# google/lyra

Measured on NVIDIA H100. Metric: 20ms-frame encode+decode throughput (frames/s) @16kHz, higher is better.
Workload: dtype f32+i8 (decoder fp32 GEMMs: split tf32 on tensor cores)

## Files before the change

lyra_b200/csrc/engine.cu:

```cuda
#include <cmath>
#include <cstdio>
#include <cstdlib>
#include <cstring>
#include <string>
#include <vector>

#include "../../include/lyra_b200.h"
#include "aux_kernels.cuh"
#include "model_spec.h"
#include "net_kernels.cuh"
#include "net_kernels_wgmma.cuh"
#include "plc_kernels.cuh"

using namespace lyra_b200;

namespace {

std::string g_create_error;

#define CU(call)                                                                        \
  do {                                                                                  \
    cudaError_t e_ = (call);                                                            \
    if (e_ != cudaSuccess) {                                                            \
      ctx->err = std::string(#call) + ": " + cudaGetErrorString(e_);                    \
      return LYRA_B200_ENODEV;                                                          \
    }                                                                                   \
  } while (0)

#define ENTER(role)                                                                     \
  if (!UseDevice(ctx)) return LYRA_B200_ENODEV;                                         \
  if ((role) && !RoleOk(ctx, (role))) return LYRA_B200_EINVAL;

}

struct lyra_b200_ctx {
  ModelSpec spec;
  int device = 0, max_streams = 0, ntiles = 0, padded = 0;
  int roles = LYRA_B200_ROLE_ENCODER | LYRA_B200_ROLE_DECODER;
  std::vector<void*> allocs;
  enum Check { kCheckNone, kCheckPlc, kCheckResamplerPos, kCheckStreamRate, kCheckStreamBits };
  struct StateEntry {
    StreamStateEntry e;
    bool reset;
    int check;
  };
  std::vector<StateEntry> state_list;
  StreamStateTable state_table{};
  StreamStateTable reset_table{};
  uint64_t model_fingerprint = 0;
  uint32_t* d_records = nullptr;
  int records_chunk = 0;
  uint8_t* d_blob = nullptr;
  uint32_t* d_state[4] = {nullptr, nullptr, nullptr, nullptr};
  int* d_n18[4] = {nullptr, nullptr, nullptr, nullptr};
  float* d_mid_enc = nullptr;
  float* d_mid_dec = nullptr;
  int16_t* d_logmel_prev[3] = {nullptr, nullptr, nullptr};
  float* d_noise = nullptr;
  float* d_noise_est = nullptr;
  uint8_t* d_is_noise = nullptr;
  float* d_noise_enc = nullptr;
  int16_t* d_logmel_prev_enc = nullptr;
  NoiseParams noise_params{};
  int* d_plc = nullptr;
  double* d_cng_work = nullptr;
  unsigned long long* d_cng_hops = nullptr;
  unsigned long long cng_seed = 0;
  uint8_t* d_plan = nullptr;
  uint8_t* d_skip = nullptr;
  uint8_t* d_feed = nullptr;
  uint8_t* d_is_cn = nullptr;
  int* d_fade0 = nullptr;
  int* d_dir = nullptr;
  int16_t* d_model_pcm = nullptr;
  int16_t* d_cng_pcm = nullptr;
  float* d_cng_feat = nullptr;
  int16_t* d_rs_delay[2] = {nullptr, nullptr};
  int* d_rs_pos[2] = {nullptr, nullptr};
  int16_t* d_rs_in = nullptr;
  int16_t* d_rs_out = nullptr;
  int* d_rs_counts = nullptr;
  int sample_rate = 16000;
  int codec_rs_tag = 1;
  int16_t* d_codec_rs_delay[2] = {nullptr, nullptr};
  int* d_codec_rs_pos[2] = {nullptr, nullptr};
  int* d_stream_rate = nullptr;
  bool rate_override = false;
  ByRate<NoiseParams> enc_noise_params{};
  ByRate<LogMelParams> enc_logmel{};
  int* d_stream_bits[2] = {nullptr, nullptr};
  std::vector<int> bits_mirror[2];
  int own_bits[2] = {0, 0};
  int16_t* d_pcm = nullptr;
  uint8_t* d_packets = nullptr;
  uint8_t* d_received = nullptr;
  float* d_features = nullptr;
  float* d_melout = nullptr;
  int* d_indices = nullptr;
  int* d_ids = nullptr;
  int* d_tile_list = nullptr;
  int* d_slot_of = nullptr;
  int* h_tile_list[2] = {nullptr, nullptr};
  int* h_slot_of[2] = {nullptr, nullptr};
  cudaEvent_t ev_map[2] = {nullptr, nullptr};
  bool map_pending[2] = {false, false};
  int map_buf = 0;
  std::vector<uint32_t> tile_gen;
  uint32_t map_gen = 0;
  std::vector<uint32_t> id_seen;
  uint32_t id_gen = 0;
  std::vector<int> touched[2];
  int map_dense_n = -1;
  int active_tiles = 0;
  cudaStream_t own_stream = nullptr, stream = nullptr;
  static constexpr int kMaxSplit = 4;
  cudaStream_t aux_stream[kMaxSplit - 1] = {nullptr, nullptr, nullptr};
  cudaEvent_t ev_fork = nullptr, ev_join[kMaxSplit - 1] = {nullptr, nullptr, nullptr};
  int nsplit = 3;
  bool blocking_sync = false;
  cudaEvent_t ev_sync = nullptr;
  int decoder_mode = LYRA_B200_DECODER_EXACT;
  int priority = 0;
  uint64_t launches = 0;
  struct GraphKey {
    int kind, n, num_bits, mode, nsplit;
    const void *a, *b, *c;
    bool rates, bits;
    bool operator==(const GraphKey& o) const {
      return kind == o.kind && n == o.n && num_bits == o.num_bits && mode == o.mode && nsplit == o.nsplit && a == o.a && b == o.b && c == o.c &&
             rates == o.rates && bits == o.bits;
    }
  };
  struct GraphEntry { GraphKey key; void* exec; uint64_t launches; };
  bool use_graphs = false;
  std::vector<GraphEntry> graphs;
  uint64_t graph_replays = 0;
  std::string err;
  bool profiling = false;
  std::vector<std::pair<cudaEvent_t, cudaEvent_t>> prof_events[LYRA_B200_NUM_KERNELS];
  size_t prof_used[LYRA_B200_NUM_KERNELS] = {};
  double prof_ms[LYRA_B200_NUM_KERNELS] = {};
  uint64_t prof_n[LYRA_B200_NUM_KERNELS] = {};
};

namespace {

int PacketBytes(int num_bits) { return (num_bits + 7) / 8; }

int RatePair(int rate_hz) { return rate_hz == 8000 ? 0 : rate_hz == 32000 ? 1 : rate_hz == 48000 ? 2 : -1; }
bool RateOk(int rate_hz) { return rate_hz == 16000 || RatePair(rate_hz) >= 0; }

bool Converts(const lyra_b200_ctx* ctx) { return ctx->sample_rate != 16000 || ctx->rate_override; }

NoiseParams MakeNoiseParams(int rate_hz) {
  NoiseParams p{};
  const float secs_per_hop = static_cast<float>(320) / rate_hz;
  p.nf = 160;
  p.hops_per_update = (int)std::round(1.f / secs_per_hop);
  p.max_smoothing = std::pow(0.5f, secs_per_hop / 0.7f);
  p.bound_decay = std::pow(0.5f, secs_per_hop / 1.f);
  p.log_nf = std::log((double)160);
  return p;
}

constexpr int kNoProf = -1;
struct ProfScope {
  lyra_b200_ctx* ctx;
  int k;
  cudaEvent_t stop = nullptr;
  cudaStream_t st;
  ProfScope(lyra_b200_ctx* c, int kernel, cudaStream_t stream) : ctx(c), k(kernel), st(stream) {
    if (!ctx->profiling || k == kNoProf) return;
    auto& pool = ctx->prof_events[k];
    if (ctx->prof_used[k] == pool.size()) {
      cudaEvent_t a, b;
      cudaEventCreate(&a);
      cudaEventCreate(&b);
      pool.emplace_back(a, b);
    }
    auto& ev = pool[ctx->prof_used[k]++];
    cudaEventRecord(ev.first, st);
    stop = ev.second;
  }
  ~ProfScope() { if (stop) cudaEventRecord(stop, st); }
};

template <typename Fn>
int Launch(lyra_b200_ctx* ctx, int prof, cudaStream_t st, Fn launch) {
  {
    ProfScope ps(ctx, prof, st);
    launch();
  }
  ctx->launches += 1;
  CU(cudaGetLastError());
  return LYRA_B200_OK;
}
#define LAUNCH(prof, kernel, grid, block, smem, st, ...) \
  Launch(ctx, (prof), (st), [&]() { LYRA_LAUNCH(kernel, grid, block, smem, st, __VA_ARGS__); })

void ProfDrain(lyra_b200_ctx* ctx) {
  for (int k = 0; k < LYRA_B200_NUM_KERNELS; ++k) {
    for (size_t i = 0; i < ctx->prof_used[k]; ++i) {
      float ms = 0.0f;
      if (cudaEventElapsedTime(&ms, ctx->prof_events[k][i].first, ctx->prof_events[k][i].second) == cudaSuccess) {
        ctx->prof_ms[k] += ms;
        ctx->prof_n[k] += 1;
      }
    }
    ctx->prof_used[k] = 0;
  }
}

cudaError_t SyncStream(lyra_b200_ctx* ctx) {
  if (!ctx->blocking_sync) return cudaStreamSynchronize(ctx->stream);
  cudaError_t e = cudaEventRecord(ctx->ev_sync, ctx->stream);
  return e != cudaSuccess ? e : cudaEventSynchronize(ctx->ev_sync);
}

bool UseDevice(lyra_b200_ctx* ctx) {
  if (cudaSetDevice(ctx->device) == cudaSuccess) return true;
  ctx->err = "cudaSetDevice failed";
  return false;
}

bool RoleOk(lyra_b200_ctx* ctx, int role) {
  if (ctx->roles & role) return true;
  ctx->err = role == LYRA_B200_ROLE_ENCODER ? "this context was created without the encoder role" : "this context was created without the decoder role";
  return false;
}

bool BitsOk(lyra_b200_ctx* ctx, int num_bits) {
  if (num_bits <= 0 || num_bits > LYRA_B200_MAX_BITS) { ctx->err = "the number of bits cannot exceed 184"; return false; }
  if (num_bits % ctx->spec.bits_per_stage != 0) { ctx->err = "the number of bits has to be divisible by the bits per quantizer (4)"; return false; }
  return true;
}

bool StreamBitsOk(const lyra_b200_ctx* ctx, int bits) {
  return bits > 0 && bits <= LYRA_B200_MAX_BITS && bits % ctx->spec.bits_per_stage == 0;
}

const int* BitsWord(const lyra_b200_ctx* ctx, int r) { return ctx->own_bits[r] ? ctx->d_stream_bits[r] : nullptr; }

void SetMirrorBits(lyra_b200_ctx* ctx, int r, int id, int bits) {
  int& w = ctx->bits_mirror[r][(size_t)id];
  ctx->own_bits[r] += (bits != 0) - (w != 0);
  w = bits;
}

uint32_t NextIdGen(lyra_b200_ctx* ctx) {
  if (++ctx->id_gen == 0) { std::fill(ctx->id_seen.begin(), ctx->id_seen.end(), 0u); ctx->id_gen = 1; }
  return ctx->id_gen;
}

int CheckIds(lyra_b200_ctx* ctx, const int32_t* ids, int n, bool allow_repeats) {
  if (n <= 0 || n > ctx->max_streams) { ctx->err = "stream count out of range"; return LYRA_B200_EINVAL; }
  if (!ids) return LYRA_B200_OK;
  const uint32_t gen = NextIdGen(ctx);
  for (int k = 0; k < n; ++k) {
    const int id = ids[k];
    if (id < 0 || id >= ctx->max_streams) { ctx->err = "stream id out of range"; return LYRA_B200_EINVAL; }
    if (allow_repeats) continue;
    if (ctx->id_seen[(size_t)id] == gen) { ctx->err = "duplicate stream id in one call"; return LYRA_B200_EINVAL; }
    ctx->id_seen[(size_t)id] = gen;
  }
  return LYRA_B200_OK;
}

int UploadIds(lyra_b200_ctx* ctx, const int32_t* ids, int n, const int** d_ids) {
  *d_ids = nullptr;
  if (!ids) return LYRA_B200_OK;
  CU(cudaMemcpyAsync(ctx->d_ids, ids, sizeof(int) * (size_t)n, cudaMemcpyHostToDevice, ctx->stream));
  *d_ids = ctx->d_ids;
  return LYRA_B200_OK;
}

int PrepareMap(lyra_b200_ctx* ctx, const int32_t* ids, int n) {
  int rc = CheckIds(ctx, ids, n, false);
  if (rc) return rc;
  if (ids == nullptr && ctx->map_dense_n == n) return LYRA_B200_OK;
  const int b = ctx->map_buf;
  if (ctx->map_pending[b]) { CU(cudaEventSynchronize(ctx->ev_map[b])); ctx->map_pending[b] = false; }
  int* slot_of = ctx->h_slot_of[b];
  int* tile_list = ctx->h_tile_list[b];
  for (int id : ctx->touched[b]) slot_of[id] = -1;
  ctx->touched[b].clear();
  int ntl = 0;
  for (int k = 0; k < n; ++k) {
    const int id = ids ? ids[k] : k;
    slot_of[id] = k;
    ctx->touched[b].push_back(id);
  }
  if (++ctx->map_gen == 0) { std::fill(ctx->tile_gen.begin(), ctx->tile_gen.end(), 0u); ctx->map_gen = 1; }
  for (int k = 0; k < n; ++k) {
    const int t = (ids ? ids[k] : k) / kTileStreams;
    if (ctx->tile_gen[(size_t)t] != ctx->map_gen) { ctx->tile_gen[(size_t)t] = ctx->map_gen; tile_list[ntl++] = t; }
  }
  ctx->active_tiles = ntl;
  CU(cudaMemcpyAsync(ctx->d_slot_of, slot_of, sizeof(int) * (size_t)ctx->padded, cudaMemcpyHostToDevice, ctx->stream));
  CU(cudaMemcpyAsync(ctx->d_tile_list, tile_list, sizeof(int) * (size_t)ntl, cudaMemcpyHostToDevice, ctx->stream));
  CU(cudaEventRecord(ctx->ev_map[b], ctx->stream));
  ctx->map_pending[b] = true;
  ctx->map_buf = b ^ 1;
  ctx->map_dense_n = ids ? -1 : n;
  return LYRA_B200_OK;
}

struct Part {
  int tile0, ntiles, slot0, nslots;
  cudaStream_t st;
};
Part WholeCall(lyra_b200_ctx* ctx, int n) { return Part{0, ctx->active_tiles, 0, n, ctx->stream}; }

int LaunchEncoderNets(lyra_b200_ctx* ctx, const Part& p, const uint8_t* skip, const int16_t* d_pcm, float* d_features) {
  const TileIo io{ctx->d_tile_list + p.tile0, ctx->d_slot_of, skip};
  const int rc = LAUNCH(0, EncoderKernelA, dim3((unsigned)p.ntiles), dim3(EncA::NT), (size_t)EncA::kSmemBytes, p.st,
                        ctx->d_blob, ctx->spec.enc, io, d_pcm, reinterpret_cast<float*>(ctx->d_state[0]), ctx->d_n18[0], ctx->d_mid_enc);
  return rc ? rc : LAUNCH(1, EncoderKernelB, dim3((unsigned)p.ntiles), dim3(EncB::NT), (size_t)EncB::kSmemBytes, p.st,
                          ctx->d_blob, ctx->spec.enc, io, ctx->d_mid_enc, reinterpret_cast<float*>(ctx->d_state[1]), ctx->d_n18[1], d_features);
}

int LaunchQuantize(lyra_b200_ctx* ctx, const Part& p, const float* d_features, int num_bits, uint8_t* d_packets, int* d_indices,
                   const uint8_t* d_skip = nullptr, const int* bits_word = nullptr, const int* d_ids = nullptr) {
  const int nq = num_bits / ctx->spec.bits_per_stage, pb = PacketBytes(num_bits);
  const int blocks = (p.nslots + kRvqSlotsPerBlock - 1) / kRvqSlotsPerBlock;
  return LAUNCH(2, RvqEncodeKernel, dim3((unsigned)blocks), dim3(kRvqThreads), (size_t)(2 * 1024 * 4 + kRvqSlotsPerBlock * (64 * 4 + 48 * 4)), p.st,
                ctx->d_blob, ctx->spec.rvq, d_features + (size_t)p.slot0 * 64, p.nslots, nq, d_packets + (size_t)p.slot0 * pb, pb,
                d_indices ? d_indices + (size_t)p.slot0 * 46 : nullptr, d_skip ? d_skip + p.slot0 : nullptr, bits_word, d_ids, p.slot0);
}

int LaunchDequantize(lyra_b200_ctx* ctx, const Part& p, const uint8_t* d_packets, const uint8_t* d_received, int num_bits, float* d_features,
                     const int* bits_word = nullptr, const int* d_ids = nullptr) {
  const int nq = num_bits / ctx->spec.bits_per_stage, pb = PacketBytes(num_bits);
  const int blocks = (p.nslots * 64 + 255) / 256;
  return LAUNCH(3, RvqDecodeKernel, dim3((unsigned)blocks), dim3(256), (size_t)0, p.st,
                ctx->d_blob, ctx->spec.rvq, d_packets + (size_t)p.slot0 * pb, pb, d_received ? d_received + p.slot0 : nullptr, p.nslots, nq,
                d_features + (size_t)p.slot0 * 64, bits_word, d_ids, p.slot0);
}

int LaunchDecoderNets(lyra_b200_ctx* ctx, const Part& p, const uint8_t* skip, const float* d_features, int16_t* d_pcm) {
  const TileIo io{ctx->d_tile_list + p.tile0, ctx->d_slot_of, skip};
  const bool tc = ctx->decoder_mode == LYRA_B200_DECODER_TENSOR;
  const dim3 grid((unsigned)p.ntiles);
  float* st_c = reinterpret_cast<float*>(ctx->d_state[2]);
  float* st_d = reinterpret_cast<float*>(ctx->d_state[3]);
  const int rc = tc ? LAUNCH(4, DecoderKernelC<true>, grid, dim3(DecC<true>::NT), (size_t)DecC<true>::kSmemBytes, p.st,
                             ctx->d_blob, ctx->spec.dec, io, d_features, st_c, ctx->d_n18[2], ctx->d_mid_dec)
                    : LAUNCH(4, DecoderKernelC<false>, grid, dim3(DecC<false>::NT), (size_t)DecC<false>::kSmemBytes, p.st,
                             ctx->d_blob, ctx->spec.dec, io, d_features, st_c, ctx->d_n18[2], ctx->d_mid_dec);
  if (rc) return rc;
  return tc ? LAUNCH(5, DecoderKernelDW, grid, dim3(DecDW::NT), (size_t)DecDW::kSmemBytes, p.st,
                     ctx->d_blob, ctx->spec.dec, io, ctx->d_mid_dec, st_d, ctx->d_n18[3], d_pcm)
            : LAUNCH(5, DecoderKernelD, grid, dim3(DecD::NT), (size_t)DecD::kSmemBytes, p.st,
                     ctx->d_blob, ctx->spec.dec, io, ctx->d_mid_dec, st_d, ctx->d_n18[3], d_pcm);
}

int SplitParts(lyra_b200_ctx* ctx, int n, Part* parts) {
  int np = ctx->nsplit < 1 ? 1 : (ctx->nsplit > lyra_b200_ctx::kMaxSplit ? lyra_b200_ctx::kMaxSplit : ctx->nsplit);
  if (!(ctx->map_dense_n == n && ctx->active_tiles >= 64 * np)) np = 1;
  if (np == 1) { parts[0] = WholeCall(ctx, n); return 1; }
  for (int i = 0; i < np; ++i) {
    const int t0 = (int)((long long)ctx->active_tiles * i / np), t1 = (int)((long long)ctx->active_tiles * (i + 1) / np);
    const int s0 = t0 * kTileStreams, s1 = i + 1 == np ? n : t1 * kTileStreams;
    parts[i] = Part{t0, t1 - t0, s0, s1 - s0, i == 0 ? ctx->stream : ctx->aux_stream[i - 1]};
  }
  return np;
}
int Fork(lyra_b200_ctx* ctx, int nparts) {
  if (nparts < 2) return LYRA_B200_OK;
  CU(cudaEventRecord(ctx->ev_fork, ctx->stream));
  for (int i = 1; i < nparts; ++i) CU(cudaStreamWaitEvent(ctx->aux_stream[i - 1], ctx->ev_fork, 0));
  return LYRA_B200_OK;
}
int Join(lyra_b200_ctx* ctx, int nparts) {
  for (int i = 1; i < nparts; ++i) {
    CU(cudaEventRecord(ctx->ev_join[i - 1], ctx->aux_stream[i - 1]));
    CU(cudaStreamWaitEvent(ctx->stream, ctx->ev_join[i - 1], 0));
  }
  return LYRA_B200_OK;
}
int JoinAfter(lyra_b200_ctx* ctx, int nparts, int rc) {
  if (!rc) return Join(ctx, nparts);
  const std::string first = ctx->err;
  Join(ctx, nparts);
  cudaStreamSynchronize(ctx->stream);
  ctx->err = first;
  return rc;
}

template <typename Fn>
int ForEachPart(lyra_b200_ctx* ctx, int n, Fn body) {
  Part parts[lyra_b200_ctx::kMaxSplit];
  const int np = SplitParts(ctx, n, parts);
  int rc = Fork(ctx, np);
  if (rc) return rc;
  for (int i = 0; i < np && !rc; ++i) rc = body(parts[i]);
  return JoinAfter(ctx, np, rc);
}

int LaunchLogMel(lyra_b200_ctx* ctx, cudaStream_t st, const ByRate<LogMelParams>& S, const int* rate_word, int rate, const int* d_ids,
                 int slot0, int count, int n, const int16_t* d_pcm, int16_t* carried, const uint8_t* d_mask) {
  const LogMelParams& P = S.p[0];
  const size_t smem = sizeof(double) * (size_t)(2 * kLogMelFftPadded + P.fft / 2 + 1 + P.window_len + P.window_len / 8 + 1);
  return LAUNCH(6, LogMelKernel, dim3((unsigned)count), dim3(kLogMelThreads), smem, st,
                ctx->d_blob, S, rate_word, rate, d_ids, n, d_pcm, carried, ctx->d_melout, d_mask, slot0);
}

int LaunchNoiseUpdate(lyra_b200_ctx* ctx, cudaStream_t st, const int* d_ids, int slot0, int count, int n, const int16_t* d_pcm,
                      const uint8_t* d_mask, uint8_t* d_is_noise, float* d_estimate, bool encoder_side = false) {
  float* noise_state = encoder_side ? ctx->d_noise_enc : ctx->d_noise;
  int16_t* carried = encoder_side ? ctx->d_logmel_prev_enc : ctx->d_logmel_prev[2];
  const int* rate_word = encoder_side ? ctx->d_stream_rate : nullptr;
  const int rate = encoder_side ? ctx->sample_rate : 16000;
  const int rc = LaunchLogMel(ctx, st, encoder_side ? ctx->enc_logmel : Uniform(ctx->spec.logmel160), rate_word, rate, d_ids, slot0, count, n,
                              d_pcm, carried, d_mask);
  return rc ? rc : LAUNCH(7, NoiseEstimatorKernel, dim3((unsigned)count), dim3(kNoiseThreads), sizeof(float) * (size_t)(2 * 160 + 2), st,
                          encoder_side ? ctx->enc_noise_params : Uniform(ctx->noise_params), rate_word, rate, d_ids, n, ctx->d_melout, d_mask,
                          noise_state, d_is_noise, d_estimate, slot0);
}

int LaunchComfortNoise(lyra_b200_ctx* ctx, cudaStream_t st, const int* d_ids, int slot0, int count, int n, const float* d_features,
                       const uint8_t* d_plan) {
  const size_t smem = sizeof(double) * (size_t)(4 * kLogMelFftPadded + 160);
  return LAUNCH(kNoProf, ComfortNoiseKernel, dim3((unsigned)count), dim3(kCngThreads), smem, st,
                ctx->d_blob, ctx->spec.cng, d_ids, n, d_features, ctx->d_noise, NoiseStateUnits(ctx->noise_params.nf),
                d_plan, ctx->d_cng_work, ctx->d_cng_hops, ctx->cng_seed, ctx->d_cng_pcm, slot0);
}

int LaunchCodecResample(lyra_b200_ctx* ctx, const Part& p, int dir, const int* d_ids, int n, const int16_t* in, int16_t* out) {
  const int ext = ctx->sample_rate / 50;
  const int in_stride = dir ? LYRA_B200_HOP : ext, out_stride = dir ? ext : LYRA_B200_HOP;
  return LAUNCH(kNoProf, ResampleKernel, dim3((unsigned)p.nslots), dim3(128), sizeof(float) * (size_t)(kResamplerTaps - 1 + in_stride), p.st,
                ctx->d_blob, ctx->spec.resampler, dir ? 3 : 0, ctx->codec_rs_tag, d_ids, n, in, in_stride, in_stride, out, out_stride,
                nullptr, ctx->d_codec_rs_delay[dir], ctx->d_codec_rs_pos[dir], p.slot0, ctx->d_stream_rate, ctx->sample_rate);
}

enum CallKind { kEncode, kDecode, kEncodeDtx, kDecodeTrackNoise, kDecodePlc };

struct CodecCall {
  struct Io {
    const int16_t* pcm_in = nullptr;
    int16_t* pcm_out = nullptr;
    const uint8_t* packets_in = nullptr;
    uint8_t* packets_out = nullptr;
    const uint8_t* received = nullptr;
    uint8_t* flags = nullptr;
  };
  CallKind kind;
  int n, num_bits;
  const int32_t* ids = nullptr;
  Io dev, host;
  int32_t* packet_bytes = nullptr;
  const int* d_ids = nullptr;
};

int RunEncode(lyra_b200_ctx* ctx, const CodecCall& c) {
  const CodecCall::Io &d = c.dev, &h = c.host;
  const bool dtx = c.kind == kEncodeDtx;
  const size_t pb = (size_t)PacketBytes(c.num_bits), hop = (size_t)ctx->sample_rate / 50;
  const bool rs = Converts(ctx);
  int16_t* stage = rs ? ctx->d_rs_in : ctx->d_pcm;
  const int16_t* in = h.pcm_in ? stage : d.pcm_in;
  const int16_t* pcm16 = rs ? ctx->d_pcm : in;
  const uint8_t* skip = dtx ? d.flags : nullptr;
  return ForEachPart(ctx, c.n, [&](const Part& p) {
    int rc = LYRA_B200_OK;
    if (h.pcm_in)
      CU(cudaMemcpyAsync(stage + (size_t)p.slot0 * hop, h.pcm_in + (size_t)p.slot0 * hop, sizeof(int16_t) * hop * (size_t)p.nslots,
                         cudaMemcpyHostToDevice, p.st));
    if (rs && (rc = LaunchCodecResample(ctx, p, 0, c.d_ids, c.n, in, ctx->d_pcm))) return rc;
    if (dtx) {
      if ((rc = LaunchNoiseUpdate(ctx, p.st, c.d_ids, p.slot0, p.nslots, c.n, pcm16, nullptr, d.flags, nullptr, true))) return rc;
      if (h.flags) CU(cudaMemcpyAsync(h.flags + p.slot0, d.flags + p.slot0, (size_t)p.nslots, cudaMemcpyDeviceToHost, p.st));
    }
    if ((rc = LaunchEncoderNets(ctx, p, skip, pcm16, ctx->d_features))) return rc;
    if ((rc = LaunchQuantize(ctx, p, ctx->d_features, c.num_bits, d.packets_out, nullptr, skip, BitsWord(ctx, 0), c.d_ids))) return rc;
    if (h.packets_out)
      CU(cudaMemcpyAsync(h.packets_out + (size_t)p.slot0 * pb, d.packets_out + (size_t)p.slot0 * pb, pb * (size_t)p.nslots, cudaMemcpyDeviceToHost, p.st));
    return LYRA_B200_OK;
  });
}

int RunDecode(lyra_b200_ctx* ctx, const CodecCall& c) {
  const CodecCall::Io &d = c.dev, &h = c.host;
  const size_t pb = (size_t)PacketBytes(c.num_bits), hop = (size_t)ctx->sample_rate / 50;
  const bool rs = Converts(ctx);
  int16_t* out = h.pcm_out && rs ? ctx->d_rs_out : d.pcm_out;
  int16_t* pcm16 = rs ? ctx->d_pcm : out;
  return ForEachPart(ctx, c.n, [&](const Part& p) {
    int rc = LYRA_B200_OK;
    if (h.packets_in)
      CU(cudaMemcpyAsync(ctx->d_packets + (size_t)p.slot0 * pb, h.packets_in + (size_t)p.slot0 * pb, pb * (size_t)p.nslots, cudaMemcpyHostToDevice, p.st));
    if (h.received)
      CU(cudaMemcpyAsync(ctx->d_received + p.slot0, h.received + p.slot0, (size_t)p.nslots, cudaMemcpyHostToDevice, p.st));
    if ((rc = LaunchDequantize(ctx, p, d.packets_in, d.received, c.num_bits, ctx->d_features, BitsWord(ctx, 1), c.d_ids))) return rc;
    if ((rc = LaunchDecoderNets(ctx, p, nullptr, ctx->d_features, pcm16))) return rc;
    if (c.kind == kDecodeTrackNoise) {
      if ((rc = LaunchNoiseUpdate(ctx, p.st, c.d_ids, p.slot0, p.nslots, c.n, pcm16, d.received, d.flags, nullptr))) return rc;
      if (h.flags) CU(cudaMemcpyAsync(h.flags + p.slot0, d.flags + p.slot0, (size_t)p.nslots, cudaMemcpyDeviceToHost, p.st));
    }
    if (rs && (rc = LaunchCodecResample(ctx, p, 1, c.d_ids, c.n, pcm16, out))) return rc;
    if (h.pcm_out)
      CU(cudaMemcpyAsync(h.pcm_out + (size_t)p.slot0 * hop, out + (size_t)p.slot0 * hop, sizeof(int16_t) * hop * (size_t)p.nslots,
                         cudaMemcpyDeviceToHost, p.st));
    return LYRA_B200_OK;
  });
}

int RunDecodePlc(lyra_b200_ctx* ctx, const CodecCall& c) {
  const CodecCall::Io &d = c.dev, &h = c.host;
  const size_t pb = (size_t)PacketBytes(c.num_bits), hop = (size_t)ctx->sample_rate / 50;
  const bool rs = Converts(ctx);
  int16_t* out = h.pcm_out && rs ? ctx->d_rs_out : d.pcm_out;
  int16_t* pcm16 = rs ? ctx->d_pcm : out;
  if (h.received) CU(cudaMemcpyAsync(ctx->d_received, h.received, (size_t)c.n, cudaMemcpyHostToDevice, ctx->stream));
  if (int rc = LAUNCH(kNoProf, PlcPlanKernel, dim3((unsigned)((c.n + 255) / 256)), dim3(256), (size_t)0, ctx->stream,
                      c.d_ids, c.n, d.received, ctx->d_plc, ctx->d_plan, ctx->d_fade0, ctx->d_dir, ctx->d_skip, ctx->d_feed, d.flags))
    return rc;
  return ForEachPart(ctx, c.n, [&](const Part& p) {
    int rc = LYRA_B200_OK;
    if (h.packets_in)
      CU(cudaMemcpyAsync(ctx->d_packets + (size_t)p.slot0 * pb, h.packets_in + (size_t)p.slot0 * pb, pb * (size_t)p.nslots, cudaMemcpyHostToDevice, p.st));
    if ((rc = LaunchDequantize(ctx, p, d.packets_in, d.received, c.num_bits, ctx->d_features, BitsWord(ctx, 1), c.d_ids))) return rc;
    if ((rc = LaunchDecoderNets(ctx, p, ctx->d_skip, ctx->d_features, ctx->d_model_pcm))) return rc;
    if ((rc = LaunchComfortNoise(ctx, p.st, c.d_ids, p.slot0, p.nslots, c.n, nullptr, ctx->d_plan))) return rc;
    if ((rc = LAUNCH(kNoProf, PlcMixKernel, dim3((unsigned)p.nslots), dim3(320), (size_t)0, p.st,
                     ctx->d_blob, ctx->spec.cng, p.nslots, ctx->d_plan + p.slot0, ctx->d_fade0 + p.slot0, ctx->d_dir + p.slot0,
                     ctx->d_model_pcm + (size_t)p.slot0 * 320, ctx->d_cng_pcm + (size_t)p.slot0 * 320, pcm16 + (size_t)p.slot0 * 320)))
      return rc;
    if ((rc = LaunchNoiseUpdate(ctx, p.st, c.d_ids, p.slot0, p.nslots, c.n, ctx->d_model_pcm, ctx->d_feed, nullptr, nullptr))) return rc;
    if (rs && (rc = LaunchCodecResample(ctx, p, 1, c.d_ids, c.n, pcm16, out))) return rc;
    if (h.pcm_out)
      CU(cudaMemcpyAsync(h.pcm_out + (size_t)p.slot0 * hop, out + (size_t)p.slot0 * hop, sizeof(int16_t) * hop * (size_t)p.nslots,
                         cudaMemcpyDeviceToHost, p.st));
    if (h.flags) CU(cudaMemcpyAsync(h.flags + p.slot0, d.flags + p.slot0, (size_t)p.nslots, cudaMemcpyDeviceToHost, p.st));
    return LYRA_B200_OK;
  });
}

bool SetSmemLimits() {
  return LYRA_SET_MAX_SMEM(EncoderKernelA, EncA::kSmemBytes) == 0 && LYRA_SET_MAX_SMEM(EncoderKernelB, EncB::kSmemBytes) == 0 &&
         LYRA_SET_MAX_SMEM(DecoderKernelC<false>, DecC<false>::kSmemBytes) == 0 && LYRA_SET_MAX_SMEM(DecoderKernelD, DecD::kSmemBytes) == 0 &&
         LYRA_SET_MAX_SMEM(DecoderKernelC<true>, DecC<true>::kSmemBytes) == 0 && LYRA_SET_MAX_SMEM(DecoderKernelDW, DecDW::kSmemBytes) == 0;
}

std::vector<uint32_t> InitImage(const ModelSpec& s, int which) {
  auto pack = [](int zp) { const uint32_t b = (uint32_t)(zp & 0xff); return b | (b << 8) | (b << 16) | (b << 24); };
  std::vector<uint32_t> v;
  if (which == 0) {
    v.assign(EncStateA::kUnits, 0u);
  } else if (which == 1) {
    v.assign(EncStateB::kUnits, 0u);
    for (int i = EncStateB::kRingQ0; i < EncStateB::kRingQ1; ++i) v[(size_t)i] = pack(s.enc.zp_state[0]);
    for (int i = EncStateB::kRingQ1; i < EncStateB::kDown2; ++i) v[(size_t)i] = pack(s.enc.zp_state[1]);
    for (int i = EncStateB::kDown2; i < EncStateB::kBott; ++i) v[(size_t)i] = pack(s.enc.zp_state[2]);
    for (int i = EncStateB::kBott; i < EncStateB::kUnits; ++i) v[(size_t)i] = pack(s.enc.zp_state[3]);
  } else if (which == 2) {
    v.assign(DecStateC::kUnits, 0u);
    for (int i = DecStateC::kRingM; i < DecStateC::kRingQ0; ++i) v[(size_t)i] = pack(s.dec.zp_state[0]);
    for (int i = DecStateC::kRingQ0; i < DecStateC::kRingQ1; ++i) v[(size_t)i] = pack(s.dec.zp_state[1]);
    for (int i = DecStateC::kRingQ1; i < DecStateC::kUnits; ++i) v[(size_t)i] = pack(s.dec.zp_state[2]);
  } else {
    v.assign(DecStateD::kUnits, 0u);
  }
  return v;
}

template <typename T>
bool DevAlloc(lyra_b200_ctx* ctx, T** p, size_t count) {
  const size_t bytes = sizeof(T) * (count ? count : 1);
  if (cudaMalloc(reinterpret_cast<void**>(p), bytes) != cudaSuccess) return false;
  ctx->allocs.push_back(*p);
  return cudaMemset(*p, 0, bytes) == cudaSuccess;
}

template <typename T>
bool DevStreamState(lyra_b200_ctx* ctx, T** p, size_t per_stream, const void* init = nullptr, int kind = kStatePlain,
                    int check = lyra_b200_ctx::kCheckNone, bool reset = true, int lanes = 1, int** n18 = nullptr) {
  const int words = (int)(sizeof(T) * per_stream / 4);
  uint32_t* d_init = nullptr;
  if (!DevAlloc(ctx, p, (size_t)ctx->padded * per_stream)) return false;
  if (n18 && !DevAlloc(ctx, n18, (size_t)ctx->padded)) return false;
  if (init && !(DevAlloc(ctx, &d_init, (size_t)words) && cudaMemcpy(d_init, init, 4 * (size_t)words, cudaMemcpyHostToDevice) == cudaSuccess))
    return false;
  ctx->state_list.push_back({{reinterpret_cast<uint32_t*>(*p), d_init, n18 ? *n18 : nullptr, words, lanes, 0, kind}, reset, check});
  return true;
}

uint64_t ModelFingerprint(const std::vector<uint8_t>& blob) {
  uint64_t h = 0xcbf29ce484222325ull ^ (uint64_t)blob.size();
  size_t i = 0;
  for (; i + 8 <= blob.size(); i += 8) {
    uint64_t w;
    std::memcpy(&w, blob.data() + i, 8);
    h = (h ^ w) * 0x100000001b3ull;
  }
  for (; i < blob.size(); ++i) h = (h ^ blob[i]) * 0x100000001b3ull;
  return h;
}

bool BuildStateTable(lyra_b200_ctx* ctx) {
  StreamStateTable& T = ctx->state_table;
  StreamStateTable& R = ctx->reset_table;
  if ((int)ctx->state_list.size() > kStateMaxEntries) return false;
  int off = 0;
  T.count = R.count = 0;
  for (lyra_b200_ctx::StateEntry& s : ctx->state_list) {
    s.e.offset = off;
    off += s.e.words + (s.e.n18 ? 1 : 0);
    T.e[T.count++] = s.e;
    if (s.reset) R.e[R.count++] = s.e;
  }
  T.record_words = kStateHeaderWords + off;
  std::memset(T.header, 0, sizeof(T.header));
  T.header[kHdrMagic] = kStateMagic;
  T.header[kHdrVersion] = kStateVersion;
  T.header[kHdrBytes] = (uint32_t)(4 * T.record_words);
  T.header[kHdrRoles] = (uint32_t)ctx->roles;
  T.header[kHdrModelLo] = (uint32_t)ctx->model_fingerprint;
  T.header[kHdrModelHi] = (uint32_t)(ctx->model_fingerprint >> 32);
  return true;
}

#ifndef LYRA_EMU
bool PinnedHost(const void* p) {
  if (p == nullptr) return true;
  cudaPointerAttributes at;
  if (cudaPointerGetAttributes(&at, p) != cudaSuccess) { cudaGetLastError(); return false; }
  return at.type == cudaMemoryTypeHost;
}
void DropGraphs(lyra_b200_ctx* ctx) {
  for (auto& e : ctx->graphs) cudaGraphExecDestroy(reinterpret_cast<cudaGraphExec_t>(e.exec));
  ctx->graphs.clear();
}
#endif

template <typename Fn>
int RunMaybeGraphed(lyra_b200_ctx* ctx, const lyra_b200_ctx::GraphKey& key, bool eligible, Fn enqueue) {
#ifdef LYRA_EMU
  (void)key; (void)eligible;
  return enqueue();
#else
  if (!ctx->use_graphs || !eligible || ctx->profiling || !PinnedHost(key.a) || !PinnedHost(key.b) || !PinnedHost(key.c)) return enqueue();
  for (auto& e : ctx->graphs)
    if (e.key == key) {
      CU(cudaGraphLaunch(reinterpret_cast<cudaGraphExec_t>(e.exec), ctx->stream));
      ctx->launches += e.launches;
      ++ctx->graph_replays;
      return LYRA_B200_OK;
    }
  const uint64_t l0 = ctx->launches;
  if (cudaStreamBeginCapture(ctx->stream, cudaStreamCaptureModeThreadLocal) != cudaSuccess) {
    cudaGetLastError();
    ctx->use_graphs = false;
    return enqueue();
  }
  const int rc = enqueue();
  cudaGraph_t g = nullptr;
  const cudaError_t ce = cudaStreamEndCapture(ctx->stream, &g);
  cudaGraphExec_t exec = nullptr;
  if (rc == LYRA_B200_OK && ce == cudaSuccess && g != nullptr && cudaGraphInstantiate(&exec, g, 0) == cudaSuccess) {
    cudaGraphDestroy(g);
    if (ctx->graphs.size() >= 32) {
      cudaGraphExecDestroy(reinterpret_cast<cudaGraphExec_t>(ctx->graphs.front().exec));
      ctx->graphs.erase(ctx->graphs.begin());
    }
    ctx->graphs.push_back(lyra_b200_ctx::GraphEntry{key, exec, ctx->launches - l0});
    CU(cudaGraphLaunch(exec, ctx->stream));
    return LYRA_B200_OK;
  }
  if (g) cudaGraphDestroy(g);
  cudaGetLastError();
  ctx->use_graphs = false;
  ctx->launches = l0;
  return enqueue();
#endif
}

int RunCodecCall(lyra_b200_ctx* ctx, CodecCall c) {
  const bool encoder = c.kind == kEncode || c.kind == kEncodeDtx;
  const int role = encoder ? LYRA_B200_ROLE_ENCODER : LYRA_B200_ROLE_DECODER;
  ENTER(role);
  if (!BitsOk(ctx, c.num_bits)) return LYRA_B200_EINVAL;
  const int r = encoder ? 0 : 1;
  const std::vector<int>& own = ctx->bits_mirror[r];
  for (int k = 0; k < c.n && ctx->own_bits[r]; ++k) {
    const int id = c.ids ? c.ids[k] : k;
    if (id >= 0 && id < ctx->max_streams && own[(size_t)id] > c.num_bits) {
      ctx->err = "a listed stream's own bit count (lyra_b200_set_stream_bits) is above the call's num_bits";
      return LYRA_B200_EINVAL;
    }
  }
  const bool by_id = Converts(ctx) || (c.kind != kEncode && c.kind != kDecode) || ctx->own_bits[r];
  int rc = PrepareMap(ctx, c.ids, c.n);
  if (rc || (by_id && (rc = UploadIds(ctx, c.ids, c.n, &c.d_ids)))) return rc;
  const bool host = c.host.packets_in || c.host.packets_out;
  if (host) {
    c.dev.pcm_in = c.dev.pcm_out = ctx->d_pcm;
    c.dev.packets_in = c.dev.packets_out = ctx->d_packets;
    c.dev.received = c.host.received ? ctx->d_received : nullptr;
  }
  if (!c.dev.flags) c.dev.flags = c.kind == kDecodePlc ? ctx->d_is_cn : ctx->d_is_noise;
  std::vector<uint8_t> dtx_flags;
  if (c.packet_bytes) {
    dtx_flags.resize((size_t)c.n);
    c.host.flags = dtx_flags.data();
  }
  const CodecCall::Io& h = c.host;
  const lyra_b200_ctx::GraphKey key =
      encoder ? lyra_b200_ctx::GraphKey{kEncode, c.n, c.num_bits, 0, ctx->nsplit, h.pcm_in, h.packets_out, nullptr, ctx->rate_override,
                                        ctx->own_bits[r] != 0}
              : lyra_b200_ctx::GraphKey{kDecode, c.n, c.num_bits, ctx->decoder_mode, ctx->nsplit, h.packets_in, h.received, h.pcm_out,
                                        ctx->rate_override, ctx->own_bits[r] != 0};
  const bool graphed = host && (c.kind == kEncode || c.kind == kDecode) && c.ids == nullptr && ctx->map_dense_n == c.n;
  if ((rc = RunMaybeGraphed(ctx, key, graphed, [&]() {
         return encoder ? RunEncode(ctx, c) : c.kind == kDecodePlc ? RunDecodePlc(ctx, c) : RunDecode(ctx, c);
       })))
    return rc;
  if (!host) return LYRA_B200_OK;
  CU(SyncStream(ctx));
  for (int k = 0; k < c.n && c.packet_bytes; ++k) {
    const int b = own[(size_t)(c.ids ? c.ids[k] : k)];
    c.packet_bytes[k] = dtx_flags[(size_t)k] ? 0 : PacketBytes(b ? b : c.num_bits);
  }
  return LYRA_B200_OK;
}


size_t RecordBytes(const lyra_b200_ctx* ctx) { return 4 * (size_t)ctx->state_table.record_words; }

int EnsureRecordStaging(lyra_b200_ctx* ctx) {
  if (ctx->d_records) return LYRA_B200_OK;
  const size_t fit = ((size_t)64 << 20) / RecordBytes(ctx);
  const int chunk = fit < 1 ? 1 : fit > (size_t)kStateChunk ? kStateChunk : (int)fit;
  uint32_t* p = nullptr;
  CU(cudaMalloc(reinterpret_cast<void**>(&p), RecordBytes(ctx) * (size_t)chunk));
  ctx->allocs.push_back(p);
  ctx->d_records = p;
  ctx->records_chunk = chunk;
  return LYRA_B200_OK;
}

bool PlcStateOk(int cp, int fp, int dir) {
  return cp >= 0 && cp <= kPlcConcealSamples && cp % 320 == 0 && fp >= 0 && fp <= kPlcFadeSamples && fp % 320 == 0 &&
         (dir == 1 || dir == -1);
}

bool StreamRateOk(const lyra_b200_ctx* ctx, int rate_hz) { return RateOk(rate_hz) && rate_hz <= ctx->sample_rate; }

uint32_t RecordWord(const uint8_t* rec, int i) {
  uint32_t w;
  std::memcpy(&w, rec + 4 * (size_t)i, 4);
  return w;
}

const char* RecordProblem(const lyra_b200_ctx* ctx, const uint8_t* rec) {
  const StreamStateTable& T = ctx->state_table;
  if (RecordWord(rec, kHdrMagic) != kStateMagic) return "not a stream-state record";
  if (RecordWord(rec, kHdrVersion) != kStateVersion) return "record format version differs";
  if (RecordWord(rec, kHdrBytes) != T.header[kHdrBytes] || RecordWord(rec, kHdrRoles) != T.header[kHdrRoles])
    return "record size / roles differ from this context's";
  if (RecordWord(rec, kHdrRate) != (uint32_t)ctx->sample_rate) return "record is from a context at another sample rate";
  if (RecordWord(rec, kHdrModelLo) != T.header[kHdrModelLo] || RecordWord(rec, kHdrModelHi) != T.header[kHdrModelHi])
    return "record is from another model";
  if (RecordWord(rec, kHdrZero5) || RecordWord(rec, kHdrLive0) > 1 || RecordWord(rec, kHdrLive1) > 1) return "malformed record header";
  for (int i = kHdrKeyHi + 1; i < kStateHeaderWords; ++i)
    if (RecordWord(rec, i)) return "malformed record header";
  for (int i = 0; i < T.count; ++i) {
    const StreamStateEntry& e = T.e[i];
    const int w0 = kStateHeaderWords + e.offset;
    if (e.n18 && RecordWord(rec, w0 + e.words) >= 18u) return "hop counter out of range";
    const int check = ctx->state_list[(size_t)i].check;
    if (check == lyra_b200_ctx::kCheckResamplerPos && (int32_t)RecordWord(rec, w0) < 0) return "resampler position out of range";
    if (check == lyra_b200_ctx::kCheckPlc &&
        !PlcStateOk((int32_t)RecordWord(rec, w0), (int32_t)RecordWord(rec, w0 + 1), (int32_t)RecordWord(rec, w0 + 2)))
      return "decoder control state out of range";
    if (check == lyra_b200_ctx::kCheckStreamRate && RecordWord(rec, w0) != 0 && !StreamRateOk(ctx, (int32_t)RecordWord(rec, w0)))
      return "stream sample rate unsupported or above the context's";
    if (check == lyra_b200_ctx::kCheckStreamBits && RecordWord(rec, w0) != 0 && !StreamBitsOk(ctx, (int32_t)RecordWord(rec, w0)))
      return "stream bit count is not a multiple of 4 in 4..184";
  }
  return nullptr;
}

int CheckCopyIds(lyra_b200_ctx* ctx, const int32_t* src, const int32_t* dst, int n) {
  if (n <= 0 || n > ctx->max_streams) { ctx->err = "stream count out of range"; return LYRA_B200_EINVAL; }
  const uint32_t g[2] = {NextIdGen(ctx), NextIdGen(ctx)};
  for (int k = 0; k < n; ++k) {
    const int id = src[k];
    if (id < -1 || id >= ctx->max_streams) { ctx->err = "source stream id out of range"; return LYRA_B200_EINVAL; }
    if (id < 0) continue;
    if (ctx->id_seen[(size_t)id] == g[0]) { ctx->err = "repeated source stream id"; return LYRA_B200_EINVAL; }
    ctx->id_seen[(size_t)id] = g[0];
  }
  for (int k = 0; k < n; ++k) {
    const int id = dst[k];
    if (id < 0 || id >= ctx->max_streams) { ctx->err = "destination stream id out of range"; return LYRA_B200_EINVAL; }
    if (ctx->id_seen[(size_t)id] == g[1]) { ctx->err = "repeated destination stream id"; return LYRA_B200_EINVAL; }
    if (ctx->id_seen[(size_t)id] == g[0]) { ctx->err = "a stream id is both a source and a destination"; return LYRA_B200_EINVAL; }
    ctx->id_seen[(size_t)id] = g[1];
  }
  return LYRA_B200_OK;
}

dim3 StateGrid(const StreamStateTable& T, int rows, int extra) {
  return dim3((unsigned)((rows + kStateRows - 1) / kStateRows), (unsigned)(T.count + extra));
}

int CopyStreamState(lyra_b200_ctx* ctx, const StreamStateTable& T, const int32_t* src, const int32_t* dst, int n) {
  StreamIdChunk ids;
  for (int k0 = 0; k0 < n; k0 += kStateChunk) {
    ids.n = n - k0 < kStateChunk ? n - k0 : kStateChunk;
    for (int k = 0; k < ids.n; ++k) {
      ids.src[k] = src ? src[k0 + k] : -1;
      ids.dst[k] = dst ? dst[k0 + k] : k0 + k;
    }
    if (int rc = LAUNCH(kNoProf, StreamStateCopyKernel, StateGrid(T, ids.n, 0), dim3(kStateThreads), (size_t)0, ctx->stream, T, ids))
      return rc;
  }
  return LYRA_B200_OK;
}

int LaunchStreamWords(lyra_b200_ctx* ctx, const int32_t* ids, int n, const int32_t* values, int ctx_value, int* word, int* conv0 = nullptr,
                      int* conv1 = nullptr) {
  StreamRateChunk c;
  for (int k0 = 0; k0 < n; k0 += kStateChunk) {
    c.n = n - k0 < kStateChunk ? n - k0 : kStateChunk;
    for (int k = 0; k < c.n; ++k) {
      c.ids[k] = ids ? ids[k0 + k] : k0 + k;
      c.rates[k] = values ? values[k0 + k] : ctx_value;
    }
    if (int rc = LAUNCH(kNoProf, StreamRateKernel, dim3((unsigned)((c.n + kStreamRateThreads - 1) / kStreamRateThreads)),
                        dim3(kStreamRateThreads), (size_t)0, ctx->stream, c, ctx_value, word, conv0, conv1))
      return rc;
  }
  return LYRA_B200_OK;
}
int LaunchStreamRates(lyra_b200_ctx* ctx, const int32_t* ids, int n, const int32_t* rates) {
  return LaunchStreamWords(ctx, ids, n, rates, ctx->sample_rate, ctx->d_stream_rate, ctx->d_codec_rs_pos[0], ctx->d_codec_rs_pos[1]);
}

int BitsRole(lyra_b200_ctx* ctx, int role) {
  if (role != LYRA_B200_ROLE_ENCODER && role != LYRA_B200_ROLE_DECODER) { ctx->err = "role must be LYRA_B200_ROLE_ENCODER or _DECODER"; return -1; }
  return RoleOk(ctx, role) ? role - 1 : -1;
}

}

extern "C" {

int lyra_b200_create(const char* model_dir, int device, int max_streams, lyra_b200_ctx** out) {
  return lyra_b200_create_ex(model_dir, device, max_streams, LYRA_B200_ROLE_ENCODER | LYRA_B200_ROLE_DECODER, out);
}

int lyra_b200_create_ex(const char* model_dir, int device, int max_streams, int roles, lyra_b200_ctx** out) {
  if (out) *out = nullptr;
  if (!out || !model_dir || max_streams <= 0 || (roles & ~3) || roles == 0) { g_create_error = "bad argument"; return LYRA_B200_EINVAL; }
  int ndev = 0;
  if (cudaGetDeviceCount(&ndev) != cudaSuccess || ndev <= 0) {
    g_create_error = "no CUDA device available (lyra_b200 has no CPU fallback)";
    return LYRA_B200_ENODEV;
  }
  if (device < 0 || device >= ndev) { g_create_error = "CUDA device index out of range"; return LYRA_B200_ENODEV; }
  lyra_b200_ctx* ctx = new lyra_b200_ctx();
  try {
    ctx->spec = BuildModelSpec(model_dir);
  } catch (const std::exception& e) {
    g_create_error = e.what();
    delete ctx;
    return LYRA_B200_EMODEL;
  }
  ctx->device = device;
  ctx->max_streams = max_streams;
  ctx->roles = roles;
  ctx->ntiles = (max_streams + kTileStreams - 1) / kTileStreams;
  ctx->padded = ctx->ntiles * kTileStreams;
  ctx->tile_gen.assign((size_t)ctx->ntiles, 0u);
  ctx->id_seen.assign((size_t)max_streams, 0u);
  const size_t P = (size_t)ctx->padded;
  bool ok = cudaSetDevice(device) == cudaSuccess;
  int prio = 0;
  if (const char* e = std::getenv(roles == LYRA_B200_ROLE_DECODER ? "LYRA_B200_DEC_PRIORITY" : "LYRA_B200_ENC_PRIORITY")) prio = std::atoi(e);
  ctx->priority = prio;
  ok = ok && cudaStreamCreateWithPriority(&ctx->own_stream, cudaStreamDefault, prio) == cudaSuccess;
  for (int i = 0; i < lyra_b200_ctx::kMaxSplit - 1; ++i) {
    ok = ok && cudaStreamCreateWithPriority(&ctx->aux_stream[i], cudaStreamDefault, prio) == cudaSuccess;
    ok = ok && cudaEventCreateWithFlags(&ctx->ev_join[i], cudaEventDisableTiming) == cudaSuccess;
  }
  ok = ok && cudaEventCreateWithFlags(&ctx->ev_fork, cudaEventDisableTiming) == cudaSuccess;
  ok = ok && cudaEventCreateWithFlags(&ctx->ev_sync, cudaEventDisableTiming | cudaEventBlockingSync) == cudaSuccess;
  ctx->stream = ctx->own_stream;
  ok = ok && DevAlloc(ctx, &ctx->d_blob, ctx->spec.blob.size());
  ok = ok && cudaMemcpy(ctx->d_blob, ctx->spec.blob.data(), ctx->spec.blob.size(), cudaMemcpyHostToDevice) == cudaSuccess;
  const int units[4] = {EncStateA::kUnits, EncStateB::kUnits, DecStateC::kUnits, DecStateD::kUnits};
  for (int w = 0; w < 4 && ok; ++w) {
    if (!(roles & (w < 2 ? LYRA_B200_ROLE_ENCODER : LYRA_B200_ROLE_DECODER))) continue;
    ok = DevStreamState(ctx, &ctx->d_state[w], (size_t)units[w], InitImage(ctx->spec, w).data(), kStatePlain, lyra_b200_ctx::kCheckNone,
                        true, kTileStreams, &ctx->d_n18[w]);
  }
  if (roles & LYRA_B200_ROLE_ENCODER) ok = ok && DevAlloc(ctx, &ctx->d_mid_enc, P * 128 * 4);
  if (roles & LYRA_B200_ROLE_DECODER) ok = ok && DevAlloc(ctx, &ctx->d_mid_dec, P * 128 * 4);
  for (int b = 0; b < 3; ++b) ok = ok && DevStreamState(ctx, &ctx->d_logmel_prev[b], LYRA_B200_HOP);
  ctx->noise_params = MakeNoiseParams(16000);
  for (int r : {16000, 8000, 32000, 48000}) {
    ctx->enc_noise_params.p[RateIndex(r)] = MakeNoiseParams(r);
    ctx->enc_logmel.p[RateIndex(r)] = r == 16000 ? ctx->spec.logmel160 : ctx->spec.logmel160_ext[RatePair(r)];
  }
  ok = ok && DevStreamState(ctx, &ctx->d_noise, NoiseStateUnits(160));
  ok = ok && DevAlloc(ctx, &ctx->d_noise_est, P * 160);
  ok = ok && DevStreamState(ctx, &ctx->d_noise_enc, NoiseStateUnits(160));
  ok = ok && DevStreamState(ctx, &ctx->d_logmel_prev_enc, LYRA_B200_HOP);
  const int plc0[4] = {0, 0, -1, 0};
  ok = ok && DevStreamState(ctx, &ctx->d_plc, 4, plc0, kStatePlain, lyra_b200_ctx::kCheckPlc);
  ok = ok && DevStreamState(ctx, &ctx->d_cng_work, 1024);
  ok = ok && DevStreamState(ctx, &ctx->d_cng_hops, 2, nullptr, kStateCng);
  ok = ok && DevAlloc(ctx, &ctx->d_plan, P);
  ok = ok && DevAlloc(ctx, &ctx->d_skip, P);
  ok = ok && DevAlloc(ctx, &ctx->d_feed, P);
  ok = ok && DevAlloc(ctx, &ctx->d_is_cn, P);
  ok = ok && DevAlloc(ctx, &ctx->d_fade0, P);
  ok = ok && DevAlloc(ctx, &ctx->d_dir, P);
  ok = ok && DevAlloc(ctx, &ctx->d_model_pcm, P * LYRA_B200_HOP);
  ok = ok && DevAlloc(ctx, &ctx->d_cng_pcm, P * LYRA_B200_HOP);
  ok = ok && DevAlloc(ctx, &ctx->d_cng_feat, P * 160);
  for (int d = 0; d < 2; ++d) {
    ok = ok && DevStreamState(ctx, &ctx->d_rs_delay[d], (size_t)(kResamplerTaps - 1), nullptr, kStatePlain, lyra_b200_ctx::kCheckNone, false);
    ok = ok && DevStreamState(ctx, &ctx->d_rs_pos[d], 2, nullptr, kStatePlain, lyra_b200_ctx::kCheckResamplerPos);
  }
  for (int d = 0; d < 2; ++d) {
    if (!(roles & (d == 0 ? LYRA_B200_ROLE_ENCODER : LYRA_B200_ROLE_DECODER))) continue;
    ok = ok && DevStreamState(ctx, &ctx->d_codec_rs_delay[d], (size_t)(kResamplerTaps - 1));
    ok = ok && DevStreamState(ctx, &ctx->d_codec_rs_pos[d], 2, nullptr, d == 0 ? kStateCodecRs0 : kStateCodecRs1,
                              lyra_b200_ctx::kCheckResamplerPos);
  }
  for (int r = 0; r < 2; ++r) {
    if (!(roles & (r + 1))) continue;
    ok = ok && DevStreamState(ctx, &ctx->d_stream_bits[r], 1, nullptr, kStatePlain, lyra_b200_ctx::kCheckStreamBits);
    ctx->bits_mirror[r].assign((size_t)max_streams, 0);
  }
  ok = ok && DevStreamState(ctx, &ctx->d_stream_rate, 1, nullptr, kStatePlain, lyra_b200_ctx::kCheckStreamRate);
  ok = ok && DevAlloc(ctx, &ctx->d_rs_in, P * 960);
  ok = ok && DevAlloc(ctx, &ctx->d_rs_out, P * 968);
  ok = ok && DevAlloc(ctx, &ctx->d_rs_counts, P);
  ok = ok && DevAlloc(ctx, &ctx->d_is_noise, P);
  ok = ok && DevAlloc(ctx, &ctx->d_pcm, P * LYRA_B200_HOP);
  ok = ok && DevAlloc(ctx, &ctx->d_packets, P * 24);
  ok = ok && DevAlloc(ctx, &ctx->d_received, P);
  ok = ok && DevAlloc(ctx, &ctx->d_features, P * LYRA_B200_NUM_FEATURES);
  ok = ok && DevAlloc(ctx, &ctx->d_melout, P * 160);
  ok = ok && DevAlloc(ctx, &ctx->d_indices, P * LYRA_B200_MAX_STAGES);
  ok = ok && DevAlloc(ctx, &ctx->d_ids, P);
  ok = ok && DevAlloc(ctx, &ctx->d_tile_list, (size_t)ctx->ntiles);
  ok = ok && DevAlloc(ctx, &ctx->d_slot_of, P);
  for (int b = 0; b < 2 && ok; ++b) {
    ok = ok && cudaMallocHost(reinterpret_cast<void**>(&ctx->h_slot_of[b]), sizeof(int) * P) == cudaSuccess;
    ok = ok && cudaMallocHost(reinterpret_cast<void**>(&ctx->h_tile_list[b]), sizeof(int) * (size_t)ctx->ntiles) == cudaSuccess;
    ok = ok && cudaEventCreateWithFlags(&ctx->ev_map[b], cudaEventDisableTiming) == cudaSuccess;
    if (ok) for (size_t i = 0; i < P; ++i) ctx->h_slot_of[b][i] = -1;
  }
  if (ok) ok = SetSmemLimits();
  ctx->model_fingerprint = ModelFingerprint(ctx->spec.blob);
  ok = ok && BuildStateTable(ctx);
  if (!ok) {
    g_create_error = std::string("CUDA allocation / setup failed: ") + cudaGetErrorString(cudaGetLastError());
    lyra_b200_destroy(ctx);
    return LYRA_B200_ENODEV;
  }
  if (lyra_b200_reset(ctx, nullptr, max_streams) != LYRA_B200_OK) {
    g_create_error = ctx->err;
    lyra_b200_destroy(ctx);
    return LYRA_B200_ENODEV;
  }
  *out = ctx;
  return LYRA_B200_OK;
}

void lyra_b200_destroy(lyra_b200_ctx* ctx) {
  if (!ctx) return;
  UseDevice(ctx);
  for (void* p : ctx->allocs) cudaFree(p);
  for (int b = 0; b < 2; ++b) {
    if (ctx->h_slot_of[b]) cudaFreeHost(ctx->h_slot_of[b]);
    if (ctx->h_tile_list[b]) cudaFreeHost(ctx->h_tile_list[b]);
    if (ctx->ev_map[b]) cudaEventDestroy(ctx->ev_map[b]);
  }
  for (int k = 0; k < LYRA_B200_NUM_KERNELS; ++k)
    for (auto& ev : ctx->prof_events[k]) { cudaEventDestroy(ev.first); cudaEventDestroy(ev.second); }
#ifndef LYRA_EMU
  DropGraphs(ctx);
#endif
  if (ctx->ev_fork) cudaEventDestroy(ctx->ev_fork);
  if (ctx->ev_sync) cudaEventDestroy(ctx->ev_sync);
  for (int i = 0; i < lyra_b200_ctx::kMaxSplit - 1; ++i) {
    if (ctx->ev_join[i]) cudaEventDestroy(ctx->ev_join[i]);
    if (ctx->aux_stream[i]) cudaStreamDestroy(ctx->aux_stream[i]);
  }
  if (ctx->own_stream) cudaStreamDestroy(ctx->own_stream);
  delete ctx;
}

const char* lyra_b200_last_error(const lyra_b200_ctx* ctx) { return ctx ? ctx->err.c_str() : g_create_error.c_str(); }
int lyra_b200_max_streams(const lyra_b200_ctx* ctx) { return ctx ? ctx->max_streams : 0; }
int lyra_b200_tile_streams(const lyra_b200_ctx* ctx) { return ctx ? kTileStreams : 0; }
uint64_t lyra_b200_launch_count(const lyra_b200_ctx* ctx) { return ctx ? ctx->launches : 0; }

int lyra_b200_profile_enable(lyra_b200_ctx* ctx, int enable) {
  if (!ctx) return LYRA_B200_EINVAL;
  ENTER(0);
  CU(SyncStream(ctx));
  ProfDrain(ctx);
  ctx->profiling = enable != 0;
  if (enable) for (int k = 0; k < LYRA_B200_NUM_KERNELS; ++k) { ctx->prof_ms[k] = 0.0; ctx->prof_n[k] = 0; }
  return LYRA_B200_OK;
}

int lyra_b200_profile_read(lyra_b200_ctx* ctx, double* ms_sum, uint64_t* launches) {
  if (!ctx || !ms_sum || !launches) return LYRA_B200_EINVAL;
  ENTER(0);
  CU(SyncStream(ctx));
  ProfDrain(ctx);
  for (int k = 0; k < LYRA_B200_NUM_KERNELS; ++k) { ms_sum[k] = ctx->prof_ms[k]; launches[k] = ctx->prof_n[k]; }
  return LYRA_B200_OK;
}

int lyra_b200_reset(lyra_b200_ctx* ctx, const int32_t* stream_ids, int n) {
  if (!ctx) return LYRA_B200_EINVAL;
  ENTER(0);
  int rc = CheckIds(ctx, stream_ids, n, true);
  if (rc) return rc;
  std::vector<int32_t> distinct;
  if (stream_ids) {
    const uint32_t gen = NextIdGen(ctx);
    for (int k = 0; k < n; ++k)
      if (ctx->id_seen[(size_t)stream_ids[k]] != gen) { ctx->id_seen[(size_t)stream_ids[k]] = gen; distinct.push_back(stream_ids[k]); }
    stream_ids = distinct.data();
    n = (int)distinct.size();
  }
  if ((rc = CopyStreamState(ctx, ctx->reset_table, nullptr, stream_ids, n))) return rc;
  for (int r = 0; r < 2; ++r)
    for (int k = 0; k < n && ctx->own_bits[r]; ++k) SetMirrorBits(ctx, r, stream_ids ? stream_ids[k] : k, 0);
  CU(SyncStream(ctx));
  return LYRA_B200_OK;
}

int lyra_b200_set_stream(lyra_b200_ctx* ctx, void* cuda_stream) {
  if (!ctx) return LYRA_B200_EINVAL;
  ENTER(0);
  ctx->stream = cuda_stream ? reinterpret_cast<cudaStream_t>(cuda_stream) : ctx->own_stream;
  return LYRA_B200_OK;
}

int lyra_b200_set_split(lyra_b200_ctx* ctx, int parts) {
  if (!ctx || parts < 1 || parts > lyra_b200_ctx::kMaxSplit) return LYRA_B200_EINVAL;
  ENTER(0);
  ctx->nsplit = parts;
  return LYRA_B200_OK;
}

int lyra_b200_set_blocking_sync(lyra_b200_ctx* ctx, int enable) {
  if (!ctx) return LYRA_B200_EINVAL;
  ENTER(0);
  ctx->blocking_sync = enable != 0;
  return LYRA_B200_OK;
}

int lyra_b200_set_priority(lyra_b200_ctx* ctx, int priority) {
  if (!ctx) return LYRA_B200_EINVAL;
  ENTER(0);
  CU(SyncStream(ctx));
#ifndef LYRA_EMU
  DropGraphs(ctx);
#endif
  const bool own = ctx->stream == ctx->own_stream;
  cudaStream_t fresh[lyra_b200_ctx::kMaxSplit];
  for (int i = 0; i < lyra_b200_ctx::kMaxSplit; ++i)
    if (cudaStreamCreateWithPriority(&fresh[i], cudaStreamDefault, priority) != cudaSuccess) {
      while (i-- > 0) cudaStreamDestroy(fresh[i]);
      ctx->err = "cudaStreamCreateWithPriority failed";
      return LYRA_B200_ENODEV;
    }
  cudaStreamDestroy(ctx->own_stream);
  ctx->own_stream = fresh[0];
  for (int i = 0; i < lyra_b200_ctx::kMaxSplit - 1; ++i) { cudaStreamDestroy(ctx->aux_stream[i]); ctx->aux_stream[i] = fresh[i + 1]; }
  if (own) ctx->stream = ctx->own_stream;
  ctx->priority = priority;
  return LYRA_B200_OK;
}

int lyra_b200_set_decoder_mode(lyra_b200_ctx* ctx, int mode) {
  if (!ctx || (mode != LYRA_B200_DECODER_EXACT && mode != LYRA_B200_DECODER_TENSOR)) return LYRA_B200_EINVAL;
  ENTER(0);
  ctx->decoder_mode = mode;
  return LYRA_B200_OK;
}

int lyra_b200_decoder_mode(const lyra_b200_ctx* ctx) { return ctx ? ctx->decoder_mode : LYRA_B200_EINVAL; }

int lyra_b200_set_sample_rate(lyra_b200_ctx* ctx, int sample_rate_hz) {
  if (!ctx) return LYRA_B200_EINVAL;
  if (!RateOk(sample_rate_hz)) { ctx->err = "the codec calls run at 8000, 16000, 32000 or 48000 Hz"; return LYRA_B200_EINVAL; }
  ENTER(0);
  if (sample_rate_hz == ctx->sample_rate && !ctx->rate_override) return LYRA_B200_OK;
  CU(SyncStream(ctx));
  if (sample_rate_hz == ctx->sample_rate) {
    int rc = LaunchStreamRates(ctx, nullptr, ctx->max_streams, nullptr);
    if (rc) return rc;
    CU(SyncStream(ctx));
    ctx->rate_override = false;
    return LYRA_B200_OK;
  }
#ifndef LYRA_EMU
  DropGraphs(ctx);
#endif
  if (ctx->rate_override) {
    CU(cudaMemsetAsync(ctx->d_stream_rate, 0, sizeof(int) * (size_t)ctx->padded, ctx->stream));
    CU(SyncStream(ctx));
    ctx->rate_override = false;
  }
  ctx->sample_rate = sample_rate_hz;
  ctx->codec_rs_tag = ctx->codec_rs_tag % 1000000000 + 1;
  return LYRA_B200_OK;
}

int lyra_b200_set_stream_sample_rates(lyra_b200_ctx* ctx, const int32_t* stream_ids, int n, const int32_t* rates_hz) {
  if (!ctx || !rates_hz) return LYRA_B200_EINVAL;
  ENTER(0);
  int rc = CheckIds(ctx, stream_ids, n, false);
  if (rc) return rc;
  bool differs = false;
  for (int k = 0; k < n; ++k) {
    if (!StreamRateOk(ctx, rates_hz[k])) {
      ctx->err = "a stream runs at 8000, 16000, 32000 or 48000 Hz, at most the context's rate (lyra_b200_set_sample_rate)";
      return LYRA_B200_EINVAL;
    }
    differs |= rates_hz[k] != ctx->sample_rate;
  }
  if (!differs && !ctx->rate_override) return LYRA_B200_OK;
  if ((rc = LaunchStreamRates(ctx, stream_ids, n, rates_hz))) return rc;
  ctx->rate_override = true;
  return LYRA_B200_OK;
}

int lyra_b200_stream_sample_rates(lyra_b200_ctx* ctx, const int32_t* stream_ids, int n, int32_t* rates_hz) {
  if (!ctx || !rates_hz) return LYRA_B200_EINVAL;
  ENTER(0);
  const int rc = CheckIds(ctx, stream_ids, n, true);
  if (rc) return rc;
  CU(SyncStream(ctx));
  std::vector<int> words((size_t)ctx->max_streams);
  CU(cudaMemcpy(words.data(), ctx->d_stream_rate, sizeof(int) * words.size(), cudaMemcpyDeviceToHost));
  for (int k = 0; k < n; ++k) {
    const int w = words[(size_t)(stream_ids ? stream_ids[k] : k)];
    rates_hz[k] = w ? w : ctx->sample_rate;
  }
  return LYRA_B200_OK;
}

int lyra_b200_sample_rate(const lyra_b200_ctx* ctx) { return ctx ? ctx->sample_rate : LYRA_B200_EINVAL; }

int lyra_b200_set_stream_bits(lyra_b200_ctx* ctx, int role, const int32_t* stream_ids, int n, const int32_t* bits) {
  if (!ctx || !bits) return LYRA_B200_EINVAL;
  ENTER(0);
  const int r = BitsRole(ctx, role);
  if (r < 0) return LYRA_B200_EINVAL;
  int rc = CheckIds(ctx, stream_ids, n, false);
  if (rc) return rc;
  bool changes = false;
  for (int k = 0; k < n; ++k) {
    if (bits[k] != 0 && !StreamBitsOk(ctx, bits[k])) {
      ctx->err = "a stream's own bit count is 0 (the call's) or a multiple of 4 in 4..184";
      return LYRA_B200_EINVAL;
    }
    changes |= ctx->bits_mirror[r][(size_t)(stream_ids ? stream_ids[k] : k)] != bits[k];
  }
  if (!changes) return LYRA_B200_OK;
  if ((rc = LaunchStreamWords(ctx, stream_ids, n, bits, 0, ctx->d_stream_bits[r]))) return rc;
  for (int k = 0; k < n; ++k) SetMirrorBits(ctx, r, stream_ids ? stream_ids[k] : k, bits[k]);
  return LYRA_B200_OK;
}

int lyra_b200_stream_bits(lyra_b200_ctx* ctx, int role, const int32_t* stream_ids, int n, int32_t* bits) {
  if (!ctx || !bits) return LYRA_B200_EINVAL;
  ENTER(0);
  const int r = BitsRole(ctx, role);
  if (r < 0) return LYRA_B200_EINVAL;
  const int rc = CheckIds(ctx, stream_ids, n, true);
  if (rc) return rc;
  CU(SyncStream(ctx));
  std::vector<int> words((size_t)ctx->max_streams);
  CU(cudaMemcpy(words.data(), ctx->d_stream_bits[r], sizeof(int) * words.size(), cudaMemcpyDeviceToHost));
  for (int k = 0; k < n; ++k) bits[k] = words[(size_t)(stream_ids ? stream_ids[k] : k)];
  return LYRA_B200_OK;
}

int lyra_b200_synchronize(lyra_b200_ctx* ctx) {
  if (!ctx) return LYRA_B200_EINVAL;
  ENTER(0);
  CU(SyncStream(ctx));
  return LYRA_B200_OK;
}

int lyra_b200_encode_device(lyra_b200_ctx* ctx, int n, const int16_t* d_pcm, int num_bits, uint8_t* d_packets) {
  if (!ctx || !d_pcm || !d_packets) return LYRA_B200_EINVAL;
  CodecCall c{kEncode, n, num_bits};
  c.dev.pcm_in = d_pcm;
  c.dev.packets_out = d_packets;
  return RunCodecCall(ctx, c);
}

int lyra_b200_decode_device(lyra_b200_ctx* ctx, int n, const uint8_t* d_packets, const uint8_t* d_received, int num_bits,
                            int16_t* d_pcm) {
  if (!ctx || !d_packets || !d_pcm) return LYRA_B200_EINVAL;
  CodecCall c{kDecode, n, num_bits};
  c.dev.packets_in = d_packets;
  c.dev.received = d_received;
  c.dev.pcm_out = d_pcm;
  return RunCodecCall(ctx, c);
}

int lyra_b200_set_graphs(lyra_b200_ctx* ctx, int enable) {
  if (!ctx) return LYRA_B200_EINVAL;
  ENTER(0);
#ifndef LYRA_EMU
  CU(SyncStream(ctx));
  if (!enable) DropGraphs(ctx);
#endif
  ctx->use_graphs = enable != 0;
  return LYRA_B200_OK;
}
uint64_t lyra_b200_graph_replays(const lyra_b200_ctx* ctx) { return ctx ? ctx->graph_replays : 0; }

int lyra_b200_encode(lyra_b200_ctx* ctx, const int32_t* ids, int n, const int16_t* pcm, int num_bits, uint8_t* packets) {
  if (!ctx || !pcm || !packets) return LYRA_B200_EINVAL;
  CodecCall c{kEncode, n, num_bits, ids};
  c.host.pcm_in = pcm;
  c.host.packets_out = packets;
  return RunCodecCall(ctx, c);
}

int lyra_b200_decode(lyra_b200_ctx* ctx, const int32_t* ids, int n, const uint8_t* packets, const uint8_t* received,
                     int num_bits, int16_t* pcm) {
  if (!ctx || !packets || !pcm) return LYRA_B200_EINVAL;
  CodecCall c{kDecode, n, num_bits, ids};
  c.host.packets_in = packets;
  c.host.received = received;
  c.host.pcm_out = pcm;
  return RunCodecCall(ctx, c);
}

int lyra_b200_extract_features(lyra_b200_ctx* ctx, const int32_t* ids, int n, const int16_t* pcm, float* features) {
  if (!ctx || !pcm || !features) return LYRA_B200_EINVAL;
  ENTER(LYRA_B200_ROLE_ENCODER);
  int rc = PrepareMap(ctx, ids, n);
  if (rc) return rc;
  CU(cudaMemcpyAsync(ctx->d_pcm, pcm, sizeof(int16_t) * 320 * (size_t)n, cudaMemcpyHostToDevice, ctx->stream));
  if ((rc = LaunchEncoderNets(ctx, WholeCall(ctx, n), nullptr, ctx->d_pcm, ctx->d_features))) return rc;
  CU(cudaMemcpyAsync(features, ctx->d_features, sizeof(float) * 64 * (size_t)n, cudaMemcpyDeviceToHost, ctx->stream));
  CU(SyncStream(ctx));
  return LYRA_B200_OK;
}

int lyra_b200_quantize(lyra_b200_ctx* ctx, int n, const float* features, int num_bits, uint8_t* packets, int32_t* indices) {
  if (!ctx || !features || !packets) return LYRA_B200_EINVAL;
  ENTER(0);
  if (!BitsOk(ctx, num_bits)) return LYRA_B200_EINVAL;
  int rc = CheckIds(ctx, nullptr, n, false);
  if (rc) return rc;
  CU(cudaMemcpyAsync(ctx->d_features, features, sizeof(float) * 64 * (size_t)n, cudaMemcpyHostToDevice, ctx->stream));
  const Part whole{0, 0, 0, n, ctx->stream};
  rc = LaunchQuantize(ctx, whole, ctx->d_features, num_bits, ctx->d_packets, indices ? ctx->d_indices : nullptr);
  if (rc) return rc;
  CU(cudaMemcpyAsync(packets, ctx->d_packets, (size_t)PacketBytes(num_bits) * (size_t)n, cudaMemcpyDeviceToHost, ctx->stream));
  if (indices) CU(cudaMemcpyAsync(indices, ctx->d_indices, sizeof(int) * 46 * (size_t)n, cudaMemcpyDeviceToHost, ctx->stream));
  CU(SyncStream(ctx));
  return LYRA_B200_OK;
}

int lyra_b200_dequantize(lyra_b200_ctx* ctx, int n, const uint8_t* packets, int num_bits, float* features) {
  if (!ctx || !features || !packets) return LYRA_B200_EINVAL;
  ENTER(0);
  if (!BitsOk(ctx, num_bits)) return LYRA_B200_EINVAL;
  int rc = CheckIds(ctx, nullptr, n, false);
  if (rc) return rc;
  CU(cudaMemcpyAsync(ctx->d_packets, packets, (size_t)PacketBytes(num_bits) * (size_t)n, cudaMemcpyHostToDevice, ctx->stream));
  const Part whole{0, 0, 0, n, ctx->stream};
  rc = LaunchDequantize(ctx, whole, ctx->d_packets, nullptr, num_bits, ctx->d_features);
  if (rc) return rc;
  CU(cudaMemcpyAsync(features, ctx->d_features, sizeof(float) * 64 * (size_t)n, cudaMemcpyDeviceToHost, ctx->stream));
  CU(SyncStream(ctx));
  return LYRA_B200_OK;
}

int lyra_b200_generate(lyra_b200_ctx* ctx, const int32_t* ids, int n, const float* features, int16_t* pcm) {
  if (!ctx || !features || !pcm) return LYRA_B200_EINVAL;
  ENTER(LYRA_B200_ROLE_DECODER);
  int rc = PrepareMap(ctx, ids, n);
  if (rc) return rc;
  CU(cudaMemcpyAsync(ctx->d_features, features, sizeof(float) * 64 * (size_t)n, cudaMemcpyHostToDevice, ctx->stream));
  if ((rc = LaunchDecoderNets(ctx, WholeCall(ctx, n), nullptr, ctx->d_features, ctx->d_pcm))) return rc;
  CU(cudaMemcpyAsync(pcm, ctx->d_pcm, sizeof(int16_t) * 320 * (size_t)n, cudaMemcpyDeviceToHost, ctx->stream));
  CU(SyncStream(ctx));
  return LYRA_B200_OK;
}

int lyra_b200_logmel(lyra_b200_ctx* ctx, int bank, const int32_t* ids, int n, const int16_t* pcm, int num_mel_bins, float* out) {
  if (!ctx || !pcm || !out) return LYRA_B200_EINVAL;
  ENTER(0);
  if (bank < 0 || bank > 1) { ctx->err = "log-mel bank must be 0 or 1"; return LYRA_B200_EINVAL; }
  if (num_mel_bins != 160 && num_mel_bins != 64) { ctx->err = "log-mel supports 160 or 64 mel bins"; return LYRA_B200_EINVAL; }
  const int* d_ids = nullptr;
  int rc = CheckIds(ctx, ids, n, false);
  if (rc || (rc = UploadIds(ctx, ids, n, &d_ids))) return rc;
  const LogMelParams& P = num_mel_bins == 160 ? ctx->spec.logmel160 : ctx->spec.logmel64;
  CU(cudaMemcpyAsync(ctx->d_pcm, pcm, sizeof(int16_t) * 320 * (size_t)n, cudaMemcpyHostToDevice, ctx->stream));
  if ((rc = LaunchLogMel(ctx, ctx->stream, Uniform(P), nullptr, 16000, d_ids, 0, n, n, ctx->d_pcm, ctx->d_logmel_prev[bank], nullptr)))
    return rc;
  CU(cudaMemcpyAsync(out, ctx->d_melout, sizeof(float) * (size_t)num_mel_bins * (size_t)n, cudaMemcpyDeviceToHost, ctx->stream));
  CU(SyncStream(ctx));
  return LYRA_B200_OK;
}

int lyra_b200_noise_update(lyra_b200_ctx* ctx, const int32_t* ids, int n, const int16_t* pcm, const uint8_t* update_mask,
                           uint8_t* is_noise, float* noise_estimate) {
  if (!ctx || !pcm) return LYRA_B200_EINVAL;
  ENTER(0);
  const int* d_ids = nullptr;
  int rc = CheckIds(ctx, ids, n, false);
  if (rc || (rc = UploadIds(ctx, ids, n, &d_ids))) return rc;
  CU(cudaMemcpyAsync(ctx->d_pcm, pcm, sizeof(int16_t) * 320 * (size_t)n, cudaMemcpyHostToDevice, ctx->stream));
  if (update_mask) CU(cudaMemcpyAsync(ctx->d_received, update_mask, (size_t)n, cudaMemcpyHostToDevice, ctx->stream));
  rc = LaunchNoiseUpdate(ctx, ctx->stream, d_ids, 0, n, n, ctx->d_pcm, update_mask ? ctx->d_received : nullptr,
                         is_noise ? ctx->d_is_noise : nullptr, noise_estimate ? ctx->d_noise_est : nullptr);
  if (rc) return rc;
  if (is_noise) CU(cudaMemcpyAsync(is_noise, ctx->d_is_noise, (size_t)n, cudaMemcpyDeviceToHost, ctx->stream));
  if (noise_estimate) CU(cudaMemcpyAsync(noise_estimate, ctx->d_noise_est, sizeof(float) * 160 * (size_t)n, cudaMemcpyDeviceToHost, ctx->stream));
  CU(SyncStream(ctx));
  return LYRA_B200_OK;
}

int lyra_b200_noise_update_device(lyra_b200_ctx* ctx, int n, const int16_t* d_pcm, const uint8_t* d_update_mask,
                                  uint8_t* d_is_noise, float* d_noise_estimate) {
  if (!ctx || !d_pcm) return LYRA_B200_EINVAL;
  ENTER(0);
  const int rc = CheckIds(ctx, nullptr, n, false);
  if (rc) return rc;
  return LaunchNoiseUpdate(ctx, ctx->stream, nullptr, 0, n, n, d_pcm, d_update_mask, d_is_noise, d_noise_estimate);
}

int lyra_b200_decode_track_noise(lyra_b200_ctx* ctx, const int32_t* ids, int n, const uint8_t* packets, const uint8_t* received,
                                 int num_bits, int16_t* pcm, uint8_t* is_noise) {
  if (!ctx || !packets || !pcm) return LYRA_B200_EINVAL;
  CodecCall c{kDecodeTrackNoise, n, num_bits, ids};
  c.host.packets_in = packets;
  c.host.received = received;
  c.host.pcm_out = pcm;
  c.host.flags = is_noise;
  return RunCodecCall(ctx, c);
}

int lyra_b200_decode_track_noise_device(lyra_b200_ctx* ctx, int n, const uint8_t* d_packets, const uint8_t* d_received, int num_bits,
                                        int16_t* d_pcm, uint8_t* d_is_noise) {
  if (!ctx || !d_packets || !d_pcm) return LYRA_B200_EINVAL;
  CodecCall c{kDecodeTrackNoise, n, num_bits};
  c.dev.packets_in = d_packets;
  c.dev.received = d_received;
  c.dev.pcm_out = d_pcm;
  c.dev.flags = d_is_noise;
  return RunCodecCall(ctx, c);
}

int lyra_b200_encode_dtx(lyra_b200_ctx* ctx, const int32_t* ids, int n, const int16_t* pcm, int num_bits, uint8_t* packets,
                         int32_t* packet_bytes) {
  if (!ctx || !pcm || !packets || !packet_bytes) return LYRA_B200_EINVAL;
  CodecCall c{kEncodeDtx, n, num_bits, ids};
  c.host.pcm_in = pcm;
  c.host.packets_out = packets;
  c.packet_bytes = packet_bytes;
  return RunCodecCall(ctx, c);
}

int lyra_b200_encode_dtx_device(lyra_b200_ctx* ctx, int n, const int16_t* d_pcm, int num_bits, uint8_t* d_packets, uint8_t* d_is_noise) {
  if (!ctx || !d_pcm || !d_packets || !d_is_noise) return LYRA_B200_EINVAL;
  CodecCall c{kEncodeDtx, n, num_bits};
  c.dev.pcm_in = d_pcm;
  c.dev.packets_out = d_packets;
  c.dev.flags = d_is_noise;
  return RunCodecCall(ctx, c);
}

int lyra_b200_decode_plc(lyra_b200_ctx* ctx, const int32_t* ids, int n, const uint8_t* packets, const uint8_t* received, int num_bits,
                         int16_t* pcm, uint8_t* is_comfort_noise) {
  if (!ctx || !packets || !pcm) return LYRA_B200_EINVAL;
  CodecCall c{kDecodePlc, n, num_bits, ids};
  c.host.packets_in = packets;
  c.host.received = received;
  c.host.pcm_out = pcm;
  c.host.flags = is_comfort_noise;
  return RunCodecCall(ctx, c);
}

int lyra_b200_decode_plc_device(lyra_b200_ctx* ctx, int n, const uint8_t* d_packets, const uint8_t* d_received, int num_bits,
                                int16_t* d_pcm, uint8_t* d_is_comfort_noise) {
  if (!ctx || !d_packets || !d_pcm) return LYRA_B200_EINVAL;
  CodecCall c{kDecodePlc, n, num_bits};
  c.dev.packets_in = d_packets;
  c.dev.received = d_received;
  c.dev.pcm_out = d_pcm;
  c.dev.flags = d_is_comfort_noise;
  return RunCodecCall(ctx, c);
}

int lyra_b200_plc_get_state(lyra_b200_ctx* ctx, const int32_t* ids, int n, int32_t* state) {
  if (!ctx || !state) return LYRA_B200_EINVAL;
  ENTER(0);
  const int rc = CheckIds(ctx, ids, n, true);
  if (rc) return rc;
  CU(SyncStream(ctx));
  for (int k = 0; k < n; ++k) {
    const int id = ids ? ids[k] : k;
    CU(cudaMemcpy(state + (size_t)k * 3, ctx->d_plc + (size_t)id * 4, sizeof(int) * 3, cudaMemcpyDeviceToHost));
  }
  return LYRA_B200_OK;
}

int lyra_b200_plc_set_state(lyra_b200_ctx* ctx, const int32_t* ids, int n, const int32_t* state) {
  if (!ctx || !state) return LYRA_B200_EINVAL;
  ENTER(0);
  const int rc = CheckIds(ctx, ids, n, true);
  if (rc) return rc;
  CU(SyncStream(ctx));
  for (int k = 0; k < n; ++k) {
    const int id = ids ? ids[k] : k;
    const int32_t* s3 = state + (size_t)k * 3;
    if (!PlcStateOk(s3[0], s3[1], s3[2])) {
      ctx->err = "decoder control state must be hop aligned: concealment 0..1280, fade 0..640, direction +-1";
      return LYRA_B200_EINVAL;
    }
    CU(cudaMemcpy(ctx->d_plc + (size_t)id * 4, s3, sizeof(int) * 3, cudaMemcpyHostToDevice));
  }
  return LYRA_B200_OK;
}

int lyra_b200_set_cng_seed(lyra_b200_ctx* ctx, uint64_t seed) {
  if (!ctx) return LYRA_B200_EINVAL;
  ctx->cng_seed = seed;
  return LYRA_B200_OK;
}

int lyra_b200_cng_generate(lyra_b200_ctx* ctx, const int32_t* ids, int n, const float* features, int16_t* pcm) {
  if (!ctx || !features || !pcm) return LYRA_B200_EINVAL;
  ENTER(0);
  const int* d_ids = nullptr;
  int rc = CheckIds(ctx, ids, n, false);
  if (rc || (rc = UploadIds(ctx, ids, n, &d_ids))) return rc;
  CU(cudaMemcpyAsync(ctx->d_cng_feat, features, sizeof(float) * 160 * (size_t)n, cudaMemcpyHostToDevice, ctx->stream));
  if ((rc = LaunchComfortNoise(ctx, ctx->stream, d_ids, 0, n, n, ctx->d_cng_feat, nullptr))) return rc;
  CU(cudaMemcpyAsync(pcm, ctx->d_cng_pcm, sizeof(int16_t) * 320 * (size_t)n, cudaMemcpyDeviceToHost, ctx->stream));
  CU(SyncStream(ctx));
  return LYRA_B200_OK;
}

int lyra_b200_resample(lyra_b200_ctx* ctx, int to_internal, const int32_t* ids, int n, int external_rate_hz, const int16_t* in,
                       int in_samples, int16_t* out, int out_stride, int32_t* out_counts) {
  if (!ctx || !in || !out) return LYRA_B200_EINVAL;
  ENTER(0);
  const int pair = RatePair(external_rate_hz);
  if (pair < 0) { ctx->err = "the resampler converts between 16 kHz and 8 / 32 / 48 kHz"; return LYRA_B200_EINVAL; }
  const int pr = to_internal ? pair : pair + 3;
  const int num = ctx->spec.resampler.num[pr], den = ctx->spec.resampler.den[pr];
  const int max_out = (in_samples * den + num - 1) / num;
  if (in_samples <= 0 || in_samples > 960 || max_out > 960 || out_stride < max_out || out_stride > 968) {
    ctx->err = "resample: at most 960 input and 960 output samples per stream and call, and room for ceil(n * out / in) outputs";
    return LYRA_B200_EINVAL;
  }
  const int* d_ids = nullptr;
  int rc = CheckIds(ctx, ids, n, false);
  if (rc || (rc = UploadIds(ctx, ids, n, &d_ids))) return rc;
  CU(cudaMemcpyAsync(ctx->d_rs_in, in, sizeof(int16_t) * (size_t)in_samples * (size_t)n, cudaMemcpyHostToDevice, ctx->stream));
  const int dir = to_internal ? 0 : 1;
  if ((rc = LAUNCH(kNoProf, ResampleKernel, dim3((unsigned)n), dim3(128), sizeof(float) * (size_t)(kResamplerTaps - 1 + in_samples),
                   ctx->stream, ctx->d_blob, ctx->spec.resampler, pr, external_rate_hz, d_ids, n, ctx->d_rs_in, in_samples, in_samples,
                   ctx->d_rs_out, out_stride, ctx->d_rs_counts, ctx->d_rs_delay[dir], ctx->d_rs_pos[dir], 0, nullptr, external_rate_hz)))
    return rc;
  CU(cudaMemcpyAsync(out, ctx->d_rs_out, sizeof(int16_t) * (size_t)out_stride * (size_t)n, cudaMemcpyDeviceToHost, ctx->stream));
  std::vector<int> counts((size_t)n);
  CU(cudaMemcpyAsync(counts.data(), ctx->d_rs_counts, sizeof(int) * (size_t)n, cudaMemcpyDeviceToHost, ctx->stream));
  CU(SyncStream(ctx));
  if (out_counts) for (int k = 0; k < n; ++k) out_counts[k] = counts[(size_t)k];
  return LYRA_B200_OK;
}

int lyra_b200_stream_state_bytes(const lyra_b200_ctx* ctx) { return ctx ? (int)RecordBytes(ctx) : 0; }

int lyra_b200_export_streams(lyra_b200_ctx* ctx, const int32_t* stream_ids, int n, void* records) {
  if (!ctx || !records) return LYRA_B200_EINVAL;
  ENTER(0);
  int rc = CheckIds(ctx, stream_ids, n, true);
  if (rc || (rc = EnsureRecordStaging(ctx))) return rc;
  ctx->state_table.header[kHdrRate] = (uint32_t)ctx->sample_rate;
  const size_t rb = RecordBytes(ctx);
  StreamIdChunk ids;
  for (int k0 = 0; k0 < n; k0 += ctx->records_chunk) {
    ids.n = n - k0 < ctx->records_chunk ? n - k0 : ctx->records_chunk;
    for (int k = 0; k < ids.n; ++k) ids.src[k] = stream_ids ? stream_ids[k0 + k] : k0 + k;
    if ((rc = LAUNCH(kNoProf, StreamStateGatherKernel, StateGrid(ctx->state_table, ids.n, 1), dim3(kStateThreads), (size_t)kStateSmemBytes,
                     ctx->stream, ctx->state_table, ids, ctx->d_records, ctx->codec_rs_tag)))
      return rc;
    CU(cudaMemcpyAsync(static_cast<uint8_t*>(records) + rb * (size_t)k0, ctx->d_records, rb * (size_t)ids.n, cudaMemcpyDeviceToHost, ctx->stream));
  }
  CU(SyncStream(ctx));
  return LYRA_B200_OK;
}

int lyra_b200_import_streams(lyra_b200_ctx* ctx, const int32_t* stream_ids, int n, const void* records) {
  if (!ctx || !records) return LYRA_B200_EINVAL;
  ENTER(0);
  int rc = CheckIds(ctx, stream_ids, n, false);
  if (rc) return rc;
  const size_t rb = RecordBytes(ctx);
  const uint8_t* recs = static_cast<const uint8_t*>(records);
  bool own_rate = false;
  for (int k = 0; k < n; ++k) {
    if (const char* why = RecordProblem(ctx, recs + rb * (size_t)k)) {
      ctx->err = "record " + std::to_string(k) + ": " + why;
      return LYRA_B200_EINVAL;
    }
    for (size_t i = 0; i < ctx->state_list.size(); ++i)
      if (ctx->state_list[i].check == lyra_b200_ctx::kCheckStreamRate)
        own_rate |= RecordWord(recs + rb * (size_t)k, kStateHeaderWords + ctx->state_list[i].e.offset) != 0;
  }
  if ((rc = EnsureRecordStaging(ctx))) return rc;
  if (own_rate) ctx->rate_override = true;
  for (size_t i = 0; i < ctx->state_list.size(); ++i) {
    const StreamStateEntry& e = ctx->state_list[i].e;
    for (int r = 0; r < 2; ++r)
      if (e.state == reinterpret_cast<uint32_t*>(ctx->d_stream_bits[r]))
        for (int k = 0; k < n; ++k)
          SetMirrorBits(ctx, r, stream_ids ? stream_ids[k] : k, (int32_t)RecordWord(recs + rb * (size_t)k, kStateHeaderWords + e.offset));
  }
  StreamIdChunk ids;
  for (int k0 = 0; k0 < n; k0 += ctx->records_chunk) {
    ids.n = n - k0 < ctx->records_chunk ? n - k0 : ctx->records_chunk;
    for (int k = 0; k < ids.n; ++k) ids.dst[k] = stream_ids ? stream_ids[k0 + k] : k0 + k;
    CU(cudaMemcpyAsync(ctx->d_records, recs + rb * (size_t)k0, rb * (size_t)ids.n, cudaMemcpyHostToDevice, ctx->stream));
    if ((rc = LAUNCH(kNoProf, StreamStateScatterKernel, StateGrid(ctx->state_table, ids.n, 0), dim3(kStateThreads), (size_t)kStateSmemBytes,
                     ctx->stream, ctx->state_table, ids, ctx->d_records, ctx->codec_rs_tag)))
      return rc;
  }
  CU(SyncStream(ctx));
  return LYRA_B200_OK;
}

int lyra_b200_copy_streams(lyra_b200_ctx* ctx, const int32_t* src_ids, const int32_t* dst_ids, int n) {
  if (!ctx || !src_ids || !dst_ids) return LYRA_B200_EINVAL;
  ENTER(0);
  int rc = CheckCopyIds(ctx, src_ids, dst_ids, n);
  if (rc || (rc = CopyStreamState(ctx, ctx->state_table, src_ids, dst_ids, n))) return rc;
  for (int r = 0; r < 2; ++r)
    for (int k = 0; k < n && ctx->d_stream_bits[r]; ++k)
      SetMirrorBits(ctx, r, dst_ids[k], src_ids[k] < 0 ? 0 : ctx->bits_mirror[r][(size_t)src_ids[k]]);
  return LYRA_B200_OK;
}

int lyra_b200_noise_estimate(lyra_b200_ctx* ctx, const int32_t* ids, int n, float* noise_estimate, uint8_t* is_noise) {
  if (!ctx || (!noise_estimate && !is_noise)) return LYRA_B200_EINVAL;
  ENTER(0);
  const int* d_ids = nullptr;
  int rc = CheckIds(ctx, ids, n, false);
  if (rc || (rc = UploadIds(ctx, ids, n, &d_ids))) return rc;
  if ((rc = LAUNCH(kNoProf, NoiseReadKernel, dim3((unsigned)n), dim3(192), (size_t)0, ctx->stream,
                   d_ids, n, ctx->d_noise, ctx->noise_params.nf, noise_estimate ? ctx->d_noise_est : nullptr, is_noise ? ctx->d_is_noise : nullptr)))
    return rc;
  if (noise_estimate) CU(cudaMemcpyAsync(noise_estimate, ctx->d_noise_est, sizeof(float) * 160 * (size_t)n, cudaMemcpyDeviceToHost, ctx->stream));
  if (is_noise) CU(cudaMemcpyAsync(is_noise, ctx->d_is_noise, (size_t)n, cudaMemcpyDeviceToHost, ctx->stream));
  CU(SyncStream(ctx));
  return LYRA_B200_OK;
}

}
```

lyra_b200/csrc/kernel_prims.cuh:

```cuda
#pragma once

#include "device_compat.h"
#include "net_params.h"

namespace lyra_b200 {

template <typename T>
__device__ __forceinline__ const T* BlobPtr(const uint8_t* blob, uint32_t off) {
  return reinterpret_cast<const T*>(blob + off);
}

__device__ __forceinline__ float LeakyRelu(float v) { return fmaxf(v, __fmul_rn(v, 0.3f)); }

__device__ __forceinline__ int QuantizeF32(float v, float scale, int zp) {
  int q = (int)roundf(__fdiv_rn(v, scale)) + zp;
  q = q < -128 ? -128 : (q > 127 ? 127 : q);
  return q;
}
__device__ __forceinline__ float DequantizeI8(int q, float scale, int zp) { return __fmul_rn(scale, (float)(q - zp)); }

__device__ __forceinline__ int Mbqm(int x, int qm, int shift) {
  const int left = shift > 0 ? shift : 0, right = shift > 0 ? 0 : -shift;
  const long long ab = (long long)(int)((unsigned)x << left) * (long long)qm;
  const int hi = (int)((ab + (1ll << 30)) >> 31);
  const int half = (int)((1u << right) >> 1);
  return right ? (hi + half + (hi >> 31)) >> right : hi;
}
__device__ __forceinline__ int ClampI8(int v) { return v < -128 ? -128 : (v > 127 ? 127 : v); }
__device__ __forceinline__ int RequantI8(int acc, int bias, int mult, int shift, int out_zp) {
  return ClampI8(Mbqm(acc + bias, mult, shift) + out_zp);
}
struct RequantP4 { int b[4], m[4], s[4]; };
__device__ __forceinline__ RequantP4 LoadRequant4(const int* __restrict__ bias, const int* __restrict__ mult, const int* __restrict__ shift, int n0) {
  const int4 b = *reinterpret_cast<const int4*>(bias + n0), m = *reinterpret_cast<const int4*>(mult + n0), s = *reinterpret_cast<const int4*>(shift + n0);
  return RequantP4{{b.x, b.y, b.z, b.w}, {m.x, m.y, m.z, m.w}, {s.x, s.y, s.z, s.w}};
}
__device__ __forceinline__ uint32_t PackI8x4(int a, int b, int c, int d) {
  return (uint32_t)(a & 0xff) | ((uint32_t)(b & 0xff) << 8) | ((uint32_t)(c & 0xff) << 16) | ((uint32_t)(d & 0xff) << 24);
}
__device__ __forceinline__ int UnpackI8(uint32_t w, int i) { return (int)(int8_t)((w >> (8 * i)) & 0xff); }

template <int NT, int U, typename T, typename LoadFn, typename StoreFn>
__device__ __forceinline__ void BatchedLoop(int n, LoadFn ld, StoreFn st) {
  for (int i0 = (int)threadIdx.x; i0 < n; i0 += NT * U) {
    T v[U];
#pragma unroll
    for (int k = 0; k < U; ++k) { const int i = i0 + k * NT; if (i < n) v[k] = ld(i); }
#pragma unroll
    for (int k = 0; k < U; ++k) { const int i = i0 + k * NT; if (i < n) st(i, v[k]); }
  }
}

constexpr int kStages = 3;
constexpr int kMaxStages = 8;

struct WeightPipe {
  LyraMbar full[2][kMaxStages];
  LyraMbar empty[2][kMaxStages];
  int cur;
};

__device__ __forceinline__ WeightPipe* GetWeightPipe() {
  LYRA_STATIC_SMEM(WeightPipe, pipe, 1);
  return pipe;
}

__device__ __forceinline__ void InitPipeSet(WeightPipe* pipe, int set, int nwarps) {
#pragma unroll
  for (int s = 0; s < kMaxStages; ++s) { lyra_mbar_init(&pipe->full[set][s], 1); lyra_mbar_init(&pipe->empty[set][s], (unsigned)nwarps); }
  lyra_mbar_fence_init();
}

template <int NT>
__device__ __forceinline__ void InitWeightPipe() {
  WeightPipe* pipe = GetWeightPipe();
  if (threadIdx.x == 0) {
    InitPipeSet(pipe, 0, NT / 32);
    InitPipeSet(pipe, 1, NT / 32);
    pipe->cur = 0;
  }
}

struct WNext {
  const void* w;
  int chunk_words;
  int nchunks;
  void* ring;
  int stages;
};
__device__ __forceinline__ WNext NoNext() { return WNext{nullptr, 0, 0, nullptr, kStages}; }
__device__ __forceinline__ WNext NextF32(const float* w, int KC, int N, int Ktot, void* ring = nullptr, int stages = kStages) {
  return WNext{w, KC * N, Ktot / KC, ring, stages};
}

__device__ __forceinline__ void IssuePrologueSet(WeightPipe* pipe, int set, void* wbuf, const void* w, int chunk_words, int nchunks,
                                                 int stages = kStages) {
#pragma unroll
  for (int p = 0; p < kMaxStages - 1; ++p)
    if (p < stages - 1 && p < nchunks)
      lyra_bulk_g2s(reinterpret_cast<uint32_t*>(wbuf) + (size_t)p * chunk_words,
                    reinterpret_cast<const uint32_t*>(w) + (size_t)p * chunk_words, (unsigned)chunk_words * 4u, &pipe->full[set][p]);
}

template <int NT>
__device__ __forceinline__ void IssuePrologue(void* wbuf_default, const WNext& nx) {
  if (nx.w == nullptr) return;
  lyra_fence_proxy_async();
  __syncthreads();
  if (threadIdx.x == 0) {
    WeightPipe* pipe = GetWeightPipe();
    IssuePrologueSet(pipe, pipe->cur, nx.ring ? nx.ring : wbuf_default, nx.w, nx.chunk_words, nx.nchunks, nx.stages);
  }
}

template <int WM>
struct TileMap {
  int MGB, NGB, nwt;
  __device__ __forceinline__ TileMap(int MG, int NG) {
    MGB = (MG + WM - 1) / WM;
    NGB = (NG + (32 / WM) - 1) / (32 / WM);
    nwt = MGB * NGB;
  }
  __device__ __forceinline__ bool Locate(int wt, int MG, int NG, int& mg, int& ng) const {
    const int lane = (int)threadIdx.x & 31;
    mg = (wt % MGB) * WM + lane % WM;
    ng = (wt / MGB) * (32 / WM) + lane / WM;
    return wt < nwt && mg < MG && ng < NG;
  }
};

template <int S, int NT, int TM, int TN, int KC, int WM, bool CIN1, int STG = kStages, typename Epi>
__device__ __forceinline__ void GemmF32Tap(const float* A, int ldA, int rowA0, int row_stride, int ntaps, int CinG,
                                           int groups, int T_out, int N, const float* __restrict__ Wg, float* wbuf,
                                           bool pre, const WNext& nxt, Epi epi) {
  static_assert(S % TM == 0 && TM % 4 == 0 && 32 % WM == 0, "tile shape");
  constexpr int MGS = S / TM;
  const int MG = T_out * MGS, NG = N / TN;
  const TileMap<WM> map(MG, NG);
  const int Ktot = ntaps * CinG, nchunks = Ktot / KC;
  const int CoutG = N / groups;
  const int warp = (int)threadIdx.x >> 5, lane = (int)threadIdx.x & 31;
  WeightPipe* pipe = GetWeightPipe();
  const int set = pipe->cur;
  const int npass = (map.nwt + NT / 32 - 1) / (NT / 32);
  const int total = npass * nchunks;
  const unsigned chunk_bytes = (unsigned)(KC * N) * 4u;
  static_assert(STG >= 2 && STG <= kMaxStages, "ring depth");
  if (nchunks < STG - 1) LYRA_TRAP();
  if (threadIdx.x == 0) {
    InitPipeSet(pipe, set ^ 1, NT / 32);
    if (!pre) IssuePrologueSet(pipe, set, wbuf, Wg, KC * N, nchunks, STG);
  }
  int cg = 0;
  for (int wt0 = 0; wt0 < map.nwt; wt0 += NT / 32) {
    int mg, ng;
    const bool active = map.Locate(wt0 + warp, MG, NG, mg, ng);
    const int nbusy = min(NT / 32, map.nwt - wt0);
    const bool busy = warp < nbusy;
    const int t_out = active ? mg / MGS : 0, s0 = active ? (mg % MGS) * TM : 0, n0 = active ? ng * TN : 0;
    const int g = n0 / CoutG;
    const float* Abase = A + (size_t)(g * CinG) * ldA + (rowA0 + t_out * row_stride) * S + s0;
    float acc[TM][TN];
#pragma unroll
    for (int i = 0; i < TM; ++i)
#pragma unroll
      for (int j = 0; j < TN; ++j) acc[i][j] = 0.0f;

    if (!busy) cg += nchunks;
    for (int c = 0; busy && c < nchunks; ++c, ++cg) {
      if (threadIdx.x == 0) {
        const int ci = cg + STG - 1;
        if (ci < total) {
          const int si = ci % STG;
          if (ci >= STG) lyra_mbar_wait(&pipe->empty[set][si], (unsigned)((ci / STG - 1) & 1));
          lyra_bulk_g2s(wbuf + (size_t)si * (KC * N), Wg + (size_t)(ci % nchunks) * KC * N, chunk_bytes, &pipe->full[set][si]);
        }
      }
      const int st = cg % STG;
      lyra_mbar_wait(&pipe->full[set][st], (unsigned)((cg / STG) & 1));
      if (active) {
        const float* wcur = wbuf + (size_t)st * (KC * N);
        const int kk0 = c * KC;
        const float* Ap;
        int astep;
        if (CIN1) { Ap = Abase + (kk0 + (kk0 >> 4)) * S; astep = S; }
        else { const int tap = kk0 / CinG, ci0 = kk0 - tap * CinG; Ap = Abase + (size_t)ci0 * ldA + tap * S; astep = ldA; }
        const float* wp = wcur + n0;
#pragma unroll 4
        for (int kk = 0; kk < KC; ++kk) {
          float a[TM];
          float w[TN];
#pragma unroll
          for (int i = 0; i < TM; i += 4) {
            const float4 v = *reinterpret_cast<const float4*>(Ap + i);
            a[i] = v.x; a[i + 1] = v.y; a[i + 2] = v.z; a[i + 3] = v.w;
          }
          if (TN % 4 == 0) {
#pragma unroll
            for (int j = 0; j + 3 < TN; j += 4) {
              const float4 v = *reinterpret_cast<const float4*>(wp + j);
              w[j] = v.x; w[j + 1] = v.y; w[j + 2] = v.z; w[j + 3] = v.w;
            }
          } else if (TN % 2 == 0) {
#pragma unroll
            for (int j = 0; j + 1 < TN; j += 2) {
              const float2 v = *reinterpret_cast<const float2*>(wp + j);
              w[j] = v.x; w[j + 1] = v.y;
            }
          } else {
#pragma unroll
            for (int j = 0; j < TN; ++j) w[j] = wp[j];
          }
#pragma unroll
          for (int j = 0; j < TN; ++j)
#pragma unroll
            for (int i = 0; i < TM; ++i) acc[i][j] = __fmaf_rn(a[i], w[j], acc[i][j]);
          Ap += astep;
          wp += N;
        }
      }
      __syncwarp();
      if (lane == 0) {
        if (warp == 0 && nbusy < NT / 32) lyra_mbar_arrive_n(&pipe->empty[set][st], (unsigned)(1 + NT / 32 - nbusy));
        else lyra_mbar_arrive(&pipe->empty[set][st]);
      }
    }
    lyra_fence_proxy_async();
    __syncthreads();
    if (wt0 + NT / 32 >= map.nwt && threadIdx.x == 0) {
      if (nxt.w != nullptr) IssuePrologueSet(pipe, set ^ 1, nxt.ring ? nxt.ring : wbuf, nxt.w, nxt.chunk_words, nxt.nchunks, nxt.stages);
      pipe->cur = set ^ 1;
    }
    if (active) epi(t_out, s0, n0, acc);
  }
  __syncthreads();
}

constexpr int kI8Pd = 2;
template <int S, int NT, int NTW, int PDI = kI8Pd, typename Epi>
__device__ __forceinline__ void GemmI8Mma(const uint32_t* A, int ldA, int rowA0, int row_stride, int ntaps, int CinG,
                                          int groups, int T_out, int N, const uint2* __restrict__ Wf, Epi epi) {
  constexpr int PD = PDI;
  const int lane = (int)threadIdx.x & 31, warp = (int)threadIdx.x >> 5, g = lane >> 2, t4 = lane & 3;
  const int M = T_out * S, MT = (M + 15) / 16, NTILES = N / 8, NWT = MT * (NTILES / NTW);
  const int CinG4 = CinG / 4, KS = ntaps * CinG4 / 8, CoutG = N / groups;
  for (int wt = warp; wt < NWT; wt += NT / 32) {
    const int mt = wt % MT, nt0 = (wt / MT) * NTW;
    const int m0 = mt * 16 + g, m1 = m0 + 8;
    const bool valid0 = m0 < M, valid1 = m1 < M;
    const int tr0 = valid0 ? m0 / S : T_out - 1, tr1 = valid1 ? m1 / S : T_out - 1;
    const int s0 = m0 % S, s1 = m1 % S;
    const int grp = (nt0 * 8) / CoutG;
    const uint32_t* pa0 = A + (size_t)(grp * CinG4) * ldA + (rowA0 + tr0 * row_stride) * S + s0;
    const uint32_t* pa1 = A + (size_t)(grp * CinG4) * ldA + (rowA0 + tr1 * row_stride) * S + s1;
    const uint2* wp = Wf + (size_t)nt0 * 32 + lane;
    const size_t ks_stride = (size_t)NTILES * 32;
    int acc[NTW][4];
#pragma unroll
    for (int j = 0; j < NTW; ++j) { acc[j][0] = 0; acc[j][1] = 0; acc[j][2] = 0; acc[j][3] = 0; }
    uint2 bf[PD][NTW];
#pragma unroll
    for (int p = 0; p < PD; ++p)
      if (p < KS) {
#pragma unroll
        for (int j = 0; j < NTW; ++j) bf[p][j] = __ldg(wp + p * ks_stride + j * 32);
      }
    for (int ks0 = 0; ks0 < KS; ks0 += PD) {
#pragma unroll
      for (int p = 0; p < PD; ++p) {
        const int ks = ks0 + p;
        if (ks < KS) {
          const int kw = ks * 8, tap = kw / CinG4, kw0 = kw - tap * CinG4;
          const size_t off = (size_t)(kw0 + t4) * ldA + tap * S;
          uint32_t a[4];
          a[0] = pa0[off]; a[1] = pa1[off]; a[2] = pa0[off + 4 * (size_t)ldA]; a[3] = pa1[off + 4 * (size_t)ldA];
#pragma unroll
          for (int j = 0; j < NTW; ++j) {
            const uint32_t b[2] = {bf[p][j].x, bf[p][j].y};
            lyra_mma_s8_16x8x32(acc[j], a, b);
          }
          if (ks + PD < KS) {
#pragma unroll
            for (int j = 0; j < NTW; ++j) bf[p][j] = __ldg(wp + (size_t)(ks + PD) * ks_stride + j * 32);
          }
        }
      }
    }
    const bool even = (t4 & 1) == 0;
#pragma unroll
    for (int j = 0; j < NTW; ++j) {
      const int r0 = __shfl_xor_sync(0xffffffffu, even ? acc[j][2] : acc[j][0], 1);
      const int r1 = __shfl_xor_sync(0xffffffffu, even ? acc[j][3] : acc[j][1], 1);
      int out[1][4];
      if (even) { out[0][0] = acc[j][0]; out[0][1] = acc[j][1]; out[0][2] = r0; out[0][3] = r1; }
      else { out[0][0] = r0; out[0][1] = r1; out[0][2] = acc[j][2]; out[0][3] = acc[j][3]; }
      const int n4 = (nt0 + j) * 8 + (t4 >> 1) * 4;
      if (even ? valid0 : valid1) epi(even ? tr0 : tr1, even ? s0 : s1, n4, out);
    }
  }
  __syncthreads();
}

__host__ __device__ constexpr int PadLd(int x) {
  while (!(x % 4 == 0 && (x % 32 == 8 || x % 32 == 24))) ++x;
  return x;
}

__device__ __forceinline__ void SplitTf32(float x, uint32_t& hi, uint32_t& lo) {
  hi = __float_as_uint(x) & 0xffffe000u;
  lo = __float_as_uint(__fsub_rn(x, __uint_as_float(hi)));
}

template <int S, int NT, int WTM, int WTN, bool SYNC_EPI, typename Epi>
__device__ __forceinline__ void GemmTf32Mma(const float* A, int ldA, int rowA0, int row_stride, int ntaps, int CinG,
                                            int groups, int T_out, int N, const float2* __restrict__ Wf, Epi epi) {
  constexpr int PD = 8;
  constexpr int NW = NT / 32;
  const int lane = (int)threadIdx.x & 31, warp = (int)threadIdx.x >> 5, g = lane >> 2, t4 = lane & 3;
  const int M = T_out * S, MT = (M + 15) / 16, MTW = (MT + WTM - 1) / WTM, NTILES = N / 8, NWT = MTW * (NTILES / WTN);
  const int KS = ntaps * CinG / 8, CoutG = N / groups;
  const size_t ks_stride = (size_t)NTILES * 32;
  float acc[WTM][WTN][4];
  int tr[WTM][2], sr[WTM][2];
  bool vr[WTM][2];
  int nt0 = 0;

  auto kloop = [&](int wt) {
    const int mtb = (wt % MTW) * WTM;
    nt0 = (wt / MTW) * WTN;
    const int grp = (nt0 * 8) / CoutG;
    const float* pa[WTM][2];
#pragma unroll
    for (int i = 0; i < WTM; ++i)
#pragma unroll
      for (int h = 0; h < 2; ++h) {
        const int m = (mtb + i) * 16 + g + 8 * h;
        vr[i][h] = m < M;
        tr[i][h] = vr[i][h] ? m / S : T_out - 1;
        sr[i][h] = m % S;
        pa[i][h] = A + (size_t)(grp * CinG) * ldA + (rowA0 + tr[i][h] * row_stride) * S + sr[i][h];
      }
#pragma unroll
    for (int i = 0; i < WTM; ++i)
#pragma unroll
      for (int j = 0; j < WTN; ++j) { acc[i][j][0] = 0.0f; acc[i][j][1] = 0.0f; acc[i][j][2] = 0.0f; acc[i][j][3] = 0.0f; }
    const float2* wp = Wf + (size_t)nt0 * 32 + lane;
    float2 bf[PD][WTN];
#pragma unroll
    for (int p = 0; p < PD; ++p)
      if (p < KS) {
#pragma unroll
        for (int j = 0; j < WTN; ++j) bf[p][j] = __ldg(wp + p * ks_stride + j * 32);
      }
    for (int ks0 = 0; ks0 < KS; ks0 += PD) {
#pragma unroll
      for (int p = 0; p < PD; ++p) {
        const int ks = ks0 + p;
        if (ks < KS) {
          const int k0 = ks * 8, tap = k0 / CinG, c0 = k0 - tap * CinG;
          const size_t off = (size_t)(c0 + t4) * ldA + tap * S, off4 = off + 4 * (size_t)ldA;
          uint32_t ahi[WTM][4], alo[WTM][4];
#pragma unroll
          for (int i = 0; i < WTM; ++i) {
            SplitTf32(pa[i][0][off], ahi[i][0], alo[i][0]);
            SplitTf32(pa[i][1][off], ahi[i][1], alo[i][1]);
            SplitTf32(pa[i][0][off4], ahi[i][2], alo[i][2]);
            SplitTf32(pa[i][1][off4], ahi[i][3], alo[i][3]);
          }
#pragma unroll
          for (int j = 0; j < WTN; ++j) {
            uint32_t bhi[2], blo[2];
            SplitTf32(bf[p][j].x, bhi[0], blo[0]);
            SplitTf32(bf[p][j].y, bhi[1], blo[1]);
#pragma unroll
            for (int i = 0; i < WTM; ++i) {
              lyra_mma_tf32_16x8x8(acc[i][j], alo[i], bhi);
              lyra_mma_tf32_16x8x8(acc[i][j], ahi[i], blo);
              lyra_mma_tf32_16x8x8(acc[i][j], ahi[i], bhi);
            }
          }
          if (ks + PD < KS) {
#pragma unroll
            for (int j = 0; j < WTN; ++j) bf[p][j] = __ldg(wp + (size_t)(ks + PD) * ks_stride + j * 32);
          }
        }
      }
    }
  };
  auto epilogue = [&]() {
#pragma unroll
    for (int i = 0; i < WTM; ++i)
#pragma unroll
      for (int h = 0; h < 2; ++h)
        if (vr[i][h]) {
#pragma unroll
          for (int j = 0; j < WTN; ++j) {
            float o[1][2] = {{acc[i][j][2 * h], acc[i][j][2 * h + 1]}};
            epi(tr[i][h], sr[i][h], (nt0 + j) * 8 + 2 * t4, o);
          }
        }
  };
  if (SYNC_EPI) {
    if (NWT > NW) LYRA_TRAP();
    const bool has = warp < NWT;
    if (has) kloop(warp);
    __syncthreads();
    if (has) epilogue();
  } else {
    for (int wt = warp; wt < NWT; wt += NW) {
      kloop(wt);
      epilogue();
    }
  }
  __syncthreads();
}

__device__ __forceinline__ int RingSlot(int base, int t, int R) {
  int v = (base + t) % R;
  return v < 0 ? v + R : v;
}

__device__ __forceinline__ float4 LeakyRelu4(float4 v) {
  return make_float4(LeakyRelu(v.x), LeakyRelu(v.y), LeakyRelu(v.z), LeakyRelu(v.w));
}

template <int S, int NT, int C, int T, int DIL>
__device__ __forceinline__ void DwF32RingFast(const float* u, int ldu, int row0u, float* dout, int ldd,
                                              const float* __restrict__ w, const float* __restrict__ bias,
                                              float* __restrict__ ring, int n18u, const int* active) {
  constexpr int R = 2 * DIL, Q = S / 4;
  const int base = (n18u * T) % R;
  for (int item = (int)threadIdx.x; item < C * Q; item += NT) {
    const int c = item / Q, s4 = (item % Q) * 4;
    float* rc = ring + (size_t)c * R * S + s4;
    float4 rg[R];
#pragma unroll
    for (int j = 0; j < R; ++j) rg[j] = *reinterpret_cast<const float4*>(rc + ((base + j) % R) * S);
    const float w0 = w[c], w1 = w[C + c], w2 = w[2 * C + c], b = bias[c];
    const float* uc = u + (size_t)c * ldu + row0u * S + s4;
    float* dc = dout + (size_t)c * ldd + s4;
#pragma unroll
    for (int t = 0; t < T; ++t) {
      const float4 x2 = LeakyRelu4(*reinterpret_cast<const float4*>(uc + t * S));
      float4 x1, x0;
      if (t - DIL >= 0) x1 = LeakyRelu4(*reinterpret_cast<const float4*>(uc + (t - DIL) * S));
      else x1 = rg[(t - DIL + R) % R];
      if (t - 2 * DIL >= 0) x0 = LeakyRelu4(*reinterpret_cast<const float4*>(uc + (t - 2 * DIL) * S));
      else x0 = rg[(t - 2 * DIL + R) % R];
      float4 o;
      o.x = __fadd_rn(__fmaf_rn(x2.x, w2, __fmaf_rn(x1.x, w1, __fmaf_rn(x0.x, w0, 0.0f))), b);
      o.y = __fadd_rn(__fmaf_rn(x2.y, w2, __fmaf_rn(x1.y, w1, __fmaf_rn(x0.y, w0, 0.0f))), b);
      o.z = __fadd_rn(__fmaf_rn(x2.z, w2, __fmaf_rn(x1.z, w1, __fmaf_rn(x0.z, w0, 0.0f))), b);
      o.w = __fadd_rn(__fmaf_rn(x2.w, w2, __fmaf_rn(x1.w, w1, __fmaf_rn(x0.w, w0, 0.0f))), b);
      *reinterpret_cast<float4*>(dc + t * S) = o;
    }
    constexpr int TF = T > R ? T - R : 0;
    const bool all4 = active[s4] && active[s4 + 1] && active[s4 + 2] && active[s4 + 3];
#pragma unroll
    for (int t = TF; t < T; ++t) {
      const float4 a = LeakyRelu4(*reinterpret_cast<const float4*>(uc + t * S));
      float* dst = rc + ((base + t) % R) * S;
      if (all4) {
        *reinterpret_cast<float4*>(dst) = a;
      } else {
        if (active[s4]) dst[0] = a.x;
        if (active[s4 + 1]) dst[1] = a.y;
        if (active[s4 + 2]) dst[2] = a.z;
        if (active[s4 + 3]) dst[3] = a.w;
      }
    }
  }
  __syncthreads();
}

template <int S, int NT, int C, int T, int DIL>
__device__ __forceinline__ void DwI8RingFast(const uint32_t* aq, int lda, int row0a, uint32_t* dq, int ldd,
                                             const uint8_t* blob, const DwI8& p, uint32_t* __restrict__ ring, int n18u,
                                             const int* active) {
  constexpr int R = 2 * DIL, C4 = C / 4;
  const int base = (n18u * T) % R;
  const int* w = BlobPtr<int>(blob, p.w);
  const int* bias = BlobPtr<int>(blob, p.bias);
  const int* mult = BlobPtr<int>(blob, p.mult);
  const int* shift = BlobPtr<int>(blob, p.shift);
  for (int item = (int)threadIdx.x; item < C4 * S; item += NT) {
    const int c4 = item / S, s = item % S;
    uint32_t* rc = ring + (size_t)c4 * R * S + s;
    const uint32_t* ac = aq + (size_t)c4 * lda + row0a * S + s;
    uint32_t x0[T], x1[T], x2[T];
#pragma unroll
    for (int t = 0; t < T; ++t) {
      x2[t] = ac[t * S];
      x1[t] = t - DIL >= 0 ? ac[(t - DIL) * S] : rc[((base + t - DIL + 2 * R) % R) * S];
      x0[t] = t - 2 * DIL >= 0 ? ac[(t - 2 * DIL) * S] : rc[((base + t - 2 * DIL + 2 * R) % R) * S];
    }
    int wk[3][4], bb[4], mm[4], sh[4];
#pragma unroll
    for (int b = 0; b < 4; ++b) {
      const int c = c4 * 4 + b;
      wk[0][b] = w[c]; wk[1][b] = w[C + c]; wk[2][b] = w[2 * C + c];
      bb[b] = bias[c]; mm[b] = mult[c]; sh[b] = shift[c];
    }
#pragma unroll
    for (int t = 0; t < T; ++t) {
      int q[4];
#pragma unroll
      for (int b = 0; b < 4; ++b) {
        const int acc = UnpackI8(x0[t], b) * wk[0][b] + UnpackI8(x1[t], b) * wk[1][b] + UnpackI8(x2[t], b) * wk[2][b];
        q[b] = RequantI8(acc, bb[b], mm[b], sh[b], p.out_zp);
      }
      dq[(size_t)c4 * ldd + t * S + s] = PackI8x4(q[0], q[1], q[2], q[3]);
    }
    constexpr int TF = T > R ? T - R : 0;
    if (active[s]) {
#pragma unroll
      for (int t = TF; t < T; ++t) rc[((base + t) % R) * S] = x2[t];
    }
  }
  __syncthreads();
}

template <int S, int NT>
__device__ __forceinline__ void DwF32Ring(const float* u, int ldu, int row0u, float* dout, int ldd, int C, int T, int dil,
                                          const float* __restrict__ w, const float* __restrict__ bias,
                                          float* __restrict__ ring, const int* n18, const int* active) {
  const int R = 2 * dil;
  const int total = C * T * S;
  for (int idx = (int)threadIdx.x; idx < total; idx += NT) {
    const int s = idx % S, t = (idx / S) % T, c = idx / (S * T);
    const int base = (n18[s] * T) % R;
    const float* uc = u + (size_t)c * ldu + row0u * S + s;
    const float x2 = LeakyRelu(uc[t * S]);
    const float x1 = t - dil >= 0 ? LeakyRelu(uc[(t - dil) * S]) : ring[((size_t)c * R + RingSlot(base, t - dil, R)) * S + s];
    const float x0 = t - 2 * dil >= 0 ? LeakyRelu(uc[(t - 2 * dil) * S]) : ring[((size_t)c * R + RingSlot(base, t - 2 * dil, R)) * S + s];
    float acc = __fmaf_rn(x0, w[c], 0.0f);
    acc = __fmaf_rn(x1, w[C + c], acc);
    acc = __fmaf_rn(x2, w[2 * C + c], acc);
    dout[(size_t)c * ldd + t * S + s] = __fadd_rn(acc, bias[c]);
  }
  __syncthreads();
  const int tfirst = T > R ? T - R : 0;
  const int nrows = T - tfirst;
  const int wtotal = C * nrows * S;
  for (int idx = (int)threadIdx.x; idx < wtotal; idx += NT) {
    const int s = idx % S, t = tfirst + (idx / S) % nrows, c = idx / (S * nrows);
    if (!active[s]) continue;
    const int base = (n18[s] * T) % R;
    ring[((size_t)c * R + RingSlot(base, t, R)) * S + s] = LeakyRelu(u[(size_t)c * ldu + (row0u + t) * S + s]);
  }
  __syncthreads();
}

template <int S, int NT>
__device__ __forceinline__ void DwI8Ring(const uint32_t* aq, int lda, int row0a, uint32_t* dq, int ldd, int C, int T, int dil,
                                         const uint8_t* blob, const DwI8& p, uint32_t* __restrict__ ring, const int* n18,
                                         const int* active) {
  const int R = 2 * dil, C4 = C / 4;
  const int* w = BlobPtr<int>(blob, p.w);
  const int* bias = BlobPtr<int>(blob, p.bias);
  const int* mult = BlobPtr<int>(blob, p.mult);
  const int* shift = BlobPtr<int>(blob, p.shift);
  const int total = C4 * T * S;
  for (int idx = (int)threadIdx.x; idx < total; idx += NT) {
    const int s = idx % S, t = (idx / S) % T, c4 = idx / (S * T);
    const int base = (n18[s] * T) % R;
    const uint32_t* ac = aq + (size_t)c4 * lda + row0a * S + s;
    const uint32_t x2 = ac[t * S];
    const uint32_t x1 = t - dil >= 0 ? ac[(t - dil) * S] : ring[((size_t)c4 * R + RingSlot(base, t - dil, R)) * S + s];
    const uint32_t x0 = t - 2 * dil >= 0 ? ac[(t - 2 * dil) * S] : ring[((size_t)c4 * R + RingSlot(base, t - 2 * dil, R)) * S + s];
    int o[4];
#pragma unroll
    for (int b = 0; b < 4; ++b) {
      const int c = c4 * 4 + b;
      const int acc = UnpackI8(x0, b) * w[c] + UnpackI8(x1, b) * w[C + c] + UnpackI8(x2, b) * w[2 * C + c];
      o[b] = RequantI8(acc, bias[c], mult[c], shift[c], p.out_zp);
    }
    dq[(size_t)c4 * ldd + t * S + s] = PackI8x4(o[0], o[1], o[2], o[3]);
  }
  __syncthreads();
  const int tfirst = T > R ? T - R : 0;
  const int nrows = T - tfirst;
  const int wtotal = C4 * nrows * S;
  for (int idx = (int)threadIdx.x; idx < wtotal; idx += NT) {
    const int s = idx % S, t = tfirst + (idx / S) % nrows, c4 = idx / (S * nrows);
    if (!active[s]) continue;
    const int base = (n18[s] * T) % R;
    ring[((size_t)c4 * R + RingSlot(base, t, R)) * S + s] = aq[(size_t)c4 * lda + (row0a + t) * S + s];
  }
  __syncthreads();
}

}
```

lyra_b200/csrc/net_kernels.cuh:

```cuda
#pragma once

#include <type_traits>

#include "kernel_prims.cuh"

namespace lyra_b200 {

constexpr int kTileStreams = 8;

struct EncStateA {
  static constexpr int kFirst = 0;
  static constexpr int kRing0 = 48, kRing1 = kRing0 + 64 * 2, kRing2 = kRing1 + 64 * 6;
  static constexpr int kDown0 = kRing2 + 64 * 18;
  static constexpr int kUnits = kDown0 + 64 * 5;
};
struct EncStateB {
  static constexpr int kRing0 = 0, kRing1 = 128 * 2, kRing2 = kRing1 + 128 * 6;
  static constexpr int kDown1 = kRing2 + 128 * 18;
  static constexpr int kRingM = kDown1 + 128 * 2;
  static constexpr int kRingQ0 = kRingM + 256 * 2;
  static constexpr int kRingQ1 = kRingQ0 + 64 * 6;
  static constexpr int kDown2 = kRingQ1 + 64 * 18;
  static constexpr int kBott = kDown2 + 64 * 2;
  static constexpr int kUnits = kBott + 128 * 2;
};
struct DecStateC {
  static constexpr int kBott = 0;
  static constexpr int kUp0 = 128;
  static constexpr int kUp1 = kUp0 + 512;
  static constexpr int kRing0 = kUp1 + 256, kRing1 = kRing0 + 128 * 2, kRing2 = kRing1 + 128 * 6;
  static constexpr int kRingM = kRing2 + 128 * 18;
  static constexpr int kRingQ0 = kRingM + 64 * 2;
  static constexpr int kRingQ1 = kRingQ0 + 64 * 6;
  static constexpr int kUnits = kRingQ1 + 64 * 18;
};
struct DecStateD {
  static constexpr int kUp2 = 0;
  static constexpr int kRing0 = 320, kRing1 = kRing0 + 64 * 2, kRing2 = kRing1 + 64 * 6;
  static constexpr int kLast = kRing2 + 64 * 18;
  static constexpr int kUnits = kLast + 48;
};

struct TileIo {
  const int* tile_list;
  const int* slot_of_stream;
  const uint8_t* skip;
};

template <int S>
__device__ __forceinline__ void LoadTileMeta(const TileIo& io, const int* n18_global, int* slot, int* active, int* n18, int& tile) {
  tile = io.tile_list[blockIdx.x];
  if ((int)threadIdx.x < S) {
    const int stream = tile * S + (int)threadIdx.x;
    const int sl = io.slot_of_stream[stream];
    slot[threadIdx.x] = sl;
    active[threadIdx.x] = sl >= 0 && !(io.skip != nullptr && io.skip[sl]);
    n18[threadIdx.x] = n18_global[stream];
  }
  __syncthreads();
  if (threadIdx.x == 0) {
    int u = -2;
    for (int s = 0; s < S; ++s)
      if (active[s]) u = (u == -2 || u == n18[s]) ? n18[s] : -1;
    n18[S] = u;
  }
  __syncthreads();
}
constexpr int kTileIdle = -2;

constexpr int kMax(int a, int b) { return a > b ? a : b; }

__device__ __forceinline__ void PrefetchTileState(const void* p, int bytes) {
  if (threadIdx.x == 0) lyra_prefetch_l2(p, (unsigned)bytes);
}

template <int S>
__device__ __forceinline__ bool BeginTile(const TileIo& io, const int* n18g, int* meta, float* state, int units, int& tile) {
  LoadTileMeta<S>(io, n18g, meta, meta + S, meta + 2 * S, tile);
  if (meta[3 * S] == kTileIdle) return false;
  PrefetchTileState(state + (size_t)tile * units * S, units * S * 4);
  return true;
}

template <int S>
__device__ __forceinline__ void AdvanceHopCounters(int* n18g, int tile, const int* active, const int* n18) {
  const int tid = (int)threadIdx.x;
  if (tid < S && active[tid]) n18g[tile * S + tid] = (n18[tid] + 1) % 18;
}

template <int S, int NT, int C, int R, typename T>
__device__ __forceinline__ void StoreCarriedRows(T* st, int unit, const T* buf, int ld, int row0, const int* active) {
  for (int i = (int)threadIdx.x; i < C * R * S; i += NT) {
    const int c = i / (R * S), r = i % (R * S);
    if (active[r % S]) st[unit * S + i] = buf[(size_t)c * ld + row0 * S + r];
  }
}

template <int S, int NT, int TM, int TN1, int TN2, int WM, int KC, int C, int T, int DIL, bool TC = false, int LDD = T * S,
          int WTM = 1, int WTN = 1, int STG = kStages>
__device__ __forceinline__ void ResUnitF32(const uint8_t* blob, const ResF32& p, float* u, int ldu, int row0u, float* d,
                                           int groups2, float* ring, const int* n18,
                                           const int* active, float* wbuf, bool last, const WNext& after, int dil_rt = DIL) {
  constexpr int ldd = LDD;
  if (n18[S] >= 0) {
    auto dw = [&](auto dil) {
      DwF32RingFast<S, NT, C, T, decltype(dil)::value>(u, ldu, row0u, d, ldd, BlobPtr<float>(blob, p.dw.w), BlobPtr<float>(blob, p.dw.bias), ring, n18[S], active);
    };
    if constexpr (DIL != 0) dw(std::integral_constant<int, DIL>());
    else if (dil_rt == 1) dw(std::integral_constant<int, 1>());
    else if (dil_rt == 3) dw(std::integral_constant<int, 3>());
    else dw(std::integral_constant<int, 9>());
  } else {
    DwF32Ring<S, NT>(u, ldu, row0u, d, ldd, C, T, dil_rt, BlobPtr<float>(blob, p.dw.w), BlobPtr<float>(blob, p.dw.bias), ring, n18, active);
  }
  {
    const float* b1 = BlobPtr<float>(blob, p.pw1.bias);
    auto epi1 = [&](int t, int s0, int n0, auto& acc) {
      constexpr int TMx = sizeof(acc) / sizeof(acc[0]), TNx = sizeof(acc[0]) / sizeof(float);
#pragma unroll
      for (int j = 0; j < TNx; ++j) {
        const float b = b1[n0 + j];
        float* o = d + (size_t)(n0 + j) * ldd + t * S + s0;
#pragma unroll
        for (int i = 0; i < TMx; ++i) o[i] = LeakyRelu(__fadd_rn(acc[i][j], b));
      }
    };
    if constexpr (TC)
      GemmTf32Mma<S, NT, WTM, WTN, true>(d, ldd, 0, 1, 1, C, 1, T, C, BlobPtr<float2>(blob, p.pw1.wf), epi1);
    else
      GemmF32Tap<S, NT, TM, TN1, KC, WM, false, STG>(d, ldd, 0, 1, 1, C, 1, T, C, BlobPtr<float>(blob, p.pw1.w), wbuf, true,
                                                     NextF32(BlobPtr<float>(blob, p.pw2.w), KC, C, C / groups2, nullptr, STG), epi1);
  }
  {
    const float* b2 = BlobPtr<float>(blob, p.pw2.bias);
    auto epi2 = [&](int t, int s0, int n0, auto& acc) {
      constexpr int TMx = sizeof(acc) / sizeof(acc[0]), TNx = sizeof(acc[0]) / sizeof(float);
#pragma unroll
      for (int j = 0; j < TNx; ++j) {
        const float b = b2[n0 + j];
        float* o = u + (size_t)(n0 + j) * ldu + (row0u + t) * S + s0;
#pragma unroll
        for (int i = 0; i < TMx; ++i) {
          const float v = __fadd_rn(__fadd_rn(acc[i][j], b), o[i]);
          o[i] = last ? LeakyRelu(v) : v;
        }
      }
    };
    if constexpr (TC)
      GemmTf32Mma<S, NT, WTM, WTN, false>(d, ldd, 0, 1, 1, C / groups2, groups2, T, C, BlobPtr<float2>(blob, p.pw2.wf), epi2);
    else
      GemmF32Tap<S, NT, TM, TN2, KC, WM, false, STG>(d, ldd, 0, 1, 1, C / groups2, groups2, T, C, BlobPtr<float>(blob, p.pw2.w), wbuf, true, after, epi2);
  }
}

template <int S, int NT, int TM, int TN1, int TN2, int WM, int KC, int C, int T, bool TC = false, int LDD = T * S, int WTM = 1, int WTN = 1,
          int STG = kStages>
__device__ __forceinline__ void ResUnitsF32x3(const uint8_t* blob, const ResF32* p3, float* u, int ldu, int row0u, float* d, int groups2,
                                              float* ring0, const int* n18, const int* active, float* wbuf, const WNext& after) {
#pragma unroll 1
  for (int i = 0; i < 3; ++i) {
    const ResF32& p = p3[i];
    const int dil = i == 0 ? 1 : (i == 1 ? 3 : 9);
    float* ring = ring0 + (size_t)(i == 0 ? 0 : (i == 1 ? 2 : 8)) * C * S;
    const WNext nx = i < 2 ? NextF32(BlobPtr<float>(blob, p3[i + 1].pw1.w), KC, C, C, nullptr, STG) : after;
    ResUnitF32<S, NT, TM, TN1, TN2, WM, KC, C, T, 0, TC, LDD, WTM, WTN, STG>(blob, p, u, ldu, row0u, d, groups2, ring, n18, active, wbuf, i == 2, nx,
                                                                       dil);
  }
}

struct RequantLutPack {
  const int* bias;
  const int* mult;
  const int* shift;
  const int8_t* lut;
  int out_zp;
  __device__ __forceinline__ RequantLutPack(const uint8_t* blob, const GemmI8& g, const LReluQ& lr)
      : bias(BlobPtr<int>(blob, g.bias)), mult(BlobPtr<int>(blob, g.mult)), shift(BlobPtr<int>(blob, g.shift)),
        lut(BlobPtr<int8_t>(blob, lr.lut)), out_zp(g.out_zp) {}
  __device__ __forceinline__ uint32_t operator()(const int (&acc)[1][4], int n0) const {
    const RequantP4 rq = LoadRequant4(bias, mult, shift, n0);
    int q[4];
#pragma unroll
    for (int j = 0; j < 4; ++j) q[j] = lut[RequantI8(acc[0][j], rq.b[j], rq.m[j], rq.s[j], out_zp) + 128];
    return PackI8x4(q[0], q[1], q[2], q[3]);
  }
};

template <int S, int NT, int PDI, typename Params>
__device__ __forceinline__ void MixedUnitPw2I8(const uint8_t* blob, const Params& P, const uint32_t* hq, const float* u,
                                               uint32_t* resq, uint32_t* aq, int lda, int row0a) {
  constexpr int LQ2 = PadLd(2 * S), LD2 = 2 * S;
  const int* bias = BlobPtr<int>(blob, P.m_pw2.bias);
  const int* mult = BlobPtr<int>(blob, P.m_pw2.mult);
  const int* shift = BlobPtr<int>(blob, P.m_pw2.shift);
  const int8_t* lut = BlobPtr<int8_t>(blob, P.m_lr2.lut);
  const QuantP dq = P.m_dq, q2 = P.m_q2;
  const int out_zp = P.m_pw2.out_zp;
  GemmI8Mma<S, NT, 4, PDI>(hq, LQ2, 0, 1, 1, 64, 4, 2, 256, BlobPtr<uint2>(blob, P.m_pw2.w),
    [&](int t, int s, int n0, int (&acc)[1][4]) {
      const RequantP4 rq = LoadRequant4(bias, mult, shift, n0);
      int r[4], a[4];
#pragma unroll
      for (int j = 0; j < 4; ++j) {
        const int q = RequantI8(acc[0][j], rq.b[j], rq.m[j], rq.s[j], out_zp);
        const float v = __fadd_rn(DequantizeI8(q, dq.scale, dq.zp), u[(size_t)(n0 + j) * LD2 + t * S + s]);
        r[j] = QuantizeF32(v, q2.scale, q2.zp);
        a[j] = lut[r[j] + 128];
      }
      resq[(size_t)(n0 / 4) * LQ2 + t * S + s] = PackI8x4(r[0], r[1], r[2], r[3]);
      aq[(size_t)(n0 / 4) * lda + (row0a + t) * S + s] = PackI8x4(a[0], a[1], a[2], a[3]);
    });
}

template <int S, int NT, int DIL, int PDI = kI8Pd>
__device__ __forceinline__ void ResUnitI8(const uint8_t* blob, const ResI8& p, uint32_t* aq, int lda, int row0a,
                                          uint32_t* resq, uint32_t* dq8, uint32_t* hq, uint32_t* ring,
                                          const int* n18, const int* active, int dil_rt = DIL) {
  constexpr int T = 2, C = 256, LD = PadLd(T * S);
  constexpr int NTW = 4;
  if (n18[S] >= 0) {
    if constexpr (DIL != 0) DwI8RingFast<S, NT, C, T, DIL>(aq, lda, row0a, dq8, LD, blob, p.dw, ring, n18[S], active);
    else if (dil_rt == 3) DwI8RingFast<S, NT, C, T, 3>(aq, lda, row0a, dq8, LD, blob, p.dw, ring, n18[S], active);
    else DwI8RingFast<S, NT, C, T, 9>(aq, lda, row0a, dq8, LD, blob, p.dw, ring, n18[S], active);
  } else {
    DwI8Ring<S, NT>(aq, lda, row0a, dq8, LD, C, T, dil_rt, blob, p.dw, ring, n18, active);
  }
  {
    const RequantLutPack epi(blob, p.pw1, p.lr1);
    GemmI8Mma<S, NT, NTW, PDI>(dq8, LD, 0, 1, 1, C, 1, T, C, BlobPtr<uint2>(blob, p.pw1.w),
      [&](int t, int s, int n0, int (&acc)[1][4]) { hq[(size_t)(n0 / 4) * LD + t * S + s] = epi(acc, n0); });
  }
  {
    const int* bias = BlobPtr<int>(blob, p.pw2.bias);
    const int* mult = BlobPtr<int>(blob, p.pw2.mult);
    const int* shift = BlobPtr<int>(blob, p.pw2.shift);
    const int* l1 = BlobPtr<int>(blob, p.add.lut1);
    const int* l2 = BlobPtr<int>(blob, p.add.lut2);
    const int8_t* lut = BlobPtr<int8_t>(blob, p.lr2.lut);
    const int out_zp = p.pw2.out_zp, m3 = p.add.m3, s3 = p.add.s3, add_zp = p.add.out_zp;
    GemmI8Mma<S, NT, NTW, PDI>(hq, LD, 0, 1, 1, C / 4, 4, T, C, BlobPtr<uint2>(blob, p.pw2.w),
      [&](int t, int s, int n0, int (&acc)[1][4]) {
        const RequantP4 rq = LoadRequant4(bias, mult, shift, n0);
        const size_t ro = (size_t)(n0 / 4) * LD + t * S + s;
        const uint32_t rw = resq[ro];
        int r[4], a[4];
#pragma unroll
        for (int j = 0; j < 4; ++j) {
          const int q = RequantI8(acc[0][j], rq.b[j], rq.m[j], rq.s[j], out_zp);
          r[j] = ClampI8(Mbqm(l1[q + 128] + l2[UnpackI8(rw, j) + 128], m3, s3) + add_zp);
          a[j] = lut[r[j] + 128];
        }
        resq[ro] = PackI8x4(r[0], r[1], r[2], r[3]);
        aq[(size_t)(n0 / 4) * lda + (row0a + t) * S + s] = PackI8x4(a[0], a[1], a[2], a[3]);
      });
  }
}

template <int S, int NT, int PDI = kI8Pd>
__device__ __forceinline__ void ResUnitsI8x2(const uint8_t* blob, const ResI8* p2, uint32_t* aq, int lda, int row0a,
                                             uint32_t* resq, uint32_t* dq8, uint32_t* hq, uint32_t* ring0,
                                             const int* n18, const int* active) {
#pragma unroll 1
  for (int i = 0; i < 2; ++i)
    ResUnitI8<S, NT, 0, PDI>(blob, p2[i], aq, lda, row0a, resq, dq8, hq, ring0 + (size_t)(i ? 64 * 6 : 0) * S, n18, active, i ? 9 : 3);
}

struct EncA {
  static constexpr int S = kTileStreams;
  static constexpr int NT = 320;
  static constexpr int TN = 4;
  static constexpr int kMinBlocks = 2;
  static constexpr int LDU = 25 * S, LDD = 20 * S;
  static constexpr int kStgDown = 5;
  static constexpr int DTM = 8, DTN = 4;
  static constexpr int kSmemU = 0;
  static constexpr int kSmemD = kSmemU + 64 * LDU * 4;
  static constexpr int kSmemW = kSmemD + 64 * LDD * 4;
  static constexpr int kSmemI = kSmemW + kStages * 16 * 64 * 4;
  static constexpr int kSmemBytes = kSmemI + 3 * S * 4 + 16;
  static_assert(391 * S <= 64 * LDD, "first-layer input (368 rows + 23 skew rows) must fit in the d buffer");
};

__global__ void __launch_bounds__(EncA::NT, EncA::kMinBlocks)
EncoderKernelA(const uint8_t* __restrict__ blob, EncoderParams P, TileIo io, const int16_t* __restrict__ pcm,
               float* __restrict__ state, int* __restrict__ n18g, float* __restrict__ mid) {
  using L = EncA;
  constexpr int S = L::S, NT = L::NT;
  unsigned char* smem = LYRA_DYN_SMEM();
  float* u = reinterpret_cast<float*>(smem + L::kSmemU);
  float* d = reinterpret_cast<float*>(smem + L::kSmemD);
  float* wbuf = reinterpret_cast<float*>(smem + L::kSmemW);
  int* slot = reinterpret_cast<int*>(smem + L::kSmemI);
  int* active = slot + S;
  int* n18 = active + S;
  int tile;
  InitWeightPipe<NT>();
  if (!BeginTile<S>(io, n18g, slot, state, EncStateA::kUnits, tile)) return;
  float* st = state + (size_t)tile * EncStateA::kUnits * S;
  const int tid = (int)threadIdx.x;
  IssuePrologue<NT>(wbuf, NextF32(BlobPtr<float>(blob, P.first.w), 16, 64, 64));

  float* X = d;
  BatchedLoop<NT, 2, float>(48 * S, [&](int i) { return st[EncStateA::kFirst * S + i]; },
                            [&](int i, float v) { const int r = i / S; X[(r + (r >> 4)) * S + i % S] = v; });
  BatchedLoop<NT, 8, float>(320 * S,
    [&](int i) { const int s = i / 320, k = i % 320; return active[s] ? (float)pcm[(size_t)slot[s] * 320 + k] * (1.0f / 32768.0f) : 0.0f; },
    [&](int i, float v) { const int s = i / 320, k = i % 320; X[(48 + k + ((48 + k) >> 4)) * S + s] = v; });
  BatchedLoop<NT, 8, float>(64 * 5 * S, [&](int i) { return st[EncStateA::kDown0 * S + i]; },
                            [&](int i, float v) { const int c = i / (5 * S), r = i % (5 * S); u[(size_t)c * L::LDU + r] = v; });
  __syncthreads();
  for (int i = tid; i < 48 * S; i += NT)
    if (active[i % S]) { const int r = 320 + i / S; st[EncStateA::kFirst * S + i] = X[(r + (r >> 4)) * S + i % S]; }
  {
    const float* b = BlobPtr<float>(blob, P.first.bias);
    GemmF32Tap<S, NT, 8, L::TN, 16, 4, true>(X, 0, 0, 17, 64, 1, 1, 20, 64, BlobPtr<float>(blob, P.first.w), wbuf, true,
      NextF32(BlobPtr<float>(blob, P.r0[0].pw1.w), 16, 64, 64),
      [&](int t, int s0, int n0, float (&acc)[8][L::TN]) {
#pragma unroll
        for (int j = 0; j < L::TN; ++j) {
          float* o = u + (size_t)(n0 + j) * L::LDU + (5 + t) * S + s0;
#pragma unroll
          for (int i = 0; i < 8; ++i) o[i] = __fadd_rn(acc[i][j], b[n0 + j]);
        }
      });
  }
  static_assert(EncStateA::kRing1 == EncStateA::kRing0 + 64 * 2 && EncStateA::kRing2 == EncStateA::kRing1 + 64 * 6, "ring blocks back to back");
  ResUnitsF32x3<S, NT, 8, L::TN, L::TN, 4, 16, 64, 20>(blob, P.r0, u, L::LDU, 5, d, 1, st + (size_t)EncStateA::kRing0 * S, n18, active, wbuf,
                                                       NextF32(BlobPtr<float>(blob, P.down0.w), 16, 128, 640, d, L::kStgDown));
  StoreCarriedRows<S, NT, 64, 5>(st, EncStateA::kDown0, u, L::LDU, 20, active);
  {
    const float* b = BlobPtr<float>(blob, P.down0.bias);
    float* out = mid + (size_t)tile * 128 * 4 * S;
    static_assert(L::kStgDown * 16 * 128 * 4 <= 64 * L::LDD * 4, "simpleconv weight ring must fit in d");
    constexpr int DTM = L::DTM, DTN = L::DTN;
    GemmF32Tap<S, NT, DTM, DTN, 16, 4, false, L::kStgDown>(u, L::LDU, 0, 5, 10, 64, 1, 4, 128, BlobPtr<float>(blob, P.down0.w), d, true, NoNext(),
      [&](int t, int s0, int n0, float (&acc)[DTM][DTN]) {
#pragma unroll
        for (int j = 0; j < DTN; ++j) {
          float* o = out + ((size_t)(n0 + j) * 4 + t) * S + s0;
#pragma unroll
          for (int i = 0; i < DTM; ++i) o[i] = __fadd_rn(acc[i][j], b[n0 + j]);
        }
      });
  }
  AdvanceHopCounters<S>(n18g, tile, active, n18);
}

struct EncB {
  static constexpr int S = kTileStreams;
  static constexpr int NT = 256;
  static constexpr int kMinBlocks = 3;
  static constexpr int TM = 8;
  static constexpr int TN = 4;
  static constexpr int WM4 = 4 * S / TM >= 4 ? 4 : 4 * S / TM;
  static constexpr int WM2 = 2 * S / TM >= 4 ? 4 : 2 * S / TM;
  static constexpr int WM1 = 1 * S / TM >= 4 ? 4 : 1 * S / TM;
  static constexpr int LD1 = 6 * S;
  static constexpr int LQ2 = PadLd(2 * S), LQA = PadLd(4 * S), LQB = PadLd(3 * S);
  static constexpr int kRA = 0;
  static constexpr int kRABytes = kMax(kMax(128 * LD1 * 4, 256 * 2 * S * 4), 64 * LQA * 4 + 128 * LQB * 4);
  static constexpr int kRB = kRA + kRABytes;
  static constexpr int kRBBytes = kMax(128 * 4 * S * 4, 256 * 2 * S * 4);
  static constexpr int kRC = kRB + kRBBytes;
  static constexpr int kW = kRC + 64 * LQ2 * 4;
  static constexpr int kStg = 3;
  static constexpr int kWBytes = kMax(kStg * 8 * 256 * 4, 2 * 64 * LQ2 * 4);
  static constexpr int kI8Pd = 4;
  static constexpr int kI = kW + kWBytes;
  static constexpr int kSmemBytes = kI + 3 * S * 4 + 16;
};

__global__ void __launch_bounds__(EncB::NT, EncB::kMinBlocks)
EncoderKernelB(const uint8_t* __restrict__ blob, EncoderParams P, TileIo io, const float* __restrict__ mid,
               float* __restrict__ state, int* __restrict__ n18g, float* __restrict__ features) {
  using L = EncB;
  constexpr int S = L::S, NT = L::NT;
  constexpr int TM = L::TM, TN = L::TN;
  unsigned char* smem = LYRA_DYN_SMEM();
  constexpr int LQ2 = L::LQ2, LQA = L::LQA, LQB = L::LQB;
  float* u1 = reinterpret_cast<float*>(smem + L::kRA);
  float* d2 = reinterpret_cast<float*>(smem + L::kRA);
  uint32_t* aq = reinterpret_cast<uint32_t*>(smem + L::kRA);
  uint32_t* bq = aq + 64 * LQA;
  float* d1 = reinterpret_cast<float*>(smem + L::kRB);
  float* u2 = reinterpret_cast<float*>(smem + L::kRB);
  uint32_t* hq = reinterpret_cast<uint32_t*>(smem + L::kRC);
  float* wbuf = reinterpret_cast<float*>(smem + L::kW);
  uint32_t* dq8 = reinterpret_cast<uint32_t*>(smem + L::kW);
  uint32_t* resq = dq8 + 64 * LQ2;
  int* slot = reinterpret_cast<int*>(smem + L::kI);
  int* active = slot + S;
  int* n18 = active + S;
  int tile;
  InitWeightPipe<NT>();
  if (!BeginTile<S>(io, n18g, slot, state, EncStateB::kUnits, tile)) return;
  float* st = state + (size_t)tile * EncStateB::kUnits * S;
  uint32_t* stw = reinterpret_cast<uint32_t*>(st);
  IssuePrologue<NT>(wbuf, NextF32(BlobPtr<float>(blob, P.r1[0].pw1.w), 16, 128, 128, nullptr, L::kStg));

  {
    const float* in = mid + (size_t)tile * 128 * 4 * S;
    BatchedLoop<NT, 4, float4>(128 * S, [&](int i) { return reinterpret_cast<const float4*>(in)[i]; },
      [&](int i, float4 v) { const int c = i / S, r = (i % S) * 4; *reinterpret_cast<float4*>(u1 + (size_t)c * L::LD1 + 2 * S + r) = v; });
    BatchedLoop<NT, 8, float>(128 * 2 * S, [&](int i) { return st[EncStateB::kDown1 * S + i]; },
      [&](int i, float v) { const int c = i / (2 * S), r = i % (2 * S); u1[(size_t)c * L::LD1 + r] = v; });
  }
  __syncthreads();
  static_assert(EncStateB::kRing1 == EncStateB::kRing0 + 128 * 2 && EncStateB::kRing2 == EncStateB::kRing1 + 128 * 6, "ring blocks back to back");
  ResUnitsF32x3<S, NT, TM, TN, TN, L::WM4, 16, 128, 4, false, 4 * S, 1, 1, L::kStg>(
      blob, P.r1, u1, L::LD1, 2, d1, 2, st + (size_t)EncStateB::kRing0 * S, n18, active, wbuf,
      NextF32(BlobPtr<float>(blob, P.down1.w), 8, 256, 256, wbuf, L::kStg));
  StoreCarriedRows<S, NT, 128, 2>(st, EncStateB::kDown1, u1, L::LD1, 4, active);
  {
    const float* b = BlobPtr<float>(blob, P.down1.bias);
    GemmF32Tap<S, NT, TM, TN, 8, L::WM2, false, L::kStg>(u1, L::LD1, 0, 2, 4, 64, 2, 2, 256, BlobPtr<float>(blob, P.down1.w), wbuf, true,
      NextF32(BlobPtr<float>(blob, P.m_pw1.w), 8, 256, 256, wbuf, L::kStg),
      [&](int t, int s0, int n0, float (&acc)[TM][TN]) {
#pragma unroll
        for (int j = 0; j < TN; ++j) {
          float* o = u2 + (size_t)(n0 + j) * 2 * S + t * S + s0;
#pragma unroll
          for (int i = 0; i < TM; ++i) o[i] = __fadd_rn(acc[i][j], b[n0 + j]);
        }
      });
  }
  constexpr int LD2 = 2 * S;
  if (n18[S] >= 0)
    DwF32RingFast<S, NT, 256, 2, 1>(u2, LD2, 0, d2, LD2, BlobPtr<float>(blob, P.m_dw.w), BlobPtr<float>(blob, P.m_dw.bias),
                                    st + (size_t)EncStateB::kRingM * S, n18[S], active);
  else
    DwF32Ring<S, NT>(u2, LD2, 0, d2, LD2, 256, 2, 1, BlobPtr<float>(blob, P.m_dw.w), BlobPtr<float>(blob, P.m_dw.bias),
                     st + (size_t)EncStateB::kRingM * S, n18, active);
  {
    const float* b = BlobPtr<float>(blob, P.m_pw1.bias);
    const int8_t* lut = BlobPtr<int8_t>(blob, P.m_lr1.lut);
    const QuantP q1 = P.m_q1;
    static_assert(TN == 4, "the epilogue packs one word of four channels per (row, stream)");
    GemmF32Tap<S, NT, TM, TN, 8, L::WM2, false, L::kStg>(d2, LD2, 0, 1, 1, 256, 1, 2, 256, BlobPtr<float>(blob, P.m_pw1.w), wbuf, true,
      NoNext(),
      [&](int t, int s0, int n0, float (&acc)[TM][TN]) {
#pragma unroll
        for (int i = 0; i < TM; ++i) {
          int q[TN];
#pragma unroll
          for (int j = 0; j < TN; ++j) q[j] = lut[QuantizeF32(__fadd_rn(acc[i][j], b[n0 + j]), q1.scale, q1.zp) + 128];
          hq[(size_t)(n0 / 4) * LQ2 + t * S + s0 + i] = PackI8x4(q[0], q[1], q[2], q[3]);
        }
      });
  }
  MixedUnitPw2I8<S, NT, L::kI8Pd>(blob, P, hq, u2, resq, aq, LQA, 2);
  static_assert(EncStateB::kRingQ1 == EncStateB::kRingQ0 + 64 * 6, "ring blocks back to back");
  ResUnitsI8x2<S, NT, L::kI8Pd>(blob, P.q, aq, LQA, 2, resq, dq8, hq, stw + (size_t)EncStateB::kRingQ0 * S, n18, active);
  BatchedLoop<NT, 4, uint32_t>(64 * 2 * S, [&](int i) { return stw[EncStateB::kDown2 * S + i]; },
    [&](int i, uint32_t v) { const int c = i / (2 * S), r = i % (2 * S); aq[(size_t)c * LQA + r] = v; });
  BatchedLoop<NT, 8, uint32_t>(128 * 2 * S, [&](int i) { return stw[EncStateB::kBott * S + i]; },
    [&](int i, uint32_t v) { const int c = i / (2 * S), r = i % (2 * S); bq[(size_t)c * LQB + r] = v; });
  __syncthreads();
  StoreCarriedRows<S, NT, 64, 2>(stw, EncStateB::kDown2, aq, LQA, 2, active);
  {
    const RequantLutPack epi(blob, P.down2, P.down2_lr);
    GemmI8Mma<S, NT, 8, L::kI8Pd>(aq, LQA, 0, 2, 4, 64, 4, 1, 512, BlobPtr<uint2>(blob, P.down2.w),
      [&](int, int s, int n0, int (&acc)[1][4]) { bq[(size_t)(n0 / 4) * LQB + 2 * S + s] = epi(acc, n0); });
  }
  StoreCarriedRows<S, NT, 128, 2>(stw, EncStateB::kBott, bq, LQB, 1, active);
  {
    const int* bias = BlobPtr<int>(blob, P.bott.bias);
    const int* mult = BlobPtr<int>(blob, P.bott.mult);
    const int* shift = BlobPtr<int>(blob, P.bott.shift);
    const QuantP dq = P.out_dq;
    const int out_zp = P.bott.out_zp;
    GemmI8Mma<S, NT, 1, L::kI8Pd>(bq, LQB, 0, 1, 3, 128, 4, 1, 64, BlobPtr<uint2>(blob, P.bott.w),
      [&](int t, int s, int n0, int (&acc)[1][4]) {
        const RequantP4 rq = LoadRequant4(bias, mult, shift, n0);
        (void)t;
        if (!active[s]) return;
        float* o = features + (size_t)slot[s] * 64 + n0;
#pragma unroll
        for (int j = 0; j < 4; ++j)
          o[j] = DequantizeI8(RequantI8(acc[0][j], rq.b[j], rq.m[j], rq.s[j], out_zp), dq.scale, dq.zp);
      });
  }
  AdvanceHopCounters<S>(n18g, tile, active, n18);
}

template <bool TC = false>
struct DecC {
  static constexpr int S = kTileStreams;
  static constexpr int NT = 256;
  static constexpr int kMinBlocks = 3;
  static constexpr int kI8Pd = 2;
  static constexpr int TM = 8;
  static constexpr int TN = 4;
  static constexpr int WM4 = 4 * S / TM >= 4 ? 4 : 4 * S / TM;
  static constexpr int WM2 = 2 * S / TM >= 4 ? 4 : 2 * S / TM;
  static constexpr int WM1 = 1 * S / TM >= 4 ? 4 : 1 * S / TM;
  static constexpr int LQ2 = PadLd(2 * S), LQA = PadLd(4 * S), LQB = PadLd(3 * S);
  static constexpr int kF = 0;
  static constexpr int kXq = kF + 64 * 3 * S * 4;
  static constexpr int LD1 = TC ? PadLd(4 * S) : 4 * S;
  static constexpr int RWM = 2, RWN = 2;
  static_assert(!TC || ((4 * S + 31) / 32) * (16 / RWN) <= NT / 32, "decoder_1: one warp tile per warp");
  static constexpr int kR1Bytes = kMax(kMax(64 * 3 * S * 4 + 128 * LQB * 4, 64 * LQA * 4), 128 * LD1 * 4);
  static constexpr int kU = kF + kR1Bytes;
  static constexpr int kW = kU + 256 * 2 * S * 4;
  static constexpr int kWBytes = kMax(kStages * 4 * 512 * 4, 3 * 64 * LQ2 * 4);
  static constexpr int kI = kW + kWBytes;
  static constexpr int kSmemBytes = kI + 3 * S * 4 + 16;
};

template <bool TC>
__global__ void __launch_bounds__(DecC<TC>::NT, DecC<TC>::kMinBlocks)
DecoderKernelC(const uint8_t* __restrict__ blob, DecoderParams P, TileIo io,
               const float* __restrict__ features, float* __restrict__ state, int* __restrict__ n18g,
               float* __restrict__ mid) {
  using L = DecC<TC>;
  constexpr int S = L::S, NT = L::NT;
  constexpr int TM = L::TM, TN = L::TN;
  unsigned char* smem = LYRA_DYN_SMEM();
  float* F = reinterpret_cast<float*>(smem + L::kF);
  uint32_t* xq = reinterpret_cast<uint32_t*>(smem + L::kXq);
  float* u = reinterpret_cast<float*>(smem + L::kU);
  float* u1 = u;
  constexpr int LQ2 = L::LQ2, LQA = L::LQA, LQB = L::LQB;
  uint32_t* aq = reinterpret_cast<uint32_t*>(smem + L::kF);
  float* d1 = reinterpret_cast<float*>(smem + L::kF);
  float* wbuf = reinterpret_cast<float*>(smem + L::kW);
  uint32_t* hq = reinterpret_cast<uint32_t*>(smem + L::kW);
  uint32_t* dq8 = hq + 64 * LQ2;
  uint32_t* resq = dq8 + 64 * LQ2;
  int* slot = reinterpret_cast<int*>(smem + L::kI);
  int* active = slot + S;
  int* n18 = active + S;
  int tile;
  InitWeightPipe<NT>();
  if (!BeginTile<S>(io, n18g, slot, state, DecStateC::kUnits, tile)) return;
  uint32_t* stw = reinterpret_cast<uint32_t*>(state) + (size_t)tile * DecStateC::kUnits * S;
  float* st = reinterpret_cast<float*>(stw);
  const int tid = (int)threadIdx.x;
  constexpr int LD2 = 2 * S;
  const UpI8& up0 = P.up0;
  const UpI8& up1 = P.up1;
  IssuePrologue<NT>(wbuf, NextF32(BlobPtr<float>(blob, P.bott.w), 4, 512, 48));

  BatchedLoop<NT, 4, float>(64 * 2 * S, [&](int i) { return st[DecStateC::kBott * S + i]; },
    [&](int i, float v) { const int c = i / (2 * S), r = i % (2 * S); F[(size_t)c * 3 * S + r] = v; });
  BatchedLoop<NT, 2, float>(64 * S, [&](int i) { const int s = i / 64, c = i % 64; return active[s] ? features[(size_t)slot[s] * 64 + c] : 0.0f; },
    [&](int i, float v) { const int s = i / 64, c = i % 64; F[(size_t)c * 3 * S + 2 * S + s] = v; });
  BatchedLoop<NT, 4, float4>(256 * 2 * S / 4, [&](int i) { return reinterpret_cast<const float4*>(st + (size_t)DecStateC::kUp0 * S)[i]; },
    [&](int i, float4 v) { reinterpret_cast<float4*>(u)[i] = v; });
  {
    const uint32_t pad = PackI8x4(P.bott_q.zp, P.bott_q.zp, P.bott_q.zp, P.bott_q.zp);
    for (int i = tid; i < 128 * S; i += NT) { const int c = i / S, s = i % S; xq[(size_t)c * LQB + s] = pad; xq[(size_t)c * LQB + 2 * S + s] = pad; }
  }
  __syncthreads();
  StoreCarriedRows<S, NT, 64, 2>(st, DecStateC::kBott, F, 3 * S, 1, active);
  {
    const float* b = BlobPtr<float>(blob, P.bott.bias);
    const QuantP q = P.bott_q;
    GemmF32Tap<S, NT, TM, 4, 4, L::WM1, false>(F, 3 * S, 0, 1, 3, 16, 4, 1, 512, BlobPtr<float>(blob, P.bott.w), wbuf, true,
      NoNext(),
      [&](int t, int s0, int n0, float (&acc)[TM][4]) {
        (void)t;
#pragma unroll
        for (int i = 0; i < TM; ++i) {
          int v[4];
#pragma unroll
          for (int j = 0; j < 4; ++j) v[j] = QuantizeF32(LeakyRelu(__fadd_rn(acc[i][j], b[n0 + j])), q.scale, q.zp);
          xq[(size_t)(n0 / 4) * LQB + S + s0 + i] = PackI8x4(v[0], v[1], v[2], v[3]);
        }
      });
  }
  {
    const int* bias = BlobPtr<int>(blob, up0.g.bias);
    const int* mult = BlobPtr<int>(blob, up0.g.mult);
    const int* shift = BlobPtr<int>(blob, up0.g.shift);
    float* tail = st + (size_t)DecStateC::kUp0 * S;
    GemmI8Mma<S, NT, 8>(xq, LQB, 0, 1, 2, 128, 4, 2, 512, BlobPtr<uint2>(blob, up0.g.w),
      [&](int q, int s, int n0, int (&acc)[1][4]) {
        const RequantP4 rq = LoadRequant4(bias, mult, shift, n0);
        const int g = n0 / 128, r = (n0 % 128) / 64;
        const float* bf = BlobPtr<float>(blob, up0.bias_f32[g]);
#pragma unroll
        for (int j = 0; j < 4; ++j) {
          const int co = (n0 + j) % 64, ch = g * 64 + co;
          const int qv = RequantI8(acc[0][j], rq.b[j], rq.m[j], rq.s[j], up0.out_zp[g]);
          const float f = DequantizeI8(qv, up0.dq[g].scale, up0.dq[g].zp);
          if (q == 0) {
            float* o = u + (size_t)ch * LD2 + r * S + s;
            *o = __fadd_rn(f, *o);
          } else if (active[s]) {
            tail[((size_t)ch * 2 + r) * S + s] = __fsub_rn(__fadd_rn(f, 0.0f), bf[co]);
          }
        }
      });
  }
  {
    const QuantP q = P.up0_q;
    for (int i = tid; i < 64 * 2 * S; i += NT) {
      const int c4 = i / (2 * S), r = i % (2 * S);
      int v[4];
#pragma unroll
      for (int b = 0; b < 4; ++b) v[b] = QuantizeF32(LeakyRelu(u[(size_t)(c4 * 4 + b) * LD2 + r]), q.scale, q.zp);
      aq[(size_t)c4 * LQA + S + r] = PackI8x4(v[0], v[1], v[2], v[3]);
    }
  }
  __syncthreads();
  if (n18[S] >= 0) DwI8RingFast<S, NT, 256, 2, 1>(aq, LQA, 1, dq8, LQ2, blob, P.m_dw, stw + (size_t)DecStateC::kRingM * S, n18[S], active);
  else DwI8Ring<S, NT>(aq, LQA, 1, dq8, LQ2, 256, 2, 1, blob, P.m_dw, stw + (size_t)DecStateC::kRingM * S, n18, active);
  {
    const RequantLutPack epi(blob, P.m_pw1, P.m_lr1);
    GemmI8Mma<S, NT, 4, L::kI8Pd>(dq8, LQ2, 0, 1, 1, 256, 1, 2, 256, BlobPtr<uint2>(blob, P.m_pw1.w),
      [&](int t, int s, int n0, int (&acc)[1][4]) { hq[(size_t)(n0 / 4) * LQ2 + t * S + s] = epi(acc, n0); });
  }
  MixedUnitPw2I8<S, NT, L::kI8Pd>(blob, P, hq, u, resq, aq, LQA, 1);
  static_assert(DecStateC::kRingQ1 == DecStateC::kRingQ0 + 64 * 6, "ring blocks back to back");
  ResUnitsI8x2<S, NT, L::kI8Pd>(blob, P.q, aq, LQA, 1, resq, dq8, hq, stw + (size_t)DecStateC::kRingQ0 * S, n18, active);
  {
    const uint32_t pad = PackI8x4(up1.g.in_zp, up1.g.in_zp, up1.g.in_zp, up1.g.in_zp);
    for (int i = tid; i < 64 * S; i += NT) { const int c = i / S, s = i % S; aq[(size_t)c * LQA + s] = pad; aq[(size_t)c * LQA + 3 * S + s] = pad; }
    BatchedLoop<NT, 8, float>(128 * 4 * S,
      [&](int i) { const int c = i / (4 * S), r = i % (4 * S); return r < 2 * S ? st[DecStateC::kUp1 * S + (size_t)c * 2 * S + r] : 0.0f; },
      [&](int i, float v) { u1[i] = v; });
  }
  __syncthreads();
  {
    const int* bias = BlobPtr<int>(blob, up1.g.bias);
    const int* mult = BlobPtr<int>(blob, up1.g.mult);
    const int* shift = BlobPtr<int>(blob, up1.g.shift);
    float* tail = st + (size_t)DecStateC::kUp1 * S;
    if (!TC) IssuePrologue<NT>(wbuf, NextF32(BlobPtr<float>(blob, P.r1[0].pw1.w), 16, 128, 128));
    GemmI8Mma<S, NT, 8>(aq, LQA, 0, 1, 2, 128, 2, 3, 256, BlobPtr<uint2>(blob, up1.g.w),
      [&](int q, int s, int n0, int (&acc)[1][4]) {
        const RequantP4 rq = LoadRequant4(bias, mult, shift, n0);
        const int g = n0 / 128, r = (n0 % 128) / 64;
        const float* bf = BlobPtr<float>(blob, up1.bias_f32[g]);
#pragma unroll
        for (int j = 0; j < 4; ++j) {
          const int co = (n0 + j) % 64, ch = g * 64 + co;
          const int qv = RequantI8(acc[0][j], rq.b[j], rq.m[j], rq.s[j], up1.out_zp[g]);
          const float f = DequantizeI8(qv, up1.dq[g].scale, up1.dq[g].zp);
          if (q < 2) {
            float* o = u1 + (size_t)ch * 4 * S + (2 * q + r) * S + s;
            *o = __fadd_rn(f, *o);
          } else if (active[s]) {
            tail[((size_t)ch * 2 + r) * S + s] = __fsub_rn(__fadd_rn(f, 0.0f), bf[co]);
          }
        }
      });
  }
  static_assert(DecStateC::kRing1 == DecStateC::kRing0 + 128 * 2 && DecStateC::kRing2 == DecStateC::kRing1 + 128 * 6, "ring blocks back to back");
  ResUnitsF32x3<S, NT, TM, TN, TN, L::WM4, 16, 128, 4, TC, L::LD1, L::RWM, L::RWN>(
      blob, P.r1, u1, 4 * S, 0, d1, 2, st + (size_t)DecStateC::kRing0 * S, n18, active, wbuf, NoNext());
  {
    float* out = mid + (size_t)tile * 128 * 4 * S;
    for (int i = tid; i < 128 * 4 * S; i += NT) out[i] = u1[i];
  }
  AdvanceHopCounters<S>(n18g, tile, active, n18);
}

struct DecD {
  static constexpr int S = kTileStreams;
  static constexpr int NT = 320;
  static constexpr int TN = 4;
  static constexpr int kMinBlocks = 2;
  static constexpr int TNU = 5;
  static constexpr int TNL = 2;
  static constexpr int WML = 4;
  static constexpr int WMU = 1;
  static constexpr int KCU = 8;
  static constexpr int LDU = 26 * S, LDD = 20 * S, LDX = 6 * S;
  static constexpr int kU = 0;
  static constexpr int kD = kU + 64 * LDU * 4;
  static constexpr int kW = kD + 64 * LDD * 4;
  static constexpr int kWBytes = kStages * 16 * 64 * 4 + 2048;
  static constexpr int kSl = kW + kWBytes;
  static_assert(128 * 6 * S * 4 + kStages * KCU * 320 * 4 <= 64 * LDD * 4 + kWBytes, "decoder_2/simple ring must fit behind X");
  static constexpr int kI = kSl + 48 * S * 4;
  static constexpr int kSmemBytes = kI + 3 * S * 4 + 16;
  static_assert(128 * LDX <= 64 * LDD, "X must fit in d");
  static_assert(S * 320 * 2 <= 64 * LDD * 4, "PCM staging must fit in d");
};

__global__ void __launch_bounds__(DecD::NT, DecD::kMinBlocks)
DecoderKernelD(const uint8_t* __restrict__ blob, DecoderParams P, TileIo io, const float* __restrict__ mid,
               float* __restrict__ state, int* __restrict__ n18g, int16_t* __restrict__ pcm) {
  using L = DecD;
  constexpr int S = L::S, NT = L::NT;
  unsigned char* smem = LYRA_DYN_SMEM();
  float* u = reinterpret_cast<float*>(smem + L::kU);
  float* d = reinterpret_cast<float*>(smem + L::kD);
  float* X = d;
  float* wbuf = reinterpret_cast<float*>(smem + L::kW);
  float* sl = reinterpret_cast<float*>(smem + L::kSl);
  int* slot = reinterpret_cast<int*>(smem + L::kI);
  int* active = slot + S;
  int* n18 = active + S;
  int tile;
  InitWeightPipe<NT>();
  if (!BeginTile<S>(io, n18g, slot, state, DecStateD::kUnits, tile)) return;
  float* st = state + (size_t)tile * DecStateD::kUnits * S;
  const int tid = (int)threadIdx.x;
  constexpr int LDX = L::LDX;
  float* wbuf_up2 = X + 128 * LDX;
  IssuePrologue<NT>(wbuf_up2, NextF32(BlobPtr<float>(blob, P.up2.w), L::KCU, 320, 256));

  {
    const float* in = mid + (size_t)tile * 128 * 4 * S;
    BatchedLoop<NT, 4, float4>(128 * S, [&](int i) { return reinterpret_cast<const float4*>(in)[i]; },
      [&](int i, float4 v) { const int c = i / S, r = (i % S) * 4; *reinterpret_cast<float4*>(X + (size_t)c * LDX + S + r) = v; });
    for (int i = tid; i < 128 * 2 * S; i += NT) { const int c = i / (2 * S), r = i % (2 * S); X[(size_t)c * LDX + (r < S ? r : 4 * S + r)] = 0.0f; }
    for (int i = tid; i < 64 * 26 * S / 4; i += NT) {
      const int c = (i * 4) / (26 * S), r = (i * 4) % (26 * S);
      if (!(r >= 3 * S && r < 8 * S)) *reinterpret_cast<float4*>(u + (size_t)c * L::LDU + r) = make_float4(0.0f, 0.0f, 0.0f, 0.0f);
    }
    BatchedLoop<NT, 8, float>(64 * 5 * S, [&](int i) { return st[DecStateD::kUp2 * S + i]; },
      [&](int i, float v) { const int c = i / (5 * S), r = i % (5 * S); u[(size_t)c * L::LDU + 3 * S + r] = v; });
    BatchedLoop<NT, 2, float>(48 * S, [&](int i) { return st[DecStateD::kLast * S + i]; }, [&](int i, float v) { sl[i] = v; });
  }
  __syncthreads();
  {
    const float* b = BlobPtr<float>(blob, P.up2.bias);
    float* tail = st + (size_t)DecStateD::kUp2 * S;
    auto epi_up = [&](int q, int s0, int n0, auto& acc) {
      constexpr int TMx = sizeof(acc) / sizeof(acc[0]), TNx = sizeof(acc[0]) / sizeof(float);
#pragma unroll
      for (int j = 0; j < TNx; ++j) {
        const int r = (n0 + j) / 64, co = (n0 + j) % 64;
        const float bias = b[co];
#pragma unroll
        for (int i = 0; i < TMx; ++i) {
          const float y = __fadd_rn(acc[i][j], bias);
          if (q < 4) {
            float* o = u + (size_t)co * L::LDU + (3 + 5 * q + r) * S + s0 + i;
            *o = __fadd_rn(y, *o);
          } else if (active[s0 + i]) {
            tail[((size_t)co * 5 + r) * S + s0 + i] = __fsub_rn(__fadd_rn(y, 0.0f), bias);
          }
        }
      }
    };
    GemmF32Tap<S, NT, 8, L::TNU, L::KCU, L::WMU, false>(X, LDX, 0, 1, 2, 128, 1, 5, 320, BlobPtr<float>(blob, P.up2.w), wbuf_up2, true,
                                                        NextF32(BlobPtr<float>(blob, P.r2[0].pw1.w), 16, 64, 64, wbuf), epi_up);
  }
  static_assert(DecStateD::kRing1 == DecStateD::kRing0 + 64 * 2 && DecStateD::kRing2 == DecStateD::kRing1 + 64 * 6, "ring blocks back to back");
  ResUnitsF32x3<S, NT, 8, L::TN, L::TN, 4, 16, 64, 20>(blob, P.r2, u, L::LDU, 3, d, 1, st + (size_t)DecStateD::kRing0 * S, n18, active, wbuf,
                                                       NextF32(BlobPtr<float>(blob, P.last.w), 16, 16, 256));
  {
    const float bias = BlobPtr<float>(blob, P.last.bias)[0];
    float* tail = st + (size_t)DecStateD::kLast * S;
    int16_t* stage = reinterpret_cast<int16_t*>(d);
    auto epi_last = [&](int q, int s0, int n0, auto& acc) {
      constexpr int TMx = sizeof(acc) / sizeof(acc[0]), TNx = sizeof(acc[0]) / sizeof(float);
#pragma unroll
      for (int j = 0; j < TNx; ++j) {
        const int t = 16 * q + n0 + j;
#pragma unroll
        for (int i = 0; i < TMx; ++i) {
          const float y = __fadd_rn(__fadd_rn(acc[i][j], bias), t < 48 ? sl[t * S + s0 + i] : 0.0f);
          if (t < 320) {
            float v = __fmul_rn(y, 32768.0f);
            v = v > -32768.0f ? v : -32768.0f;
            v = v < 32767.0f ? v : 32767.0f;
            stage[(s0 + i) * 320 + t] = (int16_t)(int)v;
          } else if (active[s0 + i]) {
            tail[(t - 320) * S + s0 + i] = __fsub_rn(y, bias);
          }
        }
      }
    };
    GemmF32Tap<S, NT, 8, L::TNL, 16, L::WML, false>(u, L::LDU, 0, 1, 4, 64, 1, 23, 16, BlobPtr<float>(blob, P.last.w), wbuf, true, NoNext(), epi_last);
    for (int i = tid; i < S * 320; i += NT) {
      const int s = i / 320;
      if (active[s]) pcm[(size_t)slot[s] * 320 + (i % 320)] = stage[i];
    }
  }
  AdvanceHopCounters<S>(n18g, tile, active, n18);
}

}
```

Baseline: 4.217 million.

## Process two stream tiles per block in encoder kernel B

Templates EncoderKernelB on tiles-per-block and launches a two-tile variant when enough tiles are active, using a TileLanes accessor so that state, ring buffers and inputs address two separate per-tile bases. The int8 MMA GEMM gains an MTW parameter so that each warp handles several M tiles and reuses each loaded weight fragment across them. The aim is to amortise weight loads and staging across twice as many streams per block and to give larger GEMM M dimensions. The cost is more shared memory and registers per block, which may reduce occupancy, and half as many blocks.

```diff
diff --git a/lyra_b200/csrc/engine.cu b/lyra_b200/csrc/engine.cu
--- a/lyra_b200/csrc/engine.cu
+++ b/lyra_b200/csrc/engine.cu
@@ -311,12 +311,19 @@
 };
 Part WholeCall(lyra_b200_ctx* ctx, int n) { return Part{0, ctx->active_tiles, 0, n, ctx->stream}; }
 
+constexpr int kEncBPairMinTiles = 128;
+
 int LaunchEncoderNets(lyra_b200_ctx* ctx, const Part& p, const uint8_t* skip, const int16_t* d_pcm, float* d_features) {
-  const TileIo io{ctx->d_tile_list + p.tile0, ctx->d_slot_of, skip};
+  const TileIo io{ctx->d_tile_list + p.tile0, p.ntiles, ctx->d_slot_of, skip};
   const int rc = LAUNCH(0, EncoderKernelA, dim3((unsigned)p.ntiles), dim3(EncA::NT), (size_t)EncA::kSmemBytes, p.st,
                         ctx->d_blob, ctx->spec.enc, io, d_pcm, reinterpret_cast<float*>(ctx->d_state[0]), ctx->d_n18[0], ctx->d_mid_enc);
-  return rc ? rc : LAUNCH(1, EncoderKernelB, dim3((unsigned)p.ntiles), dim3(EncB::NT), (size_t)EncB::kSmemBytes, p.st,
-                          ctx->d_blob, ctx->spec.enc, io, ctx->d_mid_enc, reinterpret_cast<float*>(ctx->d_state[1]), ctx->d_n18[1], d_features);
+  if (rc) return rc;
+  float* st_b = reinterpret_cast<float*>(ctx->d_state[1]);
+  return p.ntiles >= kEncBPairMinTiles
+             ? LAUNCH(1, EncoderKernelB<2>, dim3((unsigned)((p.ntiles + 1) / 2)), dim3(EncB<2>::NT), (size_t)EncB<2>::kSmemBytes, p.st,
+                      ctx->d_blob, ctx->spec.enc, io, ctx->d_mid_enc, st_b, ctx->d_n18[1], d_features)
+             : LAUNCH(1, EncoderKernelB<1>, dim3((unsigned)p.ntiles), dim3(EncB<1>::NT), (size_t)EncB<1>::kSmemBytes, p.st,
+                      ctx->d_blob, ctx->spec.enc, io, ctx->d_mid_enc, st_b, ctx->d_n18[1], d_features);
 }
 
 int LaunchQuantize(lyra_b200_ctx* ctx, const Part& p, const float* d_features, int num_bits, uint8_t* d_packets, int* d_indices,
@@ -338,7 +345,7 @@
 }
 
 int LaunchDecoderNets(lyra_b200_ctx* ctx, const Part& p, const uint8_t* skip, const float* d_features, int16_t* d_pcm) {
-  const TileIo io{ctx->d_tile_list + p.tile0, ctx->d_slot_of, skip};
+  const TileIo io{ctx->d_tile_list + p.tile0, p.ntiles, ctx->d_slot_of, skip};
   const bool tc = ctx->decoder_mode == LYRA_B200_DECODER_TENSOR;
   const dim3 grid((unsigned)p.ntiles);
   float* st_c = reinterpret_cast<float*>(ctx->d_state[2]);
@@ -538,7 +545,8 @@
 }
 
 bool SetSmemLimits() {
-  return LYRA_SET_MAX_SMEM(EncoderKernelA, EncA::kSmemBytes) == 0 && LYRA_SET_MAX_SMEM(EncoderKernelB, EncB::kSmemBytes) == 0 &&
+  return LYRA_SET_MAX_SMEM(EncoderKernelA, EncA::kSmemBytes) == 0 && LYRA_SET_MAX_SMEM(EncoderKernelB<1>, EncB<1>::kSmemBytes) == 0 &&
+         LYRA_SET_MAX_SMEM(EncoderKernelB<2>, EncB<2>::kSmemBytes) == 0 &&
          LYRA_SET_MAX_SMEM(DecoderKernelC<false>, DecC<false>::kSmemBytes) == 0 && LYRA_SET_MAX_SMEM(DecoderKernelD, DecD::kSmemBytes) == 0 &&
          LYRA_SET_MAX_SMEM(DecoderKernelC<true>, DecC<true>::kSmemBytes) == 0 && LYRA_SET_MAX_SMEM(DecoderKernelDW, DecDW::kSmemBytes) == 0;
 }
diff --git a/lyra_b200/csrc/kernel_prims.cuh b/lyra_b200/csrc/kernel_prims.cuh
--- a/lyra_b200/csrc/kernel_prims.cuh
+++ b/lyra_b200/csrc/kernel_prims.cuh
@@ -9,6 +9,31 @@
 __device__ __forceinline__ const T* BlobPtr(const uint8_t* blob, uint32_t off) {
   return reinterpret_cast<const T*>(blob + off);
 }
+
+constexpr int kTileStreams = 8;
+
+template <typename T, int NTL = 1>
+struct TileLanes {
+  T* base[NTL];
+  static_assert(NTL == 1 || NTL == 2, "one or two tiles per block");
+  __device__ __forceinline__ T& operator()(int unit, int s) const {
+    if constexpr (NTL == 1) return base[0][(size_t)unit * kTileStreams + s];
+    else return (s < kTileStreams ? base[0] : base[1])[(size_t)unit * kTileStreams + s % kTileStreams];
+  }
+  __device__ __forceinline__ TileLanes operator+(int units) const {
+    TileLanes r;
+#pragma unroll
+    for (int h = 0; h < NTL; ++h) r.base[h] = base[h] + (size_t)units * kTileStreams;
+    return r;
+  }
+  template <typename U>
+  __device__ __forceinline__ TileLanes<U, NTL> As() const {
+    TileLanes<U, NTL> r;
+#pragma unroll
+    for (int h = 0; h < NTL; ++h) r.base[h] = reinterpret_cast<U*>(base[h]);
+    return r;
+  }
+};
 
 __device__ __forceinline__ float LeakyRelu(float v) { return fmaxf(v, __fmul_rn(v, 0.3f)); }
 
@@ -237,27 +262,36 @@
 }
 
 constexpr int kI8Pd = 2;
-template <int S, int NT, int NTW, int PDI = kI8Pd, typename Epi>
+template <int S, int NT, int NTW, int PDI = kI8Pd, int MTW = 1, typename Epi>
 __device__ __forceinline__ void GemmI8Mma(const uint32_t* A, int ldA, int rowA0, int row_stride, int ntaps, int CinG,
                                           int groups, int T_out, int N, const uint2* __restrict__ Wf, Epi epi) {
   constexpr int PD = PDI;
   const int lane = (int)threadIdx.x & 31, warp = (int)threadIdx.x >> 5, g = lane >> 2, t4 = lane & 3;
-  const int M = T_out * S, MT = (M + 15) / 16, NTILES = N / 8, NWT = MT * (NTILES / NTW);
+  const int M = T_out * S, MT = (M + 15) / 16, MTB = (MT + MTW - 1) / MTW, NTILES = N / 8, NWT = MTB * (NTILES / NTW);
   const int CinG4 = CinG / 4, KS = ntaps * CinG4 / 8, CoutG = N / groups;
   for (int wt = warp; wt < NWT; wt += NT / 32) {
-    const int mt = wt % MT, nt0 = (wt / MT) * NTW;
-    const int m0 = mt * 16 + g, m1 = m0 + 8;
-    const bool valid0 = m0 < M, valid1 = m1 < M;
-    const int tr0 = valid0 ? m0 / S : T_out - 1, tr1 = valid1 ? m1 / S : T_out - 1;
-    const int s0 = m0 % S, s1 = m1 % S;
+    const int mtb = (wt % MTB) * MTW, nt0 = (wt / MTB) * NTW;
     const int grp = (nt0 * 8) / CoutG;
-    const uint32_t* pa0 = A + (size_t)(grp * CinG4) * ldA + (rowA0 + tr0 * row_stride) * S + s0;
-    const uint32_t* pa1 = A + (size_t)(grp * CinG4) * ldA + (rowA0 + tr1 * row_stride) * S + s1;
+    bool valid0[MTW], valid1[MTW];
+    int tr0[MTW], tr1[MTW], s0[MTW], s1[MTW];
+    const uint32_t* pa0[MTW];
+    const uint32_t* pa1[MTW];
+#pragma unroll
+    for (int i = 0; i < MTW; ++i) {
+      const int m0 = (mtb + i) * 16 + g, m1 = m0 + 8;
+      valid0[i] = m0 < M; valid1[i] = m1 < M;
+      tr0[i] = valid0[i] ? m0 / S : T_out - 1; tr1[i] = valid1[i] ? m1 / S : T_out - 1;
+      s0[i] = m0 % S; s1[i] = m1 % S;
+      pa0[i] = A + (size_t)(grp * CinG4) * ldA + (rowA0 + tr0[i] * row_stride) * S + s0[i];
+      pa1[i] = A + (size_t)(grp * CinG4) * ldA + (rowA0 + tr1[i] * row_stride) * S + s1[i];
+    }
     const uint2* wp = Wf + (size_t)nt0 * 32 + lane;
     const size_t ks_stride = (size_t)NTILES * 32;
-    int acc[NTW][4];
-#pragma unroll
-    for (int j = 0; j < NTW; ++j) { acc[j][0] = 0; acc[j][1] = 0; acc[j][2] = 0; acc[j][3] = 0; }
+    int acc[MTW][NTW][4];
+#pragma unroll
+    for (int i = 0; i < MTW; ++i)
+#pragma unroll
+      for (int j = 0; j < NTW; ++j) { acc[i][j][0] = 0; acc[i][j][1] = 0; acc[i][j][2] = 0; acc[i][j][3] = 0; }
     uint2 bf[PD][NTW];
 #pragma unroll
     for (int p = 0; p < PD; ++p)
@@ -272,12 +306,16 @@
         if (ks < KS) {
           const int kw = ks * 8, tap = kw / CinG4, kw0 = kw - tap * CinG4;
           const size_t off = (size_t)(kw0 + t4) * ldA + tap * S;
-          uint32_t a[4];
-          a[0] = pa0[off]; a[1] = pa1[off]; a[2] = pa0[off + 4 * (size_t)ldA]; a[3] = pa1[off + 4 * (size_t)ldA];
+          uint32_t a[MTW][4];
+#pragma unroll
+          for (int i = 0; i < MTW; ++i) {
+            a[i][0] = pa0[i][off]; a[i][1] = pa1[i][off]; a[i][2] = pa0[i][off + 4 * (size_t)ldA]; a[i][3] = pa1[i][off + 4 * (size_t)ldA];
+          }
 #pragma unroll
           for (int j = 0; j < NTW; ++j) {
             const uint32_t b[2] = {bf[p][j].x, bf[p][j].y};
-            lyra_mma_s8_16x8x32(acc[j], a, b);
+#pragma unroll
+            for (int i = 0; i < MTW; ++i) lyra_mma_s8_16x8x32(acc[i][j], a[i], b);
           }
           if (ks + PD < KS) {
 #pragma unroll
@@ -288,15 +326,17 @@
     }
     const bool even = (t4 & 1) == 0;
 #pragma unroll
-    for (int j = 0; j < NTW; ++j) {
-      const int r0 = __shfl_xor_sync(0xffffffffu, even ? acc[j][2] : acc[j][0], 1);
-      const int r1 = __shfl_xor_sync(0xffffffffu, even ? acc[j][3] : acc[j][1], 1);
-      int out[1][4];
-      if (even) { out[0][0] = acc[j][0]; out[0][1] = acc[j][1]; out[0][2] = r0; out[0][3] = r1; }
-      else { out[0][0] = r0; out[0][1] = r1; out[0][2] = acc[j][2]; out[0][3] = acc[j][3]; }
-      const int n4 = (nt0 + j) * 8 + (t4 >> 1) * 4;
-      if (even ? valid0 : valid1) epi(even ? tr0 : tr1, even ? s0 : s1, n4, out);
-    }
+    for (int i = 0; i < MTW; ++i)
+#pragma unroll
+      for (int j = 0; j < NTW; ++j) {
+        const int r0 = __shfl_xor_sync(0xffffffffu, even ? acc[i][j][2] : acc[i][j][0], 1);
+        const int r1 = __shfl_xor_sync(0xffffffffu, even ? acc[i][j][3] : acc[i][j][1], 1);
+        int out[1][4];
+        if (even) { out[0][0] = acc[i][j][0]; out[0][1] = acc[i][j][1]; out[0][2] = r0; out[0][3] = r1; }
+        else { out[0][0] = r0; out[0][1] = r1; out[0][2] = acc[i][j][2]; out[0][3] = acc[i][j][3]; }
+        const int n4 = (nt0 + j) * 8 + (t4 >> 1) * 4;
+        if (even ? valid0[i] : valid1[i]) epi(even ? tr0[i] : tr1[i], even ? s0[i] : s1[i], n4, out);
+      }
   }
   __syncthreads();
 }
@@ -424,18 +464,17 @@
   return make_float4(LeakyRelu(v.x), LeakyRelu(v.y), LeakyRelu(v.z), LeakyRelu(v.w));
 }
 
-template <int S, int NT, int C, int T, int DIL>
+template <int S, int NT, int C, int T, int DIL, typename Ring>
 __device__ __forceinline__ void DwF32RingFast(const float* u, int ldu, int row0u, float* dout, int ldd,
                                               const float* __restrict__ w, const float* __restrict__ bias,
-                                              float* __restrict__ ring, int n18u, const int* active) {
+                                              const Ring& ring, int n18u, const int* active) {
   constexpr int R = 2 * DIL, Q = S / 4;
   const int base = (n18u * T) % R;
   for (int item = (int)threadIdx.x; item < C * Q; item += NT) {
     const int c = item / Q, s4 = (item % Q) * 4;
-    float* rc = ring + (size_t)c * R * S + s4;
     float4 rg[R];
 #pragma unroll
-    for (int j = 0; j < R; ++j) rg[j] = *reinterpret_cast<const float4*>(rc + ((base + j) % R) * S);
+    for (int j = 0; j < R; ++j) rg[j] = *reinterpret_cast<const float4*>(&ring(c * R + (base + j) % R, s4));
     const float w0 = w[c], w1 = w[C + c], w2 = w[2 * C + c], b = bias[c];
     const float* uc = u + (size_t)c * ldu + row0u * S + s4;
     float* dc = dout + (size_t)c * ldd + s4;
@@ -459,7 +498,7 @@
 #pragma unroll
     for (int t = TF; t < T; ++t) {
       const float4 a = LeakyRelu4(*reinterpret_cast<const float4*>(uc + t * S));
-      float* dst = rc + ((base + t) % R) * S;
+      float* dst = &ring(c * R + (base + t) % R, s4);
       if (all4) {
         *reinterpret_cast<float4*>(dst) = a;
       } else {
@@ -473,9 +512,9 @@
   __syncthreads();
 }
 
-template <int S, int NT, int C, int T, int DIL>
+template <int S, int NT, int C, int T, int DIL, typename Ring>
 __device__ __forceinline__ void DwI8RingFast(const uint32_t* aq, int lda, int row0a, uint32_t* dq, int ldd,
-                                             const uint8_t* blob, const DwI8& p, uint32_t* __restrict__ ring, int n18u,
+                                             const uint8_t* blob, const DwI8& p, const Ring& ring, int n18u,
                                              const int* active) {
   constexpr int R = 2 * DIL, C4 = C / 4;
   const int base = (n18u * T) % R;
@@ -485,14 +524,13 @@
   const int* shift = BlobPtr<int>(blob, p.shift);
   for (int item = (int)threadIdx.x; item < C4 * S; item += NT) {
     const int c4 = item / S, s = item % S;
-    uint32_t* rc = ring + (size_t)c4 * R * S + s;
     const uint32_t* ac = aq + (size_t)c4 * lda + row0a * S + s;
     uint32_t x0[T], x1[T], x2[T];
 #pragma unroll
     for (int t = 0; t < T; ++t) {
       x2[t] = ac[t * S];
-      x1[t] = t - DIL >= 0 ? ac[(t - DIL) * S] : rc[((base + t - DIL + 2 * R) % R) * S];
-      x0[t] = t - 2 * DIL >= 0 ? ac[(t - 2 * DIL) * S] : rc[((base + t - 2 * DIL + 2 * R) % R) * S];
+      x1[t] = t - DIL >= 0 ? ac[(t - DIL) * S] : ring(c4 * R + (base + t - DIL + 2 * R) % R, s);
+      x0[t] = t - 2 * DIL >= 0 ? ac[(t - 2 * DIL) * S] : ring(c4 * R + (base + t - 2 * DIL + 2 * R) % R, s);
     }
     int wk[3][4], bb[4], mm[4], sh[4];
 #pragma unroll
@@ -514,16 +552,16 @@
     constexpr int TF = T > R ? T - R : 0;
     if (active[s]) {
 #pragma unroll
-      for (int t = TF; t < T; ++t) rc[((base + t) % R) * S] = x2[t];
-    }
-  }
-  __syncthreads();
-}
-
-template <int S, int NT>
+      for (int t = TF; t < T; ++t) ring(c4 * R + (base + t) % R, s) = x2[t];
+    }
+  }
+  __syncthreads();
+}
+
+template <int S, int NT, typename Ring>
 __device__ __forceinline__ void DwF32Ring(const float* u, int ldu, int row0u, float* dout, int ldd, int C, int T, int dil,
                                           const float* __restrict__ w, const float* __restrict__ bias,
-                                          float* __restrict__ ring, const int* n18, const int* active) {
+                                          const Ring& ring, const int* n18, const int* active) {
   const int R = 2 * dil;
   const int total = C * T * S;
   for (int idx = (int)threadIdx.x; idx < total; idx += NT) {
@@ -531,8 +569,8 @@
     const int base = (n18[s] * T) % R;
     const float* uc = u + (size_t)c * ldu + row0u * S + s;
     const float x2 = LeakyRelu(uc[t * S]);
-    const float x1 = t - dil >= 0 ? LeakyRelu(uc[(t - dil) * S]) : ring[((size_t)c * R + RingSlot(base, t - dil, R)) * S + s];
-    const float x0 = t - 2 * dil >= 0 ? LeakyRelu(uc[(t - 2 * dil) * S]) : ring[((size_t)c * R + RingSlot(base, t - 2 * dil, R)) * S + s];
+    const float x1 = t - dil >= 0 ? LeakyRelu(uc[(t - dil) * S]) : ring(c * R + RingSlot(base, t - dil, R), s);
+    const float x0 = t - 2 * dil >= 0 ? LeakyRelu(uc[(t - 2 * dil) * S]) : ring(c * R + RingSlot(base, t - 2 * dil, R), s);
     float acc = __fmaf_rn(x0, w[c], 0.0f);
     acc = __fmaf_rn(x1, w[C + c], acc);
     acc = __fmaf_rn(x2, w[2 * C + c], acc);
@@ -546,14 +584,14 @@
     const int s = idx % S, t = tfirst + (idx / S) % nrows, c = idx / (S * nrows);
     if (!active[s]) continue;
     const int base = (n18[s] * T) % R;
-    ring[((size_t)c * R + RingSlot(base, t, R)) * S + s] = LeakyRelu(u[(size_t)c * ldu + (row0u + t) * S + s]);
-  }
-  __syncthreads();
-}
-
-template <int S, int NT>
+    ring(c * R + RingSlot(base, t, R), s) = LeakyRelu(u[(size_t)c * ldu + (row0u + t) * S + s]);
+  }
+  __syncthreads();
+}
+
+template <int S, int NT, typename Ring>
 __device__ __forceinline__ void DwI8Ring(const uint32_t* aq, int lda, int row0a, uint32_t* dq, int ldd, int C, int T, int dil,
-                                         const uint8_t* blob, const DwI8& p, uint32_t* __restrict__ ring, const int* n18,
+                                         const uint8_t* blob, const DwI8& p, const Ring& ring, const int* n18,
                                          const int* active) {
   const int R = 2 * dil, C4 = C / 4;
   const int* w = BlobPtr<int>(blob, p.w);
@@ -566,8 +604,8 @@
     const int base = (n18[s] * T) % R;
     const uint32_t* ac = aq + (size_t)c4 * lda + row0a * S + s;
     const uint32_t x2 = ac[t * S];
-    const uint32_t x1 = t - dil >= 0 ? ac[(t - dil) * S] : ring[((size_t)c4 * R + RingSlot(base, t - dil, R)) * S + s];
-    const uint32_t x0 = t - 2 * dil >= 0 ? ac[(t - 2 * dil) * S] : ring[((size_t)c4 * R + RingSlot(base, t - 2 * dil, R)) * S + s];
+    const uint32_t x1 = t - dil >= 0 ? ac[(t - dil) * S] : ring(c4 * R + RingSlot(base, t - dil, R), s);
+    const uint32_t x0 = t - 2 * dil >= 0 ? ac[(t - 2 * dil) * S] : ring(c4 * R + RingSlot(base, t - 2 * dil, R), s);
     int o[4];
 #pragma unroll
     for (int b = 0; b < 4; ++b) {
@@ -585,9 +623,9 @@
     const int s = idx % S, t = tfirst + (idx / S) % nrows, c4 = idx / (S * nrows);
     if (!active[s]) continue;
     const int base = (n18[s] * T) % R;
-    ring[((size_t)c4 * R + RingSlot(base, t, R)) * S + s] = aq[(size_t)c4 * lda + (row0a + t) * S + s];
-  }
-  __syncthreads();
-}
-
-}
+    ring(c4 * R + RingSlot(base, t, R), s) = aq[(size_t)c4 * lda + (row0a + t) * S + s];
+  }
+  __syncthreads();
+}
+
+}
diff --git a/lyra_b200/csrc/net_kernels.cuh b/lyra_b200/csrc/net_kernels.cuh
--- a/lyra_b200/csrc/net_kernels.cuh
+++ b/lyra_b200/csrc/net_kernels.cuh
@@ -5,8 +5,6 @@
 #include "kernel_prims.cuh"
 
 namespace lyra_b200 {
-
-constexpr int kTileStreams = 8;
 
 struct EncStateA {
   static constexpr int kFirst = 0;
@@ -43,6 +41,7 @@
 
 struct TileIo {
   const int* tile_list;
+  int ntiles;
   const int* slot_of_stream;
   const uint8_t* skip;
 };
@@ -70,6 +69,10 @@
 
 constexpr int kMax(int a, int b) { return a > b ? a : b; }
 
+constexpr int F32WarpTiles(int S, int T, int N, int TM, int TN, int WM) {
+  return ((T * S / TM + WM - 1) / WM) * ((N / TN + 32 / WM - 1) / (32 / WM));
+}
+
 __device__ __forceinline__ void PrefetchTileState(const void* p, int bytes) {
   if (threadIdx.x == 0) lyra_prefetch_l2(p, (unsigned)bytes);
 }
@@ -88,18 +91,71 @@
   if (tid < S && active[tid]) n18g[tile * S + tid] = (n18[tid] + 1) % 18;
 }
 
-template <int S, int NT, int C, int R, typename T>
-__device__ __forceinline__ void StoreCarriedRows(T* st, int unit, const T* buf, int ld, int row0, const int* active) {
+template <int NTL, typename T>
+__device__ __forceinline__ TileLanes<T, NTL> TileBlocks(T* base, const int* tiles, int units) {
+  TileLanes<T, NTL> r;
+#pragma unroll
+  for (int h = 0; h < NTL; ++h) r.base[h] = base + (size_t)(tiles[h] >= 0 ? tiles[h] : tiles[0]) * units * kTileStreams;
+  return r;
+}
+
+template <int NTL>
+__device__ __forceinline__ bool BeginTiles(const TileIo& io, const int* n18g, int* meta, float* state, int units,
+                                           TileLanes<float, NTL>& st) {
+  constexpr int S = NTL * kTileStreams;
+  int* slot = meta;
+  int* active = meta + S;
+  int* n18 = meta + 2 * S;
+  int* tiles = n18 + S + 1;
+  const int tid = (int)threadIdx.x;
+  if (tid < S) {
+    const int h = tid / kTileStreams, k = (int)blockIdx.x * NTL + h;
+    const int tile = k < io.ntiles ? io.tile_list[k] : -1;
+    int sl = -1, n = 0;
+    if (tile >= 0) {
+      const int stream = tile * kTileStreams + tid % kTileStreams;
+      sl = io.slot_of_stream[stream];
+      n = n18g[stream];
+    }
+    slot[tid] = sl;
+    active[tid] = sl >= 0 && !(io.skip != nullptr && io.skip[sl]);
+    n18[tid] = n;
+    if (tid % kTileStreams == 0) tiles[h] = tile;
+  }
+  __syncthreads();
+  if (tid == 0) {
+    int u = -2;
+    for (int s = 0; s < S; ++s)
+      if (active[s]) u = (u == -2 || u == n18[s]) ? n18[s] : -1;
+    n18[S] = u;
+  }
+  __syncthreads();
+  if (n18[S] == kTileIdle) return false;
+  st = TileBlocks<NTL>(state, tiles, units);
+#pragma unroll
+  for (int h = 0; h < NTL; ++h)
+    if (tiles[h] >= 0) PrefetchTileState(st.base[h], units * kTileStreams * 4);
+  return true;
+}
+
+template <int NTL>
+__device__ __forceinline__ void AdvanceHopCountersOfTiles(int* n18g, const int* tiles, const int* active, const int* n18) {
+  const int tid = (int)threadIdx.x;
+  if (tid < NTL * kTileStreams && active[tid]) n18g[tiles[tid / kTileStreams] * kTileStreams + tid % kTileStreams] = (n18[tid] + 1) % 18;
+}
+
+template <int S, int NT, int C, int R, typename St, typename T>
+__device__ __forceinline__ void StoreCarriedRows(const St& st, int unit, const T* buf, int ld, int row0, const int* active) {
   for (int i = (int)threadIdx.x; i < C * R * S; i += NT) {
     const int c = i / (R * S), r = i % (R * S);
-    if (active[r % S]) st[unit * S + i] = buf[(size_t)c * ld + row0 * S + r];
+    if (active[r % S]) st(unit + i / S, i % S) = buf[(size_t)c * ld + row0 * S + r];
   }
 }
 
 template <int S, int NT, int TM, int TN1, int TN2, int WM, int KC, int C, int T, int DIL, bool TC = false, int LDD = T * S,
-          int WTM = 1, int WTN = 1, int STG = kStages>
+          int WTM = 1, int WTN = 1, int STG = kStages, typename Ring>
 __device__ __forceinline__ void ResUnitF32(const uint8_t* blob, const ResF32& p, float* u, int ldu, int row0u, float* d,
-                                           int groups2, float* ring, const int* n18,
+                                           int groups2, const Ring& ring, const int* n18,
                                            const int* active, float* wbuf, bool last, const WNext& after, int dil_rt = DIL) {
   constexpr int ldd = LDD;
   if (n18[S] >= 0) {
@@ -154,14 +210,14 @@
 }
 
 template <int S, int NT, int TM, int TN1, int TN2, int WM, int KC, int C, int T, bool TC = false, int LDD = T * S, int WTM = 1, int WTN = 1,
-          int STG = kStages>
+          int STG = kStages, typename Ring>
 __device__ __forceinline__ void ResUnitsF32x3(const uint8_t* blob, const ResF32* p3, float* u, int ldu, int row0u, float* d, int groups2,
-                                              float* ring0, const int* n18, const int* active, float* wbuf, const WNext& after) {
+                                              const Ring& ring0, const int* n18, const int* active, float* wbuf, const WNext& after) {
 #pragma unroll 1
   for (int i = 0; i < 3; ++i) {
     const ResF32& p = p3[i];
     const int dil = i == 0 ? 1 : (i == 1 ? 3 : 9);
-    float* ring = ring0 + (size_t)(i == 0 ? 0 : (i == 1 ? 2 : 8)) * C * S;
+    const Ring ring = ring0 + (i == 0 ? 0 : (i == 1 ? 2 : 8)) * C;
     const WNext nx = i < 2 ? NextF32(BlobPtr<float>(blob, p3[i + 1].pw1.w), KC, C, C, nullptr, STG) : after;
     ResUnitF32<S, NT, TM, TN1, TN2, WM, KC, C, T, 0, TC, LDD, WTM, WTN, STG>(blob, p, u, ldu, row0u, d, groups2, ring, n18, active, wbuf, i == 2, nx,
                                                                        dil);
@@ -190,13 +246,14 @@
 __device__ __forceinline__ void MixedUnitPw2I8(const uint8_t* blob, const Params& P, const uint32_t* hq, const float* u,
                                                uint32_t* resq, uint32_t* aq, int lda, int row0a) {
   constexpr int LQ2 = PadLd(2 * S), LD2 = 2 * S;
+  constexpr int MTW = (2 * S + 15) / 16;
   const int* bias = BlobPtr<int>(blob, P.m_pw2.bias);
   const int* mult = BlobPtr<int>(blob, P.m_pw2.mult);
   const int* shift = BlobPtr<int>(blob, P.m_pw2.shift);
   const int8_t* lut = BlobPtr<int8_t>(blob, P.m_lr2.lut);
   const QuantP dq = P.m_dq, q2 = P.m_q2;
   const int out_zp = P.m_pw2.out_zp;
-  GemmI8Mma<S, NT, 4, PDI>(hq, LQ2, 0, 1, 1, 64, 4, 2, 256, BlobPtr<uint2>(blob, P.m_pw2.w),
+  GemmI8Mma<S, NT, 4, PDI, MTW>(hq, LQ2, 0, 1, 1, 64, 4, 2, 256, BlobPtr<uint2>(blob, P.m_pw2.w),
     [&](int t, int s, int n0, int (&acc)[1][4]) {
       const RequantP4 rq = LoadRequant4(bias, mult, shift, n0);
       int r[4], a[4];
@@ -212,12 +269,12 @@
     });
 }
 
-template <int S, int NT, int DIL, int PDI = kI8Pd>
+template <int S, int NT, int DIL, int PDI = kI8Pd, typename Ring>
 __device__ __forceinline__ void ResUnitI8(const uint8_t* blob, const ResI8& p, uint32_t* aq, int lda, int row0a,
-                                          uint32_t* resq, uint32_t* dq8, uint32_t* hq, uint32_t* ring,
+                                          uint32_t* resq, uint32_t* dq8, uint32_t* hq, const Ring& ring,
                                           const int* n18, const int* active, int dil_rt = DIL) {
   constexpr int T = 2, C = 256, LD = PadLd(T * S);
-  constexpr int NTW = 4;
+  constexpr int NTW = 4, MTW = (T * S + 15) / 16;
   if (n18[S] >= 0) {
     if constexpr (DIL != 0) DwI8RingFast<S, NT, C, T, DIL>(aq, lda, row0a, dq8, LD, blob, p.dw, ring, n18[S], active);
     else if (dil_rt == 3) DwI8RingFast<S, NT, C, T, 3>(aq, lda, row0a, dq8, LD, blob, p.dw, ring, n18[S], active);
@@ -227,7 +284,7 @@
   }
   {
     const RequantLutPack epi(blob, p.pw1, p.lr1);
-    GemmI8Mma<S, NT, NTW, PDI>(dq8, LD, 0, 1, 1, C, 1, T, C, BlobPtr<uint2>(blob, p.pw1.w),
+    GemmI8Mma<S, NT, NTW, PDI, MTW>(dq8, LD, 0, 1, 1, C, 1, T, C, BlobPtr<uint2>(blob, p.pw1.w),
       [&](int t, int s, int n0, int (&acc)[1][4]) { hq[(size_t)(n0 / 4) * LD + t * S + s] = epi(acc, n0); });
   }
   {
@@ -238,7 +295,7 @@
     const int* l2 = BlobPtr<int>(blob, p.add.lut2);
     const int8_t* lut = BlobPtr<int8_t>(blob, p.lr2.lut);
     const int out_zp = p.pw2.out_zp, m3 = p.add.m3, s3 = p.add.s3, add_zp = p.add.out_zp;
-    GemmI8Mma<S, NT, NTW, PDI>(hq, LD, 0, 1, 1, C / 4, 4, T, C, BlobPtr<uint2>(blob, p.pw2.w),
+    GemmI8Mma<S, NT, NTW, PDI, MTW>(hq, LD, 0, 1, 1, C / 4, 4, T, C, BlobPtr<uint2>(blob, p.pw2.w),
       [&](int t, int s, int n0, int (&acc)[1][4]) {
         const RequantP4 rq = LoadRequant4(bias, mult, shift, n0);
         const size_t ro = (size_t)(n0 / 4) * LD + t * S + s;
@@ -256,13 +313,13 @@
   }
 }
 
-template <int S, int NT, int PDI = kI8Pd>
+template <int S, int NT, int PDI = kI8Pd, typename Ring>
 __device__ __forceinline__ void ResUnitsI8x2(const uint8_t* blob, const ResI8* p2, uint32_t* aq, int lda, int row0a,
-                                             uint32_t* resq, uint32_t* dq8, uint32_t* hq, uint32_t* ring0,
+                                             uint32_t* resq, uint32_t* dq8, uint32_t* hq, const Ring& ring0,
                                              const int* n18, const int* active) {
 #pragma unroll 1
   for (int i = 0; i < 2; ++i)
-    ResUnitI8<S, NT, 0, PDI>(blob, p2[i], aq, lda, row0a, resq, dq8, hq, ring0 + (size_t)(i ? 64 * 6 : 0) * S, n18, active, i ? 9 : 3);
+    ResUnitI8<S, NT, 0, PDI>(blob, p2[i], aq, lda, row0a, resq, dq8, hq, ring0 + (i ? 64 * 6 : 0), n18, active, i ? 9 : 3);
 }
 
 struct EncA {
@@ -297,6 +354,7 @@
   InitWeightPipe<NT>();
   if (!BeginTile<S>(io, n18g, slot, state, EncStateA::kUnits, tile)) return;
   float* st = state + (size_t)tile * EncStateA::kUnits * S;
+  const TileLanes<float> stl{{st}};
   const int tid = (int)threadIdx.x;
   IssuePrologue<NT>(wbuf, NextF32(BlobPtr<float>(blob, P.first.w), 16, 64, 64));
 
@@ -325,9 +383,9 @@
       });
   }
   static_assert(EncStateA::kRing1 == EncStateA::kRing0 + 64 * 2 && EncStateA::kRing2 == EncStateA::kRing1 + 64 * 6, "ring blocks back to back");
-  ResUnitsF32x3<S, NT, 8, L::TN, L::TN, 4, 16, 64, 20>(blob, P.r0, u, L::LDU, 5, d, 1, st + (size_t)EncStateA::kRing0 * S, n18, active, wbuf,
+  ResUnitsF32x3<S, NT, 8, L::TN, L::TN, 4, 16, 64, 20>(blob, P.r0, u, L::LDU, 5, d, 1, stl + EncStateA::kRing0, n18, active, wbuf,
                                                        NextF32(BlobPtr<float>(blob, P.down0.w), 16, 128, 640, d, L::kStgDown));
-  StoreCarriedRows<S, NT, 64, 5>(st, EncStateA::kDown0, u, L::LDU, 20, active);
+  StoreCarriedRows<S, NT, 64, 5>(stl, EncStateA::kDown0, u, L::LDU, 20, active);
   {
     const float* b = BlobPtr<float>(blob, P.down0.bias);
     float* out = mid + (size_t)tile * 128 * 4 * S;
@@ -346,34 +404,38 @@
   AdvanceHopCounters<S>(n18g, tile, active, n18);
 }
 
+template <int kTilesPerBlock>
 struct EncB {
-  static constexpr int S = kTileStreams;
+  static constexpr int NTL = kTilesPerBlock;
+  static constexpr int S = NTL * kTileStreams;
   static constexpr int NT = 256;
-  static constexpr int kMinBlocks = 3;
+  static constexpr int kMinBlocks = NTL == 2 ? 2 : 3;
   static constexpr int TM = 8;
   static constexpr int TN = 4;
   static constexpr int WM4 = 4 * S / TM >= 4 ? 4 : 4 * S / TM;
   static constexpr int WM2 = 2 * S / TM >= 4 ? 4 : 2 * S / TM;
-  static constexpr int WM1 = 1 * S / TM >= 4 ? 4 : 1 * S / TM;
+  static constexpr int kWarpTiles4 = F32WarpTiles(S, 4, 128, TM, TN, WM4), kWarpTiles2 = F32WarpTiles(S, 2, 256, TM, TN, WM2);
+  static_assert(kWarpTiles4 <= NT / 32 && kWarpTiles2 <= NT / 32 && (NTL == 1 || (kWarpTiles4 == NT / 32 && kWarpTiles2 == NT / 32)),
+                "warp tiles");
   static constexpr int LD1 = 6 * S;
   static constexpr int LQ2 = PadLd(2 * S), LQA = PadLd(4 * S), LQB = PadLd(3 * S);
   static constexpr int kRA = 0;
   static constexpr int kRABytes = kMax(kMax(128 * LD1 * 4, 256 * 2 * S * 4), 64 * LQA * 4 + 128 * LQB * 4);
   static constexpr int kRB = kRA + kRABytes;
   static constexpr int kRBBytes = kMax(128 * 4 * S * 4, 256 * 2 * S * 4);
-  static constexpr int kRC = kRB + kRBBytes;
-  static constexpr int kW = kRC + 64 * LQ2 * 4;
+  static constexpr int kW = kRB + kRBBytes;
   static constexpr int kStg = 3;
-  static constexpr int kWBytes = kMax(kStg * 8 * 256 * 4, 2 * 64 * LQ2 * 4);
-  static constexpr int kI8Pd = 4;
+  static constexpr int kWBytes = kMax(kStg * 8 * 256 * 4, 3 * 64 * LQ2 * 4);
+  static constexpr int kI8Pd = NTL == 2 ? 2 : 4;
   static constexpr int kI = kW + kWBytes;
   static constexpr int kSmemBytes = kI + 3 * S * 4 + 16;
 };
 
-__global__ void __launch_bounds__(EncB::NT, EncB::kMinBlocks)
+template <int kTilesPerBlock>
+__global__ void __launch_bounds__(EncB<kTilesPerBlock>::NT, EncB<kTilesPerBlock>::kMinBlocks)
 EncoderKernelB(const uint8_t* __restrict__ blob, EncoderParams P, TileIo io, const float* __restrict__ mid,
                float* __restrict__ state, int* __restrict__ n18g, float* __restrict__ features) {
-  using L = EncB;
+  using L = EncB<kTilesPerBlock>;
   constexpr int S = L::S, NT = L::NT;
   constexpr int TM = L::TM, TN = L::TN;
   unsigned char* smem = LYRA_DYN_SMEM();
@@ -384,31 +446,31 @@
   uint32_t* bq = aq + 64 * LQA;
   float* d1 = reinterpret_cast<float*>(smem + L::kRB);
   float* u2 = reinterpret_cast<float*>(smem + L::kRB);
-  uint32_t* hq = reinterpret_cast<uint32_t*>(smem + L::kRC);
   float* wbuf = reinterpret_cast<float*>(smem + L::kW);
-  uint32_t* dq8 = reinterpret_cast<uint32_t*>(smem + L::kW);
+  uint32_t* hq = reinterpret_cast<uint32_t*>(smem + L::kW);
+  uint32_t* dq8 = hq + 64 * LQ2;
   uint32_t* resq = dq8 + 64 * LQ2;
   int* slot = reinterpret_cast<int*>(smem + L::kI);
   int* active = slot + S;
   int* n18 = active + S;
-  int tile;
+  const int* tiles = n18 + S + 1;
+  TileLanes<float, L::NTL> st;
   InitWeightPipe<NT>();
-  if (!BeginTile<S>(io, n18g, slot, state, EncStateB::kUnits, tile)) return;
-  float* st = state + (size_t)tile * EncStateB::kUnits * S;
-  uint32_t* stw = reinterpret_cast<uint32_t*>(st);
+  if (!BeginTiles<L::NTL>(io, n18g, slot, state, EncStateB::kUnits, st)) return;
+  const TileLanes<uint32_t, L::NTL> stw = st.template As<uint32_t>();
   IssuePrologue<NT>(wbuf, NextF32(BlobPtr<float>(blob, P.r1[0].pw1.w), 16, 128, 128, nullptr, L::kStg));
 
   {
-    const float* in = mid + (size_t)tile * 128 * 4 * S;
-    BatchedLoop<NT, 4, float4>(128 * S, [&](int i) { return reinterpret_cast<const float4*>(in)[i]; },
+    const TileLanes<const float, L::NTL> in = TileBlocks<L::NTL>(mid, tiles, 128 * 4);
+    BatchedLoop<NT, 4, float4>(128 * S, [&](int i) { return *reinterpret_cast<const float4*>(&in(i / (S / 4), (i % (S / 4)) * 4)); },
       [&](int i, float4 v) { const int c = i / S, r = (i % S) * 4; *reinterpret_cast<float4*>(u1 + (size_t)c * L::LD1 + 2 * S + r) = v; });
-    BatchedLoop<NT, 8, float>(128 * 2 * S, [&](int i) { return st[EncStateB::kDown1 * S + i]; },
+    BatchedLoop<NT, 8, float>(128 * 2 * S, [&](int i) { return st(EncStateB::kDown1 + i / S, i % S); },
       [&](int i, float v) { const int c = i / (2 * S), r = i % (2 * S); u1[(size_t)c * L::LD1 + r] = v; });
   }
   __syncthreads();
   static_assert(EncStateB::kRing1 == EncStateB::kRing0 + 128 * 2 && EncStateB::kRing2 == EncStateB::kRing1 + 128 * 6, "ring blocks back to back");
   ResUnitsF32x3<S, NT, TM, TN, TN, L::WM4, 16, 128, 4, false, 4 * S, 1, 1, L::kStg>(
-      blob, P.r1, u1, L::LD1, 2, d1, 2, st + (size_t)EncStateB::kRing0 * S, n18, active, wbuf,
+      blob, P.r1, u1, L::LD1, 2, d1, 2, st + EncStateB::kRing0, n18, active, wbuf,
       NextF32(BlobPtr<float>(blob, P.down1.w), 8, 256, 256, wbuf, L::kStg));
   StoreCarriedRows<S, NT, 128, 2>(st, EncStateB::kDown1, u1, L::LD1, 4, active);
   {
@@ -427,10 +489,10 @@
   constexpr int LD2 = 2 * S;
   if (n18[S] >= 0)
     DwF32RingFast<S, NT, 256, 2, 1>(u2, LD2, 0, d2, LD2, BlobPtr<float>(blob, P.m_dw.w), BlobPtr<float>(blob, P.m_dw.bias),
-                                    st + (size_t)EncStateB::kRingM * S, n18[S], active);
+                                    st + EncStateB::kRingM, n18[S], active);
   else
     DwF32Ring<S, NT>(u2, LD2, 0, d2, LD2, 256, 2, 1, BlobPtr<float>(blob, P.m_dw.w), BlobPtr<float>(blob, P.m_dw.bias),
-                     st + (size_t)EncStateB::kRingM * S, n18, active);
+                     st + EncStateB::kRingM, n18, active);
   {
     const float* b = BlobPtr<float>(blob, P.m_pw1.bias);
     const int8_t* lut = BlobPtr<int8_t>(blob, P.m_lr1.lut);
@@ -450,10 +512,10 @@
   }
   MixedUnitPw2I8<S, NT, L::kI8Pd>(blob, P, hq, u2, resq, aq, LQA, 2);
   static_assert(EncStateB::kRingQ1 == EncStateB::kRingQ0 + 64 * 6, "ring blocks back to back");
-  ResUnitsI8x2<S, NT, L::kI8Pd>(blob, P.q, aq, LQA, 2, resq, dq8, hq, stw + (size_t)EncStateB::kRingQ0 * S, n18, active);
-  BatchedLoop<NT, 4, uint32_t>(64 * 2 * S, [&](int i) { return stw[EncStateB::kDown2 * S + i]; },
+  ResUnitsI8x2<S, NT, L::kI8Pd>(blob, P.q, aq, LQA, 2, resq, dq8, hq, stw + EncStateB::kRingQ0, n18, active);
+  BatchedLoop<NT, 4, uint32_t>(64 * 2 * S, [&](int i) { return stw(EncStateB::kDown2 + i / S, i % S); },
     [&](int i, uint32_t v) { const int c = i / (2 * S), r = i % (2 * S); aq[(size_t)c * LQA + r] = v; });
-  BatchedLoop<NT, 8, uint32_t>(128 * 2 * S, [&](int i) { return stw[EncStateB::kBott * S + i]; },
+  BatchedLoop<NT, 8, uint32_t>(128 * 2 * S, [&](int i) { return stw(EncStateB::kBott + i / S, i % S); },
     [&](int i, uint32_t v) { const int c = i / (2 * S), r = i % (2 * S); bq[(size_t)c * LQB + r] = v; });
   __syncthreads();
   StoreCarriedRows<S, NT, 64, 2>(stw, EncStateB::kDown2, aq, LQA, 2, active);
@@ -480,7 +542,7 @@
           o[j] = DequantizeI8(RequantI8(acc[0][j], rq.b[j], rq.m[j], rq.s[j], out_zp), dq.scale, dq.zp);
       });
   }
-  AdvanceHopCounters<S>(n18g, tile, active, n18);
+  AdvanceHopCountersOfTiles<L::NTL>(n18g, tiles, active, n18);
 }
 
 template <bool TC = false>
@@ -553,7 +615,7 @@
     for (int i = tid; i < 128 * S; i += NT) { const int c = i / S, s = i % S; xq[(size_t)c * LQB + s] = pad; xq[(size_t)c * LQB + 2 * S + s] = pad; }
   }
   __syncthreads();
-  StoreCarriedRows<S, NT, 64, 2>(st, DecStateC::kBott, F, 3 * S, 1, active);
+  StoreCarriedRows<S, NT, 64, 2>(TileLanes<float>{{st}}, DecStateC::kBott, F, 3 * S, 1, active);
   {
     const float* b = BlobPtr<float>(blob, P.bott.bias);
     const QuantP q = P.bott_q;
@@ -605,8 +667,8 @@
     }
   }
   __syncthreads();
-  if (n18[S] >= 0) DwI8RingFast<S, NT, 256, 2, 1>(aq, LQA, 1, dq8, LQ2, blob, P.m_dw, stw + (size_t)DecStateC::kRingM * S, n18[S], active);
-  else DwI8Ring<S, NT>(aq, LQA, 1, dq8, LQ2, 256, 2, 1, blob, P.m_dw, stw + (size_t)DecStateC::kRingM * S, n18, active);
+  if (n18[S] >= 0) DwI8RingFast<S, NT, 256, 2, 1>(aq, LQA, 1, dq8, LQ2, blob, P.m_dw, TileLanes<uint32_t>{{stw}} + DecStateC::kRingM, n18[S], active);
+  else DwI8Ring<S, NT>(aq, LQA, 1, dq8, LQ2, 256, 2, 1, blob, P.m_dw, TileLanes<uint32_t>{{stw}} + DecStateC::kRingM, n18, active);
   {
     const RequantLutPack epi(blob, P.m_pw1, P.m_lr1);
     GemmI8Mma<S, NT, 4, L::kI8Pd>(dq8, LQ2, 0, 1, 1, 256, 1, 2, 256, BlobPtr<uint2>(blob, P.m_pw1.w),
@@ -614,7 +676,7 @@
   }
   MixedUnitPw2I8<S, NT, L::kI8Pd>(blob, P, hq, u, resq, aq, LQA, 1);
   static_assert(DecStateC::kRingQ1 == DecStateC::kRingQ0 + 64 * 6, "ring blocks back to back");
-  ResUnitsI8x2<S, NT, L::kI8Pd>(blob, P.q, aq, LQA, 1, resq, dq8, hq, stw + (size_t)DecStateC::kRingQ0 * S, n18, active);
+  ResUnitsI8x2<S, NT, L::kI8Pd>(blob, P.q, aq, LQA, 1, resq, dq8, hq, TileLanes<uint32_t>{{stw}} + DecStateC::kRingQ0, n18, active);
   {
     const uint32_t pad = PackI8x4(up1.g.in_zp, up1.g.in_zp, up1.g.in_zp, up1.g.in_zp);
     for (int i = tid; i < 64 * S; i += NT) { const int c = i / S, s = i % S; aq[(size_t)c * LQA + s] = pad; aq[(size_t)c * LQA + 3 * S + s] = pad; }
@@ -650,7 +712,7 @@
   }
   static_assert(DecStateC::kRing1 == DecStateC::kRing0 + 128 * 2 && DecStateC::kRing2 == DecStateC::kRing1 + 128 * 6, "ring blocks back to back");
   ResUnitsF32x3<S, NT, TM, TN, TN, L::WM4, 16, 128, 4, TC, L::LD1, L::RWM, L::RWN>(
-      blob, P.r1, u1, 4 * S, 0, d1, 2, st + (size_t)DecStateC::kRing0 * S, n18, active, wbuf, NoNext());
+      blob, P.r1, u1, 4 * S, 0, d1, 2, TileLanes<float>{{st}} + DecStateC::kRing0, n18, active, wbuf, NoNext());
   {
     float* out = mid + (size_t)tile * 128 * 4 * S;
     for (int i = tid; i < 128 * 4 * S; i += NT) out[i] = u1[i];
@@ -743,7 +805,7 @@
                                                         NextF32(BlobPtr<float>(blob, P.r2[0].pw1.w), 16, 64, 64, wbuf), epi_up);
   }
   static_assert(DecStateD::kRing1 == DecStateD::kRing0 + 64 * 2 && DecStateD::kRing2 == DecStateD::kRing1 + 64 * 6, "ring blocks back to back");
-  ResUnitsF32x3<S, NT, 8, L::TN, L::TN, 4, 16, 64, 20>(blob, P.r2, u, L::LDU, 3, d, 1, st + (size_t)DecStateD::kRing0 * S, n18, active, wbuf,
+  ResUnitsF32x3<S, NT, 8, L::TN, L::TN, 4, 16, 64, 20>(blob, P.r2, u, L::LDU, 3, d, 1, TileLanes<float>{{st}} + DecStateD::kRing0, n18, active, wbuf,
                                                        NextF32(BlobPtr<float>(blob, P.last.w), 16, 16, 256));
   {
     const float bias = BlobPtr<float>(blob, P.last.bias)[0];
```

After: 4.232 million (median of 6 runs). No clear change (+0.4%).
